# holoskii/Rendering

Measured on AMD Instinct MI355X. Metric: Mrays/s + ms/frame at 4096^2, 250k-tri BVH scene, higher is better.
Workload: dtype f32

## Files before the change

### include/rtx_debug.h

```cpp
#ifndef RTX_DEBUG_H
#define RTX_DEBUG_H
#include "rtx.h"
#ifdef __cplusplus
extern "C" {
#endif

int rtx_frame_mode(rtx_scene* scene, int* mode, float* split_ms, float* fused_ms);
int rtx_set_frame_mode(rtx_scene* scene, int mode);

int rtx_mesh_flatten_probe(const rtx_mesh* mesh, uint32_t* n_wide, void* wide_out, void* prune_out, uint32_t cap_wide, float* root_rec8);
int rtx_wide_node_slots(void);

int rtx_source_p_probe(const float* tris9, uint32_t n, const double* S3, double sigma, int cam, float* out);

int rtx_cost_grid_read(rtx_scene* scene, uint32_t* out, size_t n, uint32_t* grid_w, uint32_t* grid_h);

int rtx_set_knob(rtx_scene* scene, const char* name, double value);

#define RTX_VARIANT_BOXES    1u
#define RTX_VARIANT_PLAIN    2u
#define RTX_VARIANT_ANALYTIC 4u
#define RTX_VARIANT_STATS    8u
#define RTX_VARIANT_CULL     16u
int rtx_kernel_variant(rtx_scene* scene, uint32_t* bits);

int rtx_ssaa_list_read(rtx_scene* scene, uint32_t* info, uint32_t* scan, size_t n);

int rtx_kernel_time_reset(rtx_scene* scene);
int rtx_kernel_time_stats(rtx_scene* scene, int which, uint32_t* launches, double* total_ms);

int rtx_tile_cost_read(rtx_scene* scene, uint32_t* out, size_t n);

int rtx_math_probe(int device, int op, uint32_t n, const float* x, const float* y, float* out);

int rtx_vec_probe(int device, int op, uint32_t n, const float* a, const float* b, float ior, float* out);

int rtx_desc_serialize(const rtx_scene_desc* desc, void* out, size_t cap, size_t* need);

int rtx_bvh_build_mode(int mode);
int rtx_bvh_launches(const rtx_bvh* bvh, uint32_t* launches, int* queued);

int rtx_scene_mesh_read(rtx_scene* scene, uint32_t mesh, uint32_t* counts2, float* node_bounds, int32_t* node_skip, int32_t* leaf_begin,
                        int32_t* leaf_count, uint32_t* refs);
int rtx_scene_mesh_flat_read(rtx_scene* scene, uint32_t mesh, uint32_t* n_wide, void* wide_out, void* prune_out, uint32_t cap_wide, float* root_rec8);
int rtx_scene_edit_times(rtx_scene* scene, float* ms4);
int rtx_scene_lights_read(rtx_scene* scene, uint32_t* n_lights, rtx_light* lights_out, uint32_t cap_lights, size_t* n_point_floats,
                          float* points_out, size_t cap_point_floats);
int rtx_scene_mesh_prune_copy_read(rtx_scene* scene, uint32_t mesh, uint32_t copy, uint32_t* n_copies, uint32_t* n_wide, void* prune_out,
                                   uint32_t cap_wide);
int rtx_scene_objects_read(rtx_scene* scene, uint32_t* n_objects, rtx_object* objects_out, uint32_t cap_objects, uint32_t* n_meshes);

int rtx_live_device_memory(size_t* allocations, size_t* bytes);

#ifdef __cplusplus
}
#endif
#endif
```

### rendering_amd/__init__.py

```python
import ctypes as C
import os

import numpy as np

HERE = os.path.dirname(os.path.abspath(__file__))
ROOT = os.path.dirname(HERE)
LIB_RTX = os.path.join(HERE, "librtx_hip.so")
LIB_HOST = os.path.join(HERE, "librendering_host.so")

__all__ = ["load", "Scene", "Comm", "RtxError", "device_count", "math_probe", "gather_plan", "exported_symbols", "sphere_directions"]


class RtxError(RuntimeError):
    pass


class Counters(C.Structure):
    _fields_ = [("rays", C.c_uint64), ("box_tests", C.c_uint64), ("tri_tests", C.c_uint64), ("moot_rays", C.c_uint64)]


_rtx = None
_host = None

RTX_SYMBOLS = [
    "rtx_last_error", "rtx_device_count", "rtx_scene_create", "rtx_scene_destroy", "rtx_scene_set_view", "rtx_scene_bytes",
    "rtx_render_pass1", "rtx_sobel", "rtx_render_ssaa", "rtx_render_frame", "rtx_render_ac", "rtx_frame_status", "rtx_frame_mode", "rtx_set_frame_mode", "rtx_set_knob", "rtx_cost_grid_read", "rtx_mesh_flatten_probe", "rtx_wide_node_slots", "rtx_source_p_probe", "rtx_quantize_bgr8", "rtx_render_frame_host",
    "rtx_counters_enable", "rtx_counters_reset", "rtx_counters_read", "rtx_last_kernel_ms", "rtx_math_probe",
    "rtx_cast_rays", "rtx_trace_rays", "rtx_kernel_time_reset", "rtx_kernel_time_stats", "rtx_tile_cost_read", "rtx_set_row_ownership",
    "rtx_bvh_build", "rtx_bvh_info", "rtx_bvh_read", "rtx_bvh_destroy",
    "rtx_vec_probe", "rtx_desc_serialize", "rtx_bvh_build_mode", "rtx_bvh_launches", "rtx_comm_unique_id", "rtx_comm_create", "rtx_comm_info", "rtx_comm_destroy", "rtx_comm_agree", "rtx_gather", "rtx_gather_plan",
    "rtx_scene_mesh_read", "rtx_scene_mesh_flat_read", "rtx_scene_edit_times", "rtx_kernel_variant", "rtx_ssaa_list_read", "rtx_live_device_memory",
    "rtx_scene_lights_read", "rtx_scene_mesh_prune_copy_read", "rtx_scene_objects_read",
]

RTX_EDIT_SYMBOLS = ["rtx_scene_set_object", "rtx_scene_update_mesh", "rtx_scene_set_lights", "rtx_scene_set_objects"]

RTX_QUERY_SYMBOLS = ["rtx_occluded_rays"]

RTX_AOV_SYMBOLS = ["rtx_render_aov"]


RTX_AO_SYMBOLS = ["rtx_render_ao"]


class AovBuffers(C.Structure):
    _fields_ = [(n, C.c_void_p) for n in ("depth_dev", "object_dev", "triangle_dev", "uv_dev", "normal_dev", "albedo_dev")]


class AoParams(C.Structure):
    _fields_ = [("n_dirs", C.c_uint32), ("dirs_dev", C.c_void_p), ("radius", C.c_float)]


def sphere_directions(n):
    n = int(n)
    if n < 2 or n % 2:
        raise ValueError("sphere_directions: n must be even and at least 2, got %d" % n)
    i = np.arange(n // 2, dtype=np.float64) + 0.5
    z = 1.0 - 2.0 * i / n
    phi = i * (np.pi * (3.0 - np.sqrt(5.0)))
    r = np.sqrt(1.0 - z * z)
    half = np.stack([r * np.cos(phi), r * np.sin(phi), z], 1).astype(np.float32)
    return np.concatenate([half, -half], 0)


def load():
    global _rtx, _host
    if _rtx is not None:
        return _rtx, _host
    for p in (LIB_RTX, LIB_HOST):
        if not os.path.exists(p):
            raise RtxError("native library %s is missing -- build it with ./build.sh (hipcc, gfx950); "
                           "there is no CPU fallback" % p)
    try:
        import torch
    except Exception:
        pass
    rtx = C.CDLL(LIB_RTX, mode=C.RTLD_GLOBAL)
    host = C.CDLL(LIB_HOST, mode=C.RTLD_GLOBAL)
    rtx.rtx_last_error.restype = C.c_char_p
    vp, u32, i32 = C.c_void_p, C.c_uint32, C.c_int
    rtx.rtx_device_count.argtypes = [C.POINTER(C.c_int)]
    rtx.rtx_render_pass1.argtypes = [vp, u32, u32, vp, vp]
    rtx.rtx_sobel.argtypes = [vp, vp, u32, u32, vp, vp]
    rtx.rtx_render_ssaa.argtypes = [vp, vp, u32, u32, vp, vp]
    rtx.rtx_render_frame.argtypes = [vp, u32, u32, vp, vp, vp]
    rtx.rtx_render_ac.argtypes = [vp, vp, vp, vp]
    rtx.rtx_frame_status.argtypes = [vp, C.POINTER(C.c_uint32)]
    rtx.rtx_set_frame_mode.argtypes = [vp, C.c_int]
    rtx.rtx_set_knob.argtypes = [vp, C.c_char_p, C.c_double]
    rtx.rtx_cost_grid_read.argtypes = [vp, vp, C.c_size_t, C.POINTER(C.c_uint32), C.POINTER(C.c_uint32)]
    rtx.rtx_mesh_flatten_probe.argtypes = [vp, C.POINTER(C.c_uint32), vp, vp, C.c_uint32, vp]
    rtx.rtx_source_p_probe.argtypes = [vp, u32, vp, C.c_double, i32, vp]
    rtx.rtx_frame_mode.argtypes = [vp, C.POINTER(C.c_int), C.POINTER(C.c_float), C.POINTER(C.c_float)]
    rtx.rtx_quantize_bgr8.argtypes = [vp, vp, vp, vp]
    rtx.rtx_render_frame_host.argtypes = [vp, i32, vp]
    rtx.rtx_counters_enable.argtypes = [vp, i32]
    rtx.rtx_counters_reset.argtypes = [vp]
    rtx.rtx_counters_read.argtypes = [vp, C.POINTER(Counters)]
    rtx.rtx_last_kernel_ms.argtypes = [vp, i32, C.POINTER(C.c_float)]
    rtx.rtx_math_probe.argtypes = [i32, i32, u32, vp, vp, vp]
    rtx.rtx_cast_rays.argtypes = [vp, u32, vp, vp, vp]
    rtx.rtx_trace_rays.argtypes = [vp, u32, vp, vp, vp, vp]
    rtx.rtx_occluded_rays.argtypes = [vp, u32, vp, vp, vp, vp]
    rtx.rtx_render_aov.argtypes = [vp, u32, u32, C.POINTER(AovBuffers), vp]
    rtx.rtx_render_ao.argtypes = [vp, u32, u32, C.POINTER(AoParams), vp, vp, vp]
    rtx.rtx_kernel_time_reset.argtypes = [vp]
    rtx.rtx_kernel_time_stats.argtypes = [vp, i32, C.POINTER(C.c_uint32), C.POINTER(C.c_double)]
    rtx.rtx_tile_cost_read.argtypes = [vp, vp, C.c_size_t]
    rtx.rtx_set_row_ownership.argtypes = [vp, u32, u32, u32, i32]
    rtx.rtx_bvh_build.argtypes = [vp, u32, vp, vp, C.c_int32, i32, C.POINTER(vp)]
    rtx.rtx_bvh_info.argtypes = [vp, C.POINTER(u32), C.POINTER(u32), C.POINTER(u32), C.POINTER(C.c_float)]
    rtx.rtx_bvh_launches.argtypes = [vp, C.POINTER(u32), C.POINTER(C.c_int)]
    rtx.rtx_bvh_read.argtypes = [vp, vp, vp, vp, vp, vp]
    rtx.rtx_bvh_destroy.argtypes = [vp]
    rtx.rtx_bvh_destroy.restype = None
    rtx.rtx_scene_bytes.argtypes = [vp, C.POINTER(C.c_size_t)]
    rtx.rtx_vec_probe.argtypes = [i32, i32, u32, vp, vp, C.c_float, vp]
    rtx.rtx_comm_unique_id.argtypes = [vp]
    rtx.rtx_comm_create.argtypes = [vp, i32, i32, i32, C.POINTER(vp)]
    rtx.rtx_comm_info.argtypes = [vp, C.POINTER(C.c_int), C.POINTER(C.c_int)]
    rtx.rtx_comm_destroy.argtypes = [vp]
    rtx.rtx_comm_agree.argtypes = [vp, C.c_int, C.POINTER(C.c_int), vp]
    rtx.rtx_comm_destroy.restype = None
    rtx.rtx_gather.argtypes = [vp, vp, vp, C.c_size_t, i32, i32, vp]
    rtx.rtx_gather_plan.argtypes = [u32, u32, u32, C.c_size_t, i32, u32, vp, vp, vp, C.POINTER(u32)]
    host.rah_set_ac_build.argtypes = [i32, i32]
    host.rah_set_ac_build.restype = None
    host.rah_set_ac_build_device.argtypes = [i32]
    host.rah_set_ac_build_device.restype = None
    host.rah_bvh_build_info.argtypes = [vp, i32, C.POINTER(C.c_int), C.POINTER(C.c_float)]
    host.rah_last_error.restype = C.c_char_p
    host.rah_scene_load.restype = vp
    host.rah_scene_load.argtypes = [C.c_char_p, C.c_char_p, i32, i32]
    host.rah_scene_free.argtypes = [vp]
    host.rah_scene_dims.argtypes = [vp] + [C.POINTER(C.c_int)] * 4
    host.rah_scene_resize.argtypes = [vp, i32, i32]
    host.rah_scene_set_device.argtypes = [vp, i32]
    host.rah_set_flag.argtypes = [vp, C.c_char_p, i32]
    host.rah_flatten.restype = vp
    host.rah_flatten.argtypes = [vp]
    host.rah_flat_desc.restype = vp
    host.rah_flat_desc.argtypes = [vp]
    host.rah_flat_free.argtypes = [vp]
    host.rah_bvh_counts.argtypes = [vp, i32, vp]
    host.rah_scene_gpu.restype = vp
    host.rah_scene_gpu.argtypes = [vp]
    host.rah_render_host.argtypes = [vp, vp, i32]
    host.rah_save_bmp.argtypes = [vp, vp, C.c_char_p]
    host.rah_bvh_dump.argtypes = [vp, i32, vp, vp, vp, vp, vp]
    host.rah_tris.argtypes = [vp, i32, vp]
    host.rah_camera.argtypes = [vp, vp, vp, vp, vp]
    host.rah_scene_digest.argtypes = [vp, vp, i32]
    host.rah_view_flags.argtypes = [vp]
    host.rah_load_bmp.argtypes = [C.c_char_p, C.POINTER(C.c_int), C.POINTER(C.c_int), vp, i32]
    host.rah_object_move.argtypes = [vp, i32] + [vp] * 5
    host.rah_object_type.argtypes = [vp, i32]
    host.rah_object_move_times.argtypes = [vp, vp]
    rtx.rtx_scene_set_object.argtypes = [vp, C.c_uint32, vp]
    rtx.rtx_scene_update_mesh.argtypes = [vp, C.c_uint32, vp, vp, vp, vp, vp, i32, vp]
    rtx.rtx_scene_mesh_read.argtypes = [vp, C.c_uint32] + [vp] * 6
    rtx.rtx_scene_mesh_flat_read.argtypes = [vp, C.c_uint32, vp, vp, vp, C.c_uint32, vp]
    rtx.rtx_scene_edit_times.argtypes = [vp, vp]
    rtx.rtx_kernel_variant.argtypes = [vp, C.POINTER(C.c_uint32)]
    rtx.rtx_ssaa_list_read.argtypes = [vp, vp, vp, C.c_size_t]
    rtx.rtx_live_device_memory.argtypes = [C.POINTER(C.c_size_t), C.POINTER(C.c_size_t)]
    rtx.rtx_scene_set_lights.argtypes = [vp, C.c_uint32, vp]
    rtx.rtx_scene_lights_read.argtypes = [vp, C.POINTER(C.c_uint32), vp, C.c_uint32, C.POINTER(C.c_size_t), vp, C.c_size_t]
    rtx.rtx_scene_mesh_prune_copy_read.argtypes = [vp, C.c_uint32, C.c_uint32, C.POINTER(C.c_uint32), C.POINTER(C.c_uint32), vp, C.c_uint32]
    host.rah_light_type.argtypes = [vp, i32]
    host.rah_light_set.argtypes = [vp, i32] + [vp] * 8
    host.rah_light_add.argtypes = [vp, i32] + [vp] * 8
    host.rah_light_remove.argtypes = [vp, i32]
    rtx.rtx_scene_set_objects.argtypes = [vp, C.c_uint32, vp, C.c_uint32, vp, vp]
    rtx.rtx_scene_objects_read.argtypes = [vp, C.POINTER(C.c_uint32), vp, C.c_uint32, C.POINTER(C.c_uint32)]
    host.rah_object_add.argtypes = [vp, i32, i32, C.c_char_p] + [vp] * 4 + [C.c_char_p] + [vp] * 2 + [C.c_char_p] * 4
    host.rah_object_remove.argtypes = [vp, i32]
    _rtx, _host = rtx, host
    return rtx, host


def exported_symbols():
    rtx, _ = load()
    missing = [s for s in RTX_SYMBOLS + RTX_EDIT_SYMBOLS + RTX_QUERY_SYMBOLS + RTX_AOV_SYMBOLS + RTX_AO_SYMBOLS if not hasattr(rtx, s)]
    return list(RTX_SYMBOLS), missing


VARIANT_BITS = {"boxes": 1, "plain": 2, "analytic": 4, "stats": 8, "cull": 16}


def _check(rc, what):
    if rc != 0:
        raise RtxError("%s failed (%d): %s" % (what, rc, _rtx.rtx_last_error().decode(errors="replace")))


def device_count():
    rtx, _ = load()
    n = C.c_int(0)
    _check(rtx.rtx_device_count(C.byref(n)), "rtx_device_count")
    return n.value


def live_device_memory():
    rtx, _ = load()
    n, b = C.c_size_t(0), C.c_size_t(0)
    _check(rtx.rtx_live_device_memory(C.byref(n), C.byref(b)), "rtx_live_device_memory")
    return n.value, b.value


def _np_ptr(a):
    return a.ctypes.data_as(C.c_void_p)


def set_ac_build(mode, device=0):
    _, host = load()
    host.rah_set_ac_build({"auto": -1, "host": 0, "device": 1}[mode], device)


def bvh_build(tri_pos, root_lo, root_hi, ac_penalty=1, device=0):
    rtx, _ = load()
    pos = np.ascontiguousarray(tri_pos, np.float32).reshape(-1, 9)
    lo = np.ascontiguousarray(root_lo, np.float32); hi = np.ascontiguousarray(root_hi, np.float32)
    b = C.c_void_p()
    _check(rtx.rtx_bvh_build(_np_ptr(pos), pos.shape[0], _np_ptr(lo), _np_ptr(hi), ac_penalty, device, C.byref(b)), "rtx_bvh_build")
    try:
        nn, nr, md, ms = C.c_uint32(), C.c_uint32(), C.c_uint32(), C.c_float()
        _check(rtx.rtx_bvh_info(b, C.byref(nn), C.byref(nr), C.byref(md), C.byref(ms)), "rtx_bvh_info")
        d = dict(bounds=np.zeros((nn.value, 6), np.float32), skip=np.zeros(nn.value, np.int32),
                 leaf_begin=np.zeros(nn.value, np.int32), leaf_count=np.zeros(nn.value, np.int32),
                 refs=np.zeros(nr.value, np.uint32))
        _check(rtx.rtx_bvh_read(b, _np_ptr(d["bounds"]), _np_ptr(d["skip"]), _np_ptr(d["leaf_begin"]), _np_ptr(d["leaf_count"]),
                                _np_ptr(d["refs"])), "rtx_bvh_read")
        d.update(n_nodes=nn.value, n_refs=nr.value, max_depth=md.value, build_ms=ms.value)
        ln, q = C.c_uint32(), C.c_int()
        _check(rtx.rtx_bvh_launches(b, C.byref(ln), C.byref(q)), "rtx_bvh_launches")
        d.update(launches=ln.value, queued=bool(q.value))
        return d
    finally:
        rtx.rtx_bvh_destroy(b)


def bvh_build_mode(mode):
    rtx, _ = load()
    _check(rtx.rtx_bvh_build_mode(int(mode)), "rtx_bvh_build_mode")


def bvh_build_host(tri_pos, root_lo, root_hi, ac_penalty=1):
    _, host = load()
    pos = np.ascontiguousarray(tri_pos, np.float32).reshape(-1, 9)
    lo = np.ascontiguousarray(root_lo, np.float32); hi = np.ascontiguousarray(root_hi, np.float32)
    cnt = np.zeros(4, np.int64)
    host.rah_bvh_from_tris.argtypes = [C.c_void_p, C.c_int, C.c_void_p, C.c_void_p, C.c_int, C.c_void_p] + [C.c_void_p] * 5
    if host.rah_bvh_from_tris(_np_ptr(pos), pos.shape[0], _np_ptr(lo), _np_ptr(hi), ac_penalty, _np_ptr(cnt), None, None, None, None, None) != 0:
        raise RtxError("rah_bvh_from_tris: %s" % host.rah_last_error().decode(errors="replace"))
    nn, nl, nr, md = [int(x) for x in cnt]
    d = dict(bounds=np.zeros((nn, 6), np.float32), skip=np.zeros(nn, np.int32), leaf_begin=np.zeros(nn, np.int32), leaf_count=np.zeros(nn, np.int32),
             refs=np.zeros(max(nr, 1), np.uint32)[:nr])
    host.rah_bvh_from_tris(_np_ptr(pos), pos.shape[0], _np_ptr(lo), _np_ptr(hi), ac_penalty, _np_ptr(cnt), _np_ptr(d["bounds"]), _np_ptr(d["skip"]),
                           _np_ptr(d["leaf_begin"]), _np_ptr(d["leaf_count"]), _np_ptr(d["refs"]))
    d.update(n_nodes=nn, n_leaves=nl, n_refs=nr, max_depth=md)
    return d


def gather_plan(height, band_height, n_parts, row_bytes, bottom_up=False):
    rtx, _ = load()
    n = C.c_uint32(0)
    cap = (height + band_height - 1) // band_height
    owner = np.zeros(cap, np.uint32); off = np.zeros(cap, np.uint64); ln = np.zeros(cap, np.uint64)
    _check(rtx.rtx_gather_plan(height, band_height, n_parts, row_bytes, int(bottom_up), cap, _np_ptr(owner), _np_ptr(off), _np_ptr(ln), C.byref(n)),
           "rtx_gather_plan")
    return [(int(owner[i]), int(off[i]), int(ln[i])) for i in range(n.value)]


class Comm:

    def __init__(self, n_ranks, rank, device, exchange):
        self.rtx, _ = load()
        buf = (C.c_ubyte * 128)()
        if rank == 0:
            _check(self.rtx.rtx_comm_unique_id(buf), "rtx_comm_unique_id")
        raw = exchange(bytes(buf) if rank == 0 else None)
        if len(raw) != 128:
            raise RtxError("communicator id must be 128 bytes")
        self.h = C.c_void_p()
        _check(self.rtx.rtx_comm_create(raw, n_ranks, rank, device, C.byref(self.h)), "rtx_comm_create")
        self.n_ranks, self.rank = n_ranks, rank

    def gather(self, scene, img, bottom_up=False, root=0, stream=None):
        row_bytes = img[0].numel() * img.element_size()
        _check(self.rtx.rtx_gather(scene.gpu(), self.h, C.c_void_p(img.data_ptr()), row_bytes, int(bottom_up), root,
                                   Scene._stream_ptr(stream)), "rtx_gather")

    def info(self):
        n, r = C.c_int(0), C.c_int(0)
        _check(self.rtx.rtx_comm_info(self.h, C.byref(n), C.byref(r)), "rtx_comm_info")
        return n.value, r.value

    def agree(self, ok, stream=None):
        out = C.c_int(0)
        _check(self.rtx.rtx_comm_agree(self.h, int(bool(ok)), C.byref(out), Scene._stream_ptr(stream)), "rtx_comm_agree")
        return bool(out.value)

    def close(self):
        if self.h:
            self.rtx.rtx_comm_destroy(self.h)
            self.h = C.c_void_p()


class RtxLight(C.Structure):
    _fields_ = [("type", C.c_int32), ("color", C.c_float * 3), ("intensity", C.c_float), ("dir", C.c_float * 3), ("pos", C.c_float * 3),
                ("n_points", C.c_uint32), ("points", C.c_void_p)]


LIGHT_TYPES = {"distant": 1, "point": 2, "area": 3}
LIGHT_KEYS = {"distant": ("direction", "color", "intensity"), "point": ("position", "color", "intensity"),
              "area": ("pos", "i", "j", "samples", "color", "intensity")}
_LIGHT_ARGS = ("color", "intensity", "direction", "position", "pos", "i", "j", "samples")


class RtxObject(C.Structure):
    _fields_ = [("type", C.c_int32), ("material", C.c_int32), ("pos", C.c_float * 3), ("color", C.c_float * 3), ("ior", C.c_float),
                ("ambient", C.c_float), ("diffuse", C.c_float), ("specular", C.c_float), ("n_specular", C.c_float), ("radius2", C.c_float),
                ("normal", C.c_float * 3), ("mesh", C.c_int32)]


OBJECT_TYPES = {"sphere": 1, "plane": 2, "mesh": 3}
OBJECT_KEYS = {"sphere": ("pos", "color", "material", "radius"), "plane": ("pos", "color", "material", "normal"),
               "mesh": ("pos", "size", "rot", "color", "material", "name", "diffuse_map", "normal_map", "specular_map")}
_OBJECT_ARGS = ("pos", "size", "rot", "color", "material", "radius", "normal", "name", "diffuse_map", "normal_map", "specular_map")
_OBJECT_TEXT = ("material", "name", "diffuse_map", "normal_map", "specular_map")
MATERIAL_VALUES = {"diffuse": 0, "reflective": 0, "transparent": 1, "phong": 4}


class _RtxMesh(C.Structure):
    _fields_ = [("n_nodes", C.c_uint32), ("n_refs", C.c_uint32), ("n_tris", C.c_uint32), ("node_bounds", C.c_void_p), ("node_skip", C.c_void_p),
                ("leaf_begin", C.c_void_p), ("leaf_count", C.c_void_p), ("refs", C.c_void_p), ("tri_pos", C.c_void_p), ("tri_nrm", C.c_void_p),
                ("tri_uv", C.c_void_p), ("tri_tb", C.c_void_p), ("diffuse_w", C.c_uint32), ("diffuse_h", C.c_uint32), ("diffuse_map", C.c_void_p),
                ("normal_w", C.c_uint32), ("normal_h", C.c_uint32), ("normal_map", C.c_void_p), ("specular_w", C.c_uint32), ("specular_h", C.c_uint32),
                ("specular_map", C.c_void_p)]


class RtxView(C.Structure):
    _fields_ = [("width", C.c_uint32), ("height", C.c_uint32), ("bias", C.c_float), ("max_ray_depth", C.c_int32), ("background", C.c_float * 3),
                ("flags", C.c_uint32), ("cam_pos", C.c_float * 3), ("cam_matrix", C.c_float * 16), ("scale", C.c_float), ("aspect", C.c_float)]


class RtxSceneDesc(C.Structure):
    _fields_ = [("view", RtxView), ("n_objects", C.c_uint32), ("objects", C.POINTER(RtxObject)), ("n_meshes", C.c_uint32),
                ("meshes", C.POINTER(_RtxMesh)), ("n_lights", C.c_uint32), ("lights", C.POINTER(RtxLight)), ("sky_w", C.c_uint32), ("sky_h", C.c_uint32),
                ("sky", C.c_void_p * 6)]


class RtxMeshBuild(C.Structure):
    _fields_ = [("tri_pos_dev", C.c_void_p), ("tri_nrm_dev", C.c_void_p), ("tri_tb_dev", C.c_void_p), ("root_lo", C.c_float * 3),
                ("root_hi", C.c_float * 3), ("ac_penalty", C.c_int32)]


class RtxMeshSource(C.Structure):
    _fields_ = [("keep", C.c_int32), ("mesh", C.POINTER(_RtxMesh)), ("build", C.POINTER(RtxMeshBuild))]


def mesh_flatten_probe(bvh):
    rtx, _ = load()
    bounds = np.ascontiguousarray(bvh["bounds"], np.float32); skip = np.ascontiguousarray(bvh["skip"], np.int32)
    lb = np.ascontiguousarray(bvh["leaf_begin"], np.int32); lc = np.ascontiguousarray(bvh["leaf_count"], np.int32)
    refs = np.ascontiguousarray(bvh["refs"], np.uint32); pos = np.ascontiguousarray(bvh["tris"][:, 0:9], np.float32)
    m = _RtxMesh()
    m.n_nodes, m.n_refs, m.n_tris = len(skip), len(refs), len(pos)
    m.node_bounds, m.node_skip, m.leaf_begin, m.leaf_count = bounds.ctypes.data, skip.ctypes.data, lb.ctypes.data, lc.ctypes.data
    m.refs, m.tri_pos = refs.ctypes.data, pos.ctypes.data
    n = C.c_uint32(0)
    root = np.zeros(8, np.float32)
    _check(rtx.rtx_mesh_flatten_probe(C.byref(m), C.byref(n), None, None, 0, _np_ptr(root)), "rtx_mesh_flatten_probe")
    S = int(rtx.rtx_wide_node_slots())
    wide = np.zeros((n.value, S, 8), np.float32); prune = np.zeros((n.value, 2 * S, 8), np.float32)
    _check(rtx.rtx_mesh_flatten_probe(C.byref(m), C.byref(n), _np_ptr(wide), _np_ptr(prune), n.value, _np_ptr(root)), "rtx_mesh_flatten_probe")
    return wide, prune[:, 0:S], prune[:, S:2 * S], root


def source_p_probe(v0, e1, e2, S, sigma, cam):
    rtx, _ = load()
    t = np.ascontiguousarray(np.concatenate([v0, e1, e2], 1), np.float32)
    S = np.ascontiguousarray(S, np.float64)
    out = np.zeros(len(t), np.float32)
    _check(rtx.rtx_source_p_probe(_np_ptr(t), len(t), _np_ptr(S), float(sigma), 1 if cam else 0, _np_ptr(out)), "rtx_source_p_probe")
    return out


def math_probe(op, x, y=None, device=0):
    rtx, _ = load()
    x = np.ascontiguousarray(x, np.float32)
    out = np.zeros_like(x)
    yp = None
    if y is not None:
        y = np.ascontiguousarray(np.broadcast_to(np.asarray(y, np.float32), x.shape))
        yp = _np_ptr(y)
    _check(rtx.rtx_math_probe(device, op, x.size, _np_ptr(x), yp, _np_ptr(out)), "rtx_math_probe")
    return out


def vec_probe(op, a, b=None, ior=1.0, device=0):
    rtx, _ = load()
    a = np.ascontiguousarray(a, np.float32).reshape(-1, 3)
    out = np.zeros_like(a)
    bp = None
    if b is not None:
        b = np.ascontiguousarray(b, np.float32).reshape(-1, 3)
        bp = _np_ptr(b)
    _check(rtx.rtx_vec_probe(device, op, a.shape[0], _np_ptr(a), bp, ior, _np_ptr(out)), "rtx_vec_probe")
    return out


class Scene:

    def __init__(self, scene_path, width=-1, height=-1, device=0, cwd=ROOT):
        self.rtx, self.host = load()
        self.host.rah_set_ac_build_device(device)
        self.h = C.c_void_p(self.host.rah_scene_load(cwd.encode(), scene_path.encode(), width, height))
        if not self.h:
            raise RtxError("could not load scene %s: %s" % (scene_path, self.host.rah_last_error().decode(errors="replace")))
        self.device = device
        self._cwd = cwd
        self.host.rah_scene_set_device(self.h, device)
        self._dims()
        self._gpu = None

    def _dims(self):
        w, h, no, nl = C.c_int(), C.c_int(), C.c_int(), C.c_int()
        self.host.rah_scene_dims(self.h, C.byref(w), C.byref(h), C.byref(no), C.byref(nl))
        self.width, self.height, self.n_objects, self.n_lights = w.value, h.value, no.value, nl.value

    def close(self):
        if self.h:
            self.host.rah_scene_free(self.h)
            self.h = None
            self._gpu = None

    def resize(self, width, height):
        self.host.rah_scene_resize(self.h, width, height)
        self._dims()

    def camera_pose(self):
        pos, rot = np.zeros(3, np.float32), np.zeros(3, np.float32)
        self.host.rah_camera_get.argtypes = [C.c_void_p] * 3
        self.host.rah_camera_get(self.h, _np_ptr(pos), _np_ptr(rot))
        return pos, rot

    def set_camera(self, pos, rot):
        pos = np.ascontiguousarray(pos, np.float32); rot = np.ascontiguousarray(rot, np.float32)
        self.host.rah_camera_set.argtypes = [C.c_void_p] * 3
        self.host.rah_camera_set(self.h, _np_ptr(pos), _np_ptr(rot))

    def set_flag(self, name, value):
        self.host.rah_set_flag(self.h, name.encode(), int(value))

    def camera(self):
        scale, aspect = C.c_float(), C.c_float()
        m = np.zeros(16, np.float32)
        pos = np.zeros(3, np.float32)
        self.host.rah_camera(self.h, C.byref(scale), C.byref(aspect), _np_ptr(m), _np_ptr(pos))
        return np.float32(scale.value), np.float32(aspect.value), m, pos

    def view_flags(self):
        return self.host.rah_view_flags(self.h)

    def digest(self):
        out = np.zeros(4096, np.float32)
        n = self.host.rah_scene_digest(self.h, _np_ptr(out), out.size)
        return out[:n].copy()

    def bvh(self, obj_idx):
        cnt = np.zeros(5, np.int64)
        if self.host.rah_bvh_counts(self.h, obj_idx, _np_ptr(cnt)) != 0:
            return None
        nn, nl, nr, md, nt = [int(x) for x in cnt]
        d = dict(bounds=np.zeros((nn, 6), np.float32), skip=np.zeros(nn, np.int32),
                 leaf_begin=np.zeros(nn, np.int32), leaf_count=np.zeros(nn, np.int32),
                 refs=np.zeros(nr, np.uint32))
        self.host.rah_bvh_dump(self.h, obj_idx, _np_ptr(d["bounds"]), _np_ptr(d["skip"]), _np_ptr(d["leaf_begin"]),
                               _np_ptr(d["leaf_count"]), _np_ptr(d["refs"]))
        tris = np.zeros((nt, 30), np.float32)
        self.host.rah_tris(self.h, obj_idx, _np_ptr(tris))
        d.update(tris=tris, n_nodes=nn, n_leaves=nl, n_refs=nr, max_depth=md, n_tris=nt)
        on, ms = C.c_int(0), C.c_float(0)
        self.host.rah_bvh_build_info(self.h, obj_idx, C.byref(on), C.byref(ms))
        d.update(built_on_device=bool(on.value), build_ms=ms.value)
        return d

    def bvh_build_info(self, obj_idx):
        on, ms = C.c_int(0), C.c_float(-1)
        if self.host.rah_bvh_build_info(self.h, obj_idx, C.byref(on), C.byref(ms)) != 0:
            return None
        return bool(on.value), ms.value

    def move_object(self, index, pos=None, rot=None, size=None, radius=None, normal=None):
        keys = {"mesh": ("pos", "rot", "size"), "sphere": ("pos", "radius"), "plane": ("pos", "normal")}
        given = {k: v for k, v in (("pos", pos), ("rot", rot), ("size", size), ("radius", radius), ("normal", normal)) if v is not None}
        if not 0 <= index < self.n_objects:
            raise ValueError("move_object: object index %d out of range (%d objects)" % (index, self.n_objects))
        kind = {1: "sphere", 2: "plane", 3: "mesh"}.get(self.host.rah_object_type(self.h, index))
        bad = [k for k in given if kind is None or k not in keys[kind]]
        if bad:
            raise ValueError("move_object: a %s has no key %s (it takes %s)" % (kind, ", ".join(bad), ", ".join(keys.get(kind, ()))))
        arrs = {}
        for k, v in given.items():
            a = np.ascontiguousarray(np.asarray(v, np.float32).reshape(-1))
            if a.size != (1 if k == "radius" else 3):
                raise ValueError("move_object: %s takes %d values, got %d" % (k, 1 if k == "radius" else 3, a.size))
            arrs[k] = a
        ptr = lambda k: _np_ptr(arrs[k]) if k in arrs else None
        if self.host.rah_object_move(self.h, index, ptr("pos"), ptr("rot"), ptr("size"), ptr("radius"), ptr("normal")) != 0:
            raise RtxError("move_object: %s" % self.host.rah_last_error().decode(errors="replace"))

    def light_type(self, index):
        if not 0 <= index < self.n_lights:
            raise ValueError("light_type: light index %d out of range (%d lights)" % (index, self.n_lights))
        return {v: k for k, v in LIGHT_TYPES.items()}[self.host.rah_light_type(self.h, index)]

    @staticmethod
    def _light_args(who, kind, keys):
        bad = [k for k in keys if k not in LIGHT_KEYS[kind]]
        if bad:
            raise ValueError("%s: a %s light has no key %s (it takes %s)" % (who, kind, ", ".join(bad), ", ".join(LIGHT_KEYS[kind])))
        arrs = {}
        for k, v in keys.items():
            want = 1 if k in ("intensity", "samples") else 3
            a = np.ascontiguousarray(np.asarray(v, np.int32 if k == "samples" else np.float32).reshape(-1))
            if a.size != want:
                raise ValueError("%s: %s takes %d value%s, got %d" % (who, k, want, "" if want == 1 else "s", a.size))
            if k == "samples" and a[0] != np.asarray(v).reshape(-1)[0]:
                raise ValueError("%s: samples must be a whole number, got %r" % (who, v))
            arrs[k] = a
        return [_np_ptr(arrs[k]) if k in arrs else None for k in _LIGHT_ARGS], arrs

    def set_light(self, index, **keys):
        if not 0 <= index < self.n_lights:
            raise ValueError("set_light: light index %d out of range (%d lights)" % (index, self.n_lights))
        args, _keep = self._light_args("set_light", self.light_type(index), keys)
        if self.host.rah_light_set(self.h, index, *args) != 0:
            raise RtxError("set_light: %s" % self.host.rah_last_error().decode(errors="replace"))

    def add_light(self, type, **keys):
        if type not in LIGHT_TYPES:
            raise ValueError("add_light: unknown light type %r (point, distant, area)" % (type,))
        args, _keep = self._light_args("add_light", type, keys)
        index = self.host.rah_light_add(self.h, LIGHT_TYPES[type], *args)
        if index < 0:
            raise RtxError("add_light: %s" % self.host.rah_last_error().decode(errors="replace"))
        self._dims()
        return index

    def remove_light(self, index):
        if not 0 <= index < self.n_lights:
            raise ValueError("remove_light: light index %d out of range (%d lights)" % (index, self.n_lights))
        if self.host.rah_light_remove(self.h, index) != 0:
            raise RtxError("remove_light: %s" % self.host.rah_last_error().decode(errors="replace"))
        self._dims()

    def add_object(self, type, at=None, **keys):
        if type not in OBJECT_TYPES:
            raise ValueError("add_object: unknown object type %r (sphere, plane, mesh)" % (type,))
        if at is not None and not 0 <= at <= self.n_objects:
            raise ValueError("add_object: object index %d out of range (%d objects)" % (at, self.n_objects))
        bad = [k for k in keys if k not in OBJECT_KEYS[type]]
        if bad:
            raise ValueError("add_object: a %s has no key %s (it takes %s)" % (type, ", ".join(bad), ", ".join(OBJECT_KEYS[type])))
        arrs = {}
        for k, v in keys.items():
            if k in _OBJECT_TEXT:
                if not isinstance(v, str) or not v or "\n" in v:
                    raise ValueError("add_object: %s takes a line of text, got %r" % (k, v))
                if k == "material":
                    parts = v.split(",")
                    if parts[0] not in MATERIAL_VALUES or len(parts) - 1 != MATERIAL_VALUES[parts[0]]:
                        raise ValueError("add_object: material %r (diffuse, reflective, transparent,<ior>, phong,<ambient>,<diffuse>,<specular>,<n>)" % (v,))
                    try:
                        [float(x) for x in parts[1:]]
                    except ValueError:
                        raise ValueError("add_object: material %r: its values must be numbers" % (v,))
                arrs[k] = v.encode()
                continue
            want = 1 if k == "radius" else 3
            a = np.ascontiguousarray(np.asarray(v, np.float32).reshape(-1))
            if a.size != want:
                raise ValueError("add_object: %s takes %d value%s, got %d" % (k, want, "" if want == 1 else "s", a.size))
            arrs[k] = a
        args = [(arrs[k] if k in _OBJECT_TEXT else _np_ptr(arrs[k])) if k in arrs else None for k in _OBJECT_ARGS]
        index = self.host.rah_object_add(self.h, OBJECT_TYPES[type], -1 if at is None else at, self._cwd.encode(), *args)
        if index < 0:
            raise RtxError("add_object: %s" % self.host.rah_last_error().decode(errors="replace"))
        self._dims()
        return index

    def remove_object(self, index):
        if not 0 <= index < self.n_objects:
            raise ValueError("remove_object: object index %d out of range (%d objects)" % (index, self.n_objects))
        if self.host.rah_object_remove(self.h, index) != 0:
            raise RtxError("remove_object: %s" % self.host.rah_last_error().decode(errors="replace"))
        self._dims()

    def gpu(self):
        self._gpu = C.c_void_p(self.host.rah_scene_gpu(self.h))
        if not self._gpu:
            raise RtxError("no GPU scene: %s" % self.host.rah_last_error().decode(errors="replace"))
        return self._gpu

    @staticmethod
    def _stream_ptr(stream):
        if stream is None:
            try:
                import torch
                if torch.cuda.is_available():
                    return C.c_void_p(torch.cuda.current_stream().cuda_stream)
            except Exception:
                pass
            return None
        return C.c_void_p(getattr(stream, "cuda_stream", stream))

    def render_pass1(self, fb, rows=None, stream=None):
        r0, r1 = rows if rows is not None else (0, self.height)
        _check(self.rtx.rtx_render_pass1(self.gpu(), r0, r1, C.c_void_p(fb.data_ptr()), self._stream_ptr(stream)),
               "rtx_render_pass1")

    def sobel(self, fb, mask, rows=None, stream=None):
        r0, r1 = rows if rows is not None else (0, self.height)
        _check(self.rtx.rtx_sobel(self.gpu(), C.c_void_p(fb.data_ptr()), r0, r1, C.c_void_p(mask.data_ptr()),
                                  self._stream_ptr(stream)), "rtx_sobel")

    def render_ssaa(self, mask, fb, rows=None, stream=None):
        r0, r1 = rows if rows is not None else (0, self.height)
        _check(self.rtx.rtx_render_ssaa(self.gpu(), C.c_void_p(mask.data_ptr()), r0, r1, C.c_void_p(fb.data_ptr()),
                                        self._stream_ptr(stream)), "rtx_render_ssaa")

    def render_frame(self, fb, mask, rows=None, stream=None):
        r0, r1 = rows if rows is not None else (0, self.height)
        _check(self.rtx.rtx_render_frame(self.gpu(), r0, r1, C.c_void_p(fb.data_ptr()), C.c_void_p(mask.data_ptr()),
                                         self._stream_ptr(stream)), "rtx_render_frame")

    def render_ac(self, fb, counts=None, stream=None):
        cp = C.c_void_p(counts.data_ptr()) if counts is not None else None
        _check(self.rtx.rtx_render_ac(self.gpu(), C.c_void_p(fb.data_ptr()), cp, self._stream_ptr(stream)), "rtx_render_ac")

    def set_knob(self, name, value):
        _check(self.rtx.rtx_set_knob(self.gpu(), name.encode(), float(value)), "rtx_set_knob")

    def kernel_variant(self):
        b = C.c_uint32(0)
        _check(self.rtx.rtx_kernel_variant(self.gpu(), C.byref(b)), "rtx_kernel_variant")
        return {k: bool(b.value & bit) for k, bit in VARIANT_BITS.items()}

    def ssaa_list(self):
        g = self.gpu()
        info = np.zeros(16, np.uint32)
        _check(self.rtx.rtx_ssaa_list_read(g, _np_ptr(info), None, 0), "rtx_ssaa_list_read")
        d = dict(local=bool(info[0]), flagged=int(info[1]), sparse=bool(info[2]), tiles=int(info[3]), tiles_x=int(info[4]),
                 heavy_ticks=int(info[5]), spread_slots=int(info[6]), very=int(info[7]), spread_px=int(info[8]),
                 split4=int(info[9]), split16=int(info[10]), cost_sum=int(info[11]) | int(info[12]) << 32, frame_waves=int(info[13]), scan=None)
        if d["tiles"]:
            scan = np.zeros(2 * d["tiles"] + 1, np.uint32)
            _check(self.rtx.rtx_ssaa_list_read(g, _np_ptr(info), _np_ptr(scan), scan.size), "rtx_ssaa_list_read")
            d["scan"] = scan
        return d

    def cost_grid(self):
        gw, gh = C.c_uint32(0), C.c_uint32(0)
        _check(self.rtx.rtx_cost_grid_read(self.gpu(), None, 0, C.byref(gw), C.byref(gh)), "rtx_cost_grid_read")
        g = np.zeros((gh.value, gw.value, 2), np.uint32)
        _check(self.rtx.rtx_cost_grid_read(self.gpu(), _np_ptr(g), g.size, C.byref(gw), C.byref(gh)), "rtx_cost_grid_read")
        return g[..., 0], g[..., 1]

    def frame_status(self):
        st = C.c_uint32(0)
        _check(self.rtx.rtx_frame_status(self.gpu(), C.byref(st)), "rtx_frame_status")
        return st.value

    def set_frame_mode(self, mode):
        _check(self.rtx.rtx_set_frame_mode(self.gpu(), int(mode)), "rtx_set_frame_mode")

    def frame_mode(self):
# ... 277 lines not shown
```

### rendering_amd/csrc/rtx_api.hip

```cpp
#include <hip/hip_runtime.h>

#include <cstdio>
#include <dlfcn.h>
#include <algorithm>
#include <array>
#include <functional>
#include <cmath>
#include <cstring>
#include <memory>
#include <string>
#include <type_traits>
#include <vector>

#include "../../include/rtx.h"
#include "../../include/rtx_debug.h"
#include "../../include/rtx_scene_edit.h"
#include "../../include/rtx_query.h"
#include "../../include/rtx_aov.h"
#include "../../include/rtx_ao.h"
#include "rtx_device.h"
#include "rtx_own.h"

using namespace rtxd;
using rtxown::DevArray; using rtxown::DevBag; using rtxown::Event; using rtxown::PinnedArray;

#include "rtx_kernels.hip"
#include "rtx_source.hip"
#include "rtx_rays.hip"
#include "rtx_aov.hip"
#include "rtx_ao.hip"

hipError_t rtxSortRayKeys(void* temp, size_t* tempBytes, const uint32_t* keysIn, uint32_t* keysOut, uint32_t* order, uint32_t n, int endBit,
                          hipStream_t st);

namespace {

thread_local std::string gErr;

struct RoctxApi { int (*push)(const char*) = nullptr; int (*pop)() = nullptr; };
const RoctxApi& roctx()
{
	static const RoctxApi api = [] {
		RoctxApi a;
		if (!getenv("ROCP_TOOL_LIBRARIES") && !getenv("RTX_ROCTX")) return a;
		void* h = dlopen("librocprofiler-sdk-roctx.so.1", RTLD_NOW | RTLD_GLOBAL);
		if (!h) h = dlopen("libroctx64.so.4", RTLD_NOW | RTLD_GLOBAL);
		if (!h) return a;
		a.push = (int (*)(const char*))dlsym(h, "roctxRangePushA");
		a.pop = (int (*)())dlsym(h, "roctxRangePop");
		if (!a.push || !a.pop) a = RoctxApi();
		return a;
	}();
	return api;
}
struct RoctxRange {
	bool on;
	explicit RoctxRange(const char* name) : on(roctx().push != nullptr) { if (on) roctx().push(name); }
	~RoctxRange() { if (on) roctx().pop(); }
};

int scanExclusive(uint32_t* data, uint32_t n, uint32_t* tmp, hipStream_t st, uint32_t& launches);

int fail(int code, const std::string& msg) { gErr = msg; return code; }

#define HIPCHK(expr)                                                                                         \
	do {                                                                                                     \
		hipError_t e_ = (expr);                                                                              \
		if (e_ != hipSuccess)                                                                                \
			return fail(RTX_ERR_DEVICE, std::string(#expr) + ": " + hipGetErrorString(e_));                  \
	} while (0)

template <typename F> auto dispatchVariant(bool boxes, bool cull, bool third, F&& f)
{
	auto withThird = [&](auto b, auto c) { return third ? f(b, c, std::true_type()) : f(b, c, std::false_type()); };
	auto withCull = [&](auto b) { return cull ? withThird(b, std::integral_constant<int, 1>()) : withThird(b, std::integral_constant<int, 0>()); };
	return boxes ? withCull(std::true_type()) : withCull(std::false_type());
}

}

namespace {

void makeRef(const rtx_mesh& m, uint32_t ref, RefA& a, RefB& b, RefC& c)
{
	const uint32_t t = m.refs[ref];
	const float* p = m.tri_pos + (size_t)t * 9;
	a.v0x = p[0]; a.v0y = p[1]; a.v0z = p[2]; a.tri = t;
	b.e1x = p[3] - p[0]; b.e1y = p[4] - p[1]; b.e1z = p[5] - p[2];
	b.e2x = p[6] - p[0]; c.e2y = p[7] - p[1]; c.e2z = p[8] - p[2];
}

}

struct Knobs {
	int pass1BlocksPerCU = 0, ssaaBlocksPerCU = 0, frameBlocksPerCU = 0;
	bool prune = true;
	bool sources = true;
	int pruneBoxes = -1;
	bool estimate = true;
	bool estimateShadows = true;
	float costPerRef = 2.0f, costPerLeaf = 95.0f, costBase = 6100.0f;
	float fatFactor = 3.0f;
	uint32_t stripLimit = 100000u;
	uint32_t heavyTicks = 18000u;
	uint32_t spreadSlots = 1u << 20;
	uint32_t splitPercent = 100;
	long long localBelow = -1;
	long long sparseBelow = -1;
	int frameMode = -1;
	uint32_t frameRuleTiles = 65536u, frameRuleTilesAnalytic = 8192u;
	uint32_t frameQueueCap = 0;
	bool debugItems = false;
	int traceReorder = -1;
	int traceOriginFirst = 1;
	int occludedSceneOrder = 0;
	uint32_t dbgTile = 0;
};

struct rtx_scene {
	int device = 0;
	int numCUs = 0;
	Knobs knobs;
	DevBag owned;
	DevBag lightsOwned;
	std::vector<Light> lightRecs;
	std::vector<Mesh> meshRecs;
	std::vector<DevBag> meshOwned;
	std::vector<DevBag> meshFixed;
	DevBag recordsOwned;
	std::vector<Object> objectRecs;
	std::vector<rtx_object> objectDescs;
	DevArray<float> sphereLeafDev;
	DevArray<char> flatScratch;
	float editMs[4] = { 0, 0, 0, 0 };
	Params params;
	bool stats = false;
	bool analytic = true;
	bool boxPrune = false;
	bool plain = true;
	DevArray<float> frames; size_t framesArea = 0;
	DevArray<uint32_t> tileCost, items; size_t tileCap = 0;
	DevArray<uint32_t> ssaaPixels;
	DevArray<uint32_t> work;
	DevArray<unsigned long long> counters;
	DevArray<uint32_t> orderWork;
	int blocksPass1 = 0, blocksSsaa = 0, blocksFrame = 0;
	DevArray<uint32_t> tileDeps; DevArray<unsigned long long> tileFlags; DevArray<uint8_t> tileClass;
	DevArray<unsigned long long> ssaaQueue;
	DevArray<unsigned long long> frameCtl;
	uint32_t epoch = 0;
	std::vector<float> meshBounds;
	struct TileQueues {
		std::vector<uint32_t> key;
		uint32_t* list = nullptr;
		uint8_t* need = nullptr; uint32_t listed = 0;
		uint32_t* countExpect = nullptr; bool needValid = false;
		bool costValid = false;
		uint64_t lastUse = 0;
		float frameMs[2] = { -1.f, -1.f };
		uint32_t frameSamples[2] = { 0, 0 };
		uint32_t framesSeen = 0, generation = 0;
		bool fusedGaveUp = false;
		hipStream_t builtOn = nullptr; Event builtEv;
		void forget()
		{
			key.clear(); costValid = false;
			frameMs[0] = frameMs[1] = -1.f; frameSamples[0] = frameSamples[1] = 0; framesSeen = 0; generation++; fusedGaveUp = false;
		}
	};
	struct LastFused { bool valid = false; uint32_t rowBegin = 0, rowEnd = 0; float* fb = nullptr; uint8_t* mask = nullptr; void* stream = nullptr; size_t queue = ~(size_t)0; uint32_t generation = 0;
	                   uint64_t viewSerial = 0; uint32_t bandH = 0, nParts = 0, part = 0, halo = 0; };
	LastFused lastFused;
	uint32_t framesRecovered = 0;
	DevArray<uint32_t> acCounts, acMax;
	DevArray<uint32_t> rayKeys, rayOrder; size_t rayCap = 0;
	DevArray<char> raySortTemp;
	DevArray<uint32_t> rayWork;
	int rayHitBlocks[2] = { 0, 0 };
	int rayOccludedBlocks[2][2] = { { 0, 0 }, { 0, 0 } };
	struct MeshLeaves { const float* boxes; uint32_t n; };
	std::vector<MeshLeaves> meshLeaves;
	DevArray<uint32_t> costGrid;
	DevArray<uint8_t> needSlab; size_t needStride = 0;
	DevArray<uint32_t> listSlab; size_t listStride = 0;
	DevArray<uint32_t> orderedList;
	bool costsUsable = false;
	struct SrcMesh { PruneBlock* pruneAlloc = nullptr; uint32_t pruneWide = 0; PruneBlock* base = nullptr; uint32_t nWide = 0, nRefs = 0; const RefA* refA = nullptr; const RefB* refB = nullptr; const RefC* refC = nullptr;
	                 const uint32_t* slotRange = nullptr; float* refP = nullptr; float* blockP = nullptr; float vmax = 0; uint32_t meshIndex = 0; };
	std::vector<SrcMesh> srcMeshes;
	std::vector<std::array<float, 4>> estLights;
	std::vector<std::array<float, 6>> estPlanes;
	std::vector<std::array<float, 3>> srcLightPos;
	std::vector<uint8_t> srcLightIsPoint;
	float srcNmax = 1.0f;
	float srcBuiltBias = -1.0f; bool srcLightsBuilt = false;
	std::vector<uint8_t> srcLightFresh;
	float srcBuiltCam[3] = { 0, 0, 0 }; bool srcCamBuilt = false;
	hipStream_t lastRenderStream = nullptr; bool rendered = false;
	Event evPrepDone; bool prepRecorded = false; hipStream_t prepSeenBy = nullptr;
	struct RenderStream { hipStream_t st = nullptr; Event done; bool active = false, prepSeen = false; };
	std::vector<RenderStream> renderStreams;
	struct PlanSlot { uint32_t* host = nullptr; uint32_t* dev = nullptr; size_t capWords = 0; PinnedArray<uint32_t> own; Event done; bool used = false; };
	PinnedArray<uint32_t> planRingBase;
	PlanSlot planRing[8]; unsigned planNext = 0;
	bool verifyLists = false;
	struct FrameProbe { Event a, b; int mode = -1; size_t queue = 0; uint32_t generation = 0; bool pending = false, refresh = false; };
	FrameProbe probes[8];
	unsigned probeNext = 0;
	int lastFrameMode = -1, frameModeForced = -1;
	uint64_t viewSerial = 1, ssaaLayoutKey = 0;
	uint32_t ssaaLayoutAge = 0;
	uint32_t ssaaListTiles = 0, ssaaListHeavy = 0, ssaaListSpread = 0;
	size_t lastFrameQueue = ~(size_t)0;
	std::vector<TileQueues> tileQueues;
	uint64_t tileUse = 0;
	std::vector<Event> evPool[5];
	size_t evUsed[5] = { 0, 0, 0, 0, 0 };
	bool evCollect = false;
};

namespace {

void readKnobs(Knobs& k)
{
	const char* allow = ::getenv("RTX_ALLOW_ENV_KNOBS");
	if (!(allow && allow[0] == '1')) return;
	auto getenv = [](const char* name) { return ::getenv(name); };
	auto num = [](const char* name, long long dflt) { const char* e = ::getenv(name); return e ? strtoll(e, nullptr, 10) : dflt; };
	k.pass1BlocksPerCU = (int)num("RTX_PASS1_BLOCKS_PER_CU", 0); k.ssaaBlocksPerCU = (int)num("RTX_SSAA_BLOCKS_PER_CU", 0); k.frameBlocksPerCU = (int)num("RTX_FRAME_BLOCKS_PER_CU", 0);
	k.prune = !getenv("RTX_NO_PRUNE");
	k.sources = !getenv("RTX_NO_SRC");
	k.pruneBoxes = (int)num("RTX_PRUNE_BOXES", -1);
	k.estimate = !getenv("RTX_NO_COST_ESTIMATE");
	k.estimateShadows = !getenv("RTX_NO_SHADOW_ESTIMATE");
	if (const char* e = getenv("RTX_COST_COEFFS")) sscanf(e, "%f,%f,%f", &k.costPerRef, &k.costPerLeaf, &k.costBase);
	if (const char* e = getenv("RTX_FAT_FACTOR")) k.fatFactor = strtof(e, nullptr);
	k.stripLimit = (uint32_t)num("RTX_STRIP_LIMIT", k.stripLimit);
	k.heavyTicks = (uint32_t)num("RTX_SSAA_HEAVY_TICKS", k.heavyTicks);
	k.spreadSlots = (uint32_t)std::min<long long>(num("RTX_SSAA_SPREAD_SLOTS", k.spreadSlots), 1ll << 20);
	k.splitPercent = (uint32_t)num("RTX_SPLIT_PERCENT", k.splitPercent);
	k.localBelow = num("RTX_SSAA_LOCAL_BELOW", -1);
	k.sparseBelow = num("RTX_SSAA_SPARSE_BELOW", -1);
	if (const char* e = getenv("RTX_FRAME_MODE")) k.frameMode = !strcmp(e, "split") ? 0 : (!strcmp(e, "fused") ? 1 : -1);
	k.frameQueueCap = (uint32_t)num("RTX_FRAME_QUEUE_CAP", 0);
	k.debugItems = getenv("RTX_DEBUG_ITEMS") != nullptr;
	if (const char* e = getenv("RTX_DBG_TILE")) { unsigned tx = 0, ty = 0; if (sscanf(e, "%u,%u", &tx, &ty) == 2) k.dbgTile = ((ty << 16) | tx) + 1; }
}

void chooseBoxPrune(rtx_scene* s)
{
	s->boxPrune = false;
	for (const Object& d : s->objectRecs) {
		if (d.type != RTX_OBJ_MESH) continue;
		if (d.pruneBoxes && s->knobs.pruneBoxes != 0) s->boxPrune = true;
		if (s->knobs.pruneBoxes > 0 && d.prune) s->boxPrune = true;
	}
}

int setView(rtx_scene* s, const rtx_view* v)
{
	if (v->width < 2 || v->height < 2) return fail(RTX_ERR_ARG, "view: width/height must be >= 2");
	View& d = s->params.view;
	d.width = v->width; d.height = v->height; d.bias = v->bias; d.maxDepth = v->max_ray_depth;
	memcpy(d.bg, v->background, 12);
	d.flags = v->flags;
	memcpy(d.camPos, v->cam_pos, 12);
	memcpy(d.camM, v->cam_matrix, 64);
	d.scale = v->scale; d.aspect = v->aspect;
	if ((d.flags & RTX_FLAG_SKYBOX) && !s->params.sky) return fail(RTX_ERR_ARG, "view: skybox flag without skybox faces");
	if (d.maxDepth < 0) d.maxDepth = -1;
	return RTX_OK;
}

constexpr size_t kMaxTimedLaunches = 4096;
constexpr uint32_t kSsaaSpreadSlots = 1u << 20;
constexpr size_t kFrameCtlBytes = 256 * 64;

struct Variant { bool analytic, stats, boxes, cull, plain; };
Variant variantOf(const rtx_scene* s)
{
	return { s->analytic, s->stats, s->boxPrune, (s->params.view.flags & RTX_FLAG_BACKFACE_CULL) != 0, s->plain };
}

typedef void (*FrameKernel)(const Params);
FrameKernel pass1Kernel(const Variant& v)
{
	if (v.stats) return rtxPass1Kernel<true>;
	if (v.analytic) return rtxPass1Kernel<false, false>;
	return dispatchVariant(v.boxes, v.cull, v.plain, [](auto b, auto c, auto pl) -> FrameKernel { return rtxPass1Kernel<false, true, decltype(b)::value, decltype(c)::value, decltype(pl)::value>; });
}
FrameKernel ssaaKernel(const Variant& v)
{
	if (v.stats) return rtxSsaaKernel<true>;
	if (v.analytic) return rtxSsaaKernel<false, false>;
	return dispatchVariant(v.boxes, v.cull, v.plain, [](auto b, auto c, auto pl) -> FrameKernel { return rtxSsaaKernel<false, true, decltype(b)::value, decltype(c)::value, decltype(pl)::value>; });
}
FrameKernel frameKernel(const Variant& v)
{
	if (v.analytic) return rtxFrameKernel<false>;
	return dispatchVariant(v.boxes, v.cull, v.plain, [](auto b, auto c, auto pl) -> FrameKernel { return rtxFrameKernel<true, decltype(b)::value, decltype(c)::value, decltype(pl)::value>; });
}
typedef void (*RayKernel)(const Params, const uint32_t*, float*);
RayKernel rayHitKernel(const Variant& v)
{
	if (v.analytic) return rtxRayHitKernel<false, true, -1>;
	return dispatchVariant(v.boxes, v.cull, false, [](auto b, auto c, auto) -> RayKernel { return rtxRayHitKernel<true, decltype(b)::value, decltype(c)::value>; });
}
RayKernel rayColourKernel(const Variant& v)
{
	if (v.analytic) return rtxRayColourKernel<false, true, -1, false>;
	return dispatchVariant(v.boxes, v.cull, v.plain, [](auto b, auto c, auto pl) -> RayKernel { return rtxRayColourKernel<true, decltype(b)::value, decltype(c)::value, decltype(pl)::value>; });
}
typedef void (*AovKernel)(const Params, const rtx_aov_buffers);
AovKernel aovKernel(const Variant& v, bool surface)
{
	if (v.analytic) return surface ? rtxAovKernel<false, true, -1, true> : rtxAovKernel<false, true, -1, false>;
	return dispatchVariant(v.boxes, v.cull, surface, [](auto b, auto c, auto sf) -> AovKernel { return rtxAovKernel<true, decltype(b)::value, decltype(c)::value, decltype(sf)::value>; });
}
typedef void (*AoKernel)(const Params, const AoArgs);
AoKernel aoKernel(const Variant& v)
{
	if (v.analytic) return rtxAoKernel<false, true, -1>;
	return dispatchVariant(v.boxes, v.cull, false, [](auto b, auto c, auto) -> AoKernel { return rtxAoKernel<true, decltype(b)::value, decltype(c)::value>; });
}
typedef void (*OccludedKernel)(const Params, const uint32_t*, const float*, uint8_t*);
OccludedKernel rayOccludedKernel(const Variant& v, bool sceneOrder)
{
	if (v.analytic) return rtxRayOccludedKernel<false, true, -1, true>;
	return dispatchVariant(v.boxes, v.cull, sceneOrder, [](auto b, auto c, auto ord) -> OccludedKernel { return rtxRayOccludedKernel<true, decltype(b)::value, decltype(c)::value, decltype(ord)::value>; });
}

int askBlocksPerCU(int& perCU, const void* kernel)
{
	if (perCU == 0) { HIPCHK(hipOccupancyMaxActiveBlocksPerMultiprocessor(&perCU, kernel, 256, 0)); perCU = std::max(perCU, 1); }
	return RTX_OK;
}

int residentBlocks(const rtx_scene* s, FrameKernel kernel, int knobPerCU, int* blocks)
{
	int b = 0;
	const int rc = askBlocksPerCU(b, (const void*)kernel);
	if (rc) return rc;
	if (knobPerCU >= 1 && knobPerCU < b) b = knobPerCU;
	*blocks = b * s->numCUs;
	return RTX_OK;
}

int askResidentBlocks(rtx_scene* s)
{
	Variant v = { false, false, true, true, s->plain };
	int rc;
	if ((rc = residentBlocks(s, pass1Kernel(v), s->knobs.pass1BlocksPerCU, &s->blocksPass1))) return rc;
	v.plain = false;
	if ((rc = residentBlocks(s, ssaaKernel(v), s->knobs.ssaaBlocksPerCU, &s->blocksSsaa))) return rc;
	v.analytic = s->analytic;
	return residentBlocks(s, frameKernel(v), s->knobs.frameBlocksPerCU, &s->blocksFrame);
}

int ensureWork(rtx_scene* s)
{
	HIPCHK(hipSetDevice(s->device));
	if (!s->work) {
		HIPCHK(s->work.reserve(256));
		HIPCHK(hipMemset(s->work, 0, 256 * sizeof(uint32_t)));
		HIPCHK(s->orderWork.reserve(8 * 32 * 32));
		HIPCHK(s->counters.reserve(16));
		HIPCHK(hipMemset(s->counters, 0, 16 * sizeof(unsigned long long)));
		const int rc = askResidentBlocks(s);
		if (rc) return rc;
	}
	const int blocks = std::max(s->blocksFrame, s->blocksPass1 > s->blocksSsaa ? s->blocksPass1 : s->blocksSsaa);
	const uint32_t totalLanes = (uint32_t)blocks * 256u;
	const int slots = s->params.view.maxDepth + 2;
	const size_t area = (size_t)(slots < 1 ? 1 : slots) * kFrameFields * sizeof(float) * totalLanes;
	const size_t need = 2 * area;
	s->framesArea = area / sizeof(float);
	HIPCHK(s->frames.reserve(need / sizeof(float)));
	const uint32_t txFull = (s->params.view.width + 7) / 8, tyFull = (s->params.view.height + 7) / 8;
	const size_t tiles = (size_t)txFull * tyFull;
	if (tiles > s->tileCap) {
		s->tileCap = 0;
		HIPCHK(s->tileCost.reserve(2 * tiles));
		HIPCHK(s->items.reserve(tiles * 2 + 1 + tiles / 256 + 1024));
		HIPCHK(hipMemset(s->tileCost, 0, 2 * tiles * sizeof(uint32_t)));
		s->tileCap = tiles;
	}
	const size_t pixels = tiles * 64 + kSsaaSpreadSlots;
	HIPCHK(s->ssaaPixels.reserve(pixels));
	s->params.tileCost = s->tileCost;
	s->params.tilesXFull = txFull;
	s->params.frames = s->frames;
	s->params.totalLanes = totalLanes;
	s->params.workCounter = s->work;
	s->params.counters = s->counters;
	return RTX_OK;
}

int prepareView(rtx_scene* s);

int prepBegin(rtx_scene* s)
{
	for (auto& rs : s->renderStreams) {
		if (!rs.active) continue;
		HIPCHK(rs.done.create(hipEventDisableTiming));
		if (hipEventRecord(rs.done, rs.st) == hipSuccess) HIPCHK(hipStreamWaitEvent(nullptr, rs.done, 0));
		else (void)hipGetLastError();
		rs.active = false;
	}
	return RTX_OK;
}
int prepEnd(rtx_scene* s)
{
	HIPCHK(s->evPrepDone.create(hipEventDisableTiming));
	HIPCHK(hipEventRecord(s->evPrepDone, nullptr));
	s->prepRecorded = true; s->prepSeenBy = nullptr;
	for (auto& rs : s->renderStreams) rs.prepSeen = false;
	return RTX_OK;
}
int renderOn(rtx_scene* s, hipStream_t st)
{
	s->lastRenderStream = st; s->rendered = true;
	if (st == nullptr) return RTX_OK;
	rtx_scene::RenderStream* rs = nullptr;
	for (auto& r : s->renderStreams) if (r.st == st) { rs = &r; break; }
	if (!rs) {
		if (s->renderStreams.size() >= 8) { for (auto& r : s->renderStreams) if (!r.active) { rs = &r; break; } }
		if (!rs) { s->renderStreams.emplace_back(); rs = &s->renderStreams.back(); }
		rs->st = st; rs->active = false; rs->prepSeen = false;
	}
	if (s->prepRecorded && !rs->prepSeen) { HIPCHK(hipStreamWaitEvent(st, s->evPrepDone, 0)); rs->prepSeen = true; s->prepSeenBy = st; }
	rs->active = true;
	return RTX_OK;
}

int buildSources(rtx_scene* s)
{
	if (s->srcMeshes.empty() || !s->knobs.sources) return RTX_OK;
	const View& v = s->params.view;
	const bool camSame = s->srcCamBuilt && !memcmp(s->srcBuiltCam, v.camPos, 12);
	const bool lightsSame = s->srcLightsBuilt && s->srcBuiltBias == v.bias;
	if (camSame && lightsSame) return RTX_OK;
	bool any = false;
	for (const auto& sm : s->srcMeshes) any = any || sm.base;
	if (!any) return RTX_OK;
	const uint32_t nLights = std::min<uint32_t>((uint32_t)s->srcLightPos.size(), kMaxSrcLights);
	bool failed = false;
	for (const auto& sm : s->srcMeshes) {
		if (!sm.base) continue;
		auto build = [&](uint32_t copy, const float* S, double sigma, bool cam) {
			PruneBlock* dst = sm.base + (size_t)copy * sm.nWide;
			if (hipMemcpyAsync(dst, sm.base, (size_t)sm.nWide * sizeof(PruneBlock), hipMemcpyDeviceToDevice, nullptr) != hipSuccess) { failed = true; return; }
			if (!(sigma >= 0.0) || !std::isfinite(sigma) || !std::isfinite((double)S[0] + S[1] + S[2])) return;
			hipLaunchKernelGGL(rtxsrc::rtxSourceRefKernel, dim3((sm.nRefs + 255) / 256), dim3(256), 0, nullptr, sm.refA, sm.refB, sm.refC, sm.nRefs,
			                   (double)S[0], (double)S[1], (double)S[2], sigma, cam ? 1 : 0, sm.refP, sm.blockP);
			hipLaunchKernelGGL(rtxsrc::rtxSourceSlotKernel, dim3(sm.nWide * (kWideSlots / 4)), dim3(256), 0, nullptr, sm.slotRange, sm.nWide, (const float*)sm.refP, (const float*)sm.blockP, dst);
		};
		if (!camSame) build(1, v.camPos, 0.0, true);
		if (!lightsSame)
			for (uint32_t l = 0; l < nLights; l++) {
				if (!s->srcLightIsPoint[l]) continue;
				if (s->srcBuiltBias == v.bias && l < s->srcLightFresh.size() && s->srcLightFresh[l]) continue;
				const float* lp = s->srcLightPos[l].data();
				const double nb = (double)s->srcNmax * std::fabs((double)v.bias);
				const double lpm = std::max(std::fabs((double)lp[0]), std::max(std::fabs((double)lp[1]), std::fabs((double)lp[2])));
				const double sigma = nb * 1.001 + 4.0 * 0x1p-24 * (3.01 * ((double)sm.vmax + kSrcAinfMax + nb) + 2.01 * lpm);
				build(2 + l, lp, sigma, false);
			}
	}
	HIPCHK(hipGetLastError());
	s->srcLightFresh.clear();
	if (failed) { s->srcCamBuilt = false; s->srcLightsBuilt = false; return fail(RTX_ERR_DEVICE, "buildSources: a source copy of the prune records could not be reset"); }
	memcpy(s->srcBuiltCam, v.camPos, 12); s->srcCamBuilt = true;
	s->srcBuiltBias = v.bias; s->srcLightsBuilt = true;
	return RTX_OK;
}

int estimateCosts(rtx_scene* s)
{
	s->costsUsable = false;
	if (!s->knobs.estimate || s->meshLeaves.empty() || !s->tileCost) return RTX_OK;
	const View& v = s->params.view;
	const uint32_t txFull = (v.width + 7) / 8, tyFull = (v.height + 7) / 8;
	const uint32_t gridW = (txFull + 1) / 2, gridH = (tyFull + 1) / 2;
	const size_t cells = (size_t)gridW * gridH;
	HIPCHK(s->costGrid.reserve(2 * cells));
	HIPCHK(hipMemsetAsync(s->costGrid, 0, 2 * cells * sizeof(uint32_t), nullptr));
	SplatSources src;
	memset(&src, 0, sizeof(src));
	if (s->knobs.estimateShadows)
		for (size_t l = 0; l < s->estLights.size() && l < 8; l++)
			for (size_t q = 0; q < s->estPlanes.size() && q < 4 && src.n < 16; q++) {
				const auto& L = s->estLights[l]; const auto& P = s->estPlanes[q];
				src.kind[src.n] = L[3] > 2.5f ? 2 : (int32_t)L[3]; src.weight[src.n] = L[3] > 2.5f ? (uint32_t)((L[3] - 2.0f) / 4.0f) : 1u;
				memcpy(src.l[src.n], L.data(), 12); memcpy(src.p[src.n], P.data(), 24);
				src.n++;
			}
	for (const auto& m : s->meshLeaves)
		if (m.n) hipLaunchKernelGGL(rtxCostSplatKernel, dim3((m.n + 255) / 256, 1 + src.n), dim3(256), 0, nullptr, m.boxes, m.n, v, gridW, gridH, s->costGrid, src);
	const uint32_t tiles = txFull * tyFull;
	FarPlanes far;
	memset(&far, 0, sizeof(far));
	if (s->knobs.estimateShadows) {
		for (size_t q = 0; q < s->estPlanes.size() && q < 4; q++) memcpy(far.p[far.n++], s->estPlanes[q].data(), 24);
		far.farDist = 1500.0f; far.farTicks = 200000u;
	}
	hipLaunchKernelGGL(rtxCostFillKernel, dim3((tiles + 255) / 256), dim3(256), 0, nullptr, (const uint32_t*)s->costGrid, gridW, txFull, tyFull, s->tileCost,
	                   s->knobs.costPerRef, s->knobs.costPerLeaf, s->knobs.costBase, v, far);
	HIPCHK(hipGetLastError());
	s->costsUsable = true;
	return RTX_OK;
}

int stamp(rtx_scene* s, int which, hipStream_t st)
{
	if ((s->evUsed[which] & 1) == 0 && s->evUsed[which] >= 2 && (!s->evCollect || s->evUsed[which] >= 2 * kMaxTimedLaunches))
		s->evUsed[which] -= 2;
	if (s->evUsed[which] == s->evPool[which].size()) {
		Event e;
		HIPCHK(e.create());
		s->evPool[which].push_back(std::move(e));
	}
	HIPCHK(hipEventRecord(s->evPool[which][s->evUsed[which]++], st));
	return RTX_OK;
}

}

namespace {

struct FlatMesh {
	std::vector<Node> nodes;
	std::vector<WideNode> wide;
	std::vector<PruneBlock> prune;
	std::vector<uint32_t> slotRange;
	PruneRec rootRec;
	float vmaxMesh = 0;
	bool boxesRegular = true;
};

int flattenMesh(const rtx_mesh& m, bool pruneWanted, FlatMesh& out)
{
	if (!m.node_bounds || !m.node_skip || !m.leaf_begin || !m.leaf_count || (m.n_refs && !m.refs) || (m.n_tris && !m.tri_pos)) return fail(RTX_ERR_ARG, "mesh arrays missing");
	for (uint32_t r = 0; r < m.n_refs; r++)
		if (m.refs[r] >= m.n_tris) return fail(RTX_ERR_ARG, "leaf reference out of range");
	std::vector<Node> nodes(m.n_nodes);
	bool boxesRegular = true;
	for (uint32_t i = 0; i < m.n_nodes; i++) {
		Node& nd = nodes[i];
		for (int c = 0; c < 3; c++) {
			nd.b[2 * c] = m.node_bounds[(size_t)i * 6 + c]; nd.b[2 * c + 1] = m.node_bounds[(size_t)i * 6 + 3 + c];
			if (!(std::fabs(nd.b[2 * c]) < 1e30f && std::fabs(nd.b[2 * c + 1]) < 1e30f && nd.b[2 * c] <= nd.b[2 * c + 1])) boxesRegular = false;
		}
		if (m.leaf_count[i] < 0) {
			if (m.node_skip[i] <= (int32_t)i + 1 || m.node_skip[i] > (int32_t)m.n_nodes) return (fail(RTX_ERR_ARG, "bad skip index"));
			nd.link = m.node_skip[i]; nd.first = 0;
			continue;
		}
		const uint32_t begin = (uint32_t)m.leaf_begin[i], count = (uint32_t)m.leaf_count[i];
		if (begin + count > m.n_refs) return (fail(RTX_ERR_ARG, "leaf range out of bounds"));
		nd.link = ~m.leaf_count[i]; nd.first = (int32_t)begin;
	}
	for (uint32_t i = 0; i < m.n_nodes; i++) {
		if (m.leaf_count[i] >= 0) continue;
		if (i + 1 >= m.n_nodes) return fail(RTX_ERR_ARG, "inner node without children");
		const uint32_t right = m.leaf_count[i + 1] >= 0 ? i + 2 : (uint32_t)m.node_skip[i + 1];
		if (right <= i + 1 || right >= (uint32_t)m.node_skip[i] || right >= m.n_nodes) return fail(RTX_ERR_ARG, "inner node whose right child lies outside its subtree");
	}
	std::vector<WideNode> wide;
	
	std::vector<PruneBlock> prune;
	float vmaxMesh = 0;
	PruneRec rootRec;
	memset(&rootRec, 0, sizeof(rootRec));
	rootRec.h[0] = rootRec.h[1] = rootRec.h[2] = INFINITY; rootRec.P = INFINITY;
	std::vector<std::array<uint32_t, kWideSlots>> slotNode;
	constexpr uint32_t kNoNode = 0xffffffffu;
	std::array<uint32_t, kWideSlots> noSlots; noSlots.fill(kNoNode);
	if (boxesRegular && m.n_nodes > 0) {
		bool nested = true;
		uint32_t depthMax = 0;
		auto isLeaf = [&](uint32_t i) { return m.leaf_count[i] >= 0; };
		auto rightOf = [&](uint32_t i) { return isLeaf(i + 1) ? i + 2 : (uint32_t)m.node_skip[i + 1]; };
		auto inside = [&](uint32_t c, uint32_t p) {
			for (int k = 0; k < 3; k++)
				if (!(nodes[c].b[2 * k] >= nodes[p].b[2 * k] && nodes[c].b[2 * k + 1] <= nodes[p].b[2 * k + 1])) return false;
			return true;
		};
		struct Item { uint32_t node, wideIndex, depth; };
		std::vector<Item> todo;
		wide.emplace_back(); memset(&wide[0], 0, sizeof(WideNode));
		slotNode.push_back(noSlots);
		if (isLeaf(0)) { wide[0].slot[0] = nodes[0]; slotNode[0][0] = 0; }
		else todo.push_back({ 0u, 0u, 1u });
		while (!todo.empty() && nested) {
			const Item it = todo.back(); todo.pop_back();
			depthMax = std::max(depthMax, it.depth);
			uint32_t slots[kWideSlots]; int ns = 0;
			std::function<void(uint32_t, int)> gather = [&](uint32_t node, int levels) {
				if (!nested) return;
				const uint32_t kids[2] = { node + 1, rightOf(node) };
				for (uint32_t c : kids) {
					if (c >= m.n_nodes || !inside(c, node)) { nested = false; return; }
					if (isLeaf(c) || levels == 1) slots[ns++] = c;
					else gather(c, levels - 1);
					if (!nested) return;
				}
			};
			gather(it.node, kWideLevels);
			if (!nested) break;
			uint32_t childWide[kWideSlots] = { 0 };
			for (int k = 0; k < ns; k++)
				if (!isLeaf(slots[k])) { childWide[k] = (uint32_t)wide.size(); wide.emplace_back(); memset(&wide.back(), 0, sizeof(WideNode)); slotNode.push_back(noSlots); }
			for (int k = ns - 1; k >= 0; k--) {
				slotNode[it.wideIndex][k] = slots[k];
				Node sl = nodes[slots[k]];
				if (!isLeaf(slots[k])) { sl.link = (int32_t)childWide[k] + 1; sl.first = 0; todo.push_back({ slots[k], childWide[k], it.depth + 1 }); }
				wide[it.wideIndex].slot[k] = sl;
			}
		}
		if (!nested || (kWideSlots - 1) * depthMax + 1 > kWideStackEntries) wide.clear();
		if (!wide.empty() && pruneWanted) {
			struct Agg { double lo[3], hi[3], ps, qlo[3], qhi[3], wlo, whi; bool planes; uint32_t rb, re; };
			std::vector<Agg> agg(m.n_nodes);
			for (uint32_t i = m.n_nodes; i-- > 0;) {
				Agg& a = agg[i];
				for (int k = 0; k < 3; k++) { a.lo[k] = a.qlo[k] = INFINITY; a.hi[k] = a.qhi[k] = -INFINITY; }
				a.ps = 0; a.wlo = INFINITY; a.whi = -INFINITY; a.planes = true; a.rb = 0xffffffffu; a.re = 0;
				auto merge = [&](const Agg& b) {
					a.rb = std::min(a.rb, b.rb); a.re = std::max(a.re, b.re);
					for (int k = 0; k < 3; k++) {
						a.lo[k] = std::min(a.lo[k], b.lo[k]); a.hi[k] = std::max(a.hi[k], b.hi[k]);
						a.qlo[k] = std::min(a.qlo[k], b.qlo[k]); a.qhi[k] = std::max(a.qhi[k], b.qhi[k]);
					}
					a.ps = std::max(a.ps, b.ps); a.wlo = std::min(a.wlo, b.wlo); a.whi = std::max(a.whi, b.whi);
					a.planes = a.planes && b.planes;
				};
				if (!isLeaf(i)) { merge(agg[i + 1]); merge(agg[rightOf(i)]); continue; }
				const uint32_t begin = (uint32_t)m.leaf_begin[i], count = (uint32_t)m.leaf_count[i];
				if (count) { a.rb = begin; a.re = begin + count; }
				for (uint32_t r = begin; r < begin + count; r++) {
					RefA ra; RefB rb; RefC rc;
					makeRef(m, r, ra, rb, rc);
					const double v0[3] = { ra.v0x, ra.v0y, ra.v0z }, e1[3] = { rb.e1x, rb.e1y, rb.e1z }, e2[3] = { rb.e2x, rc.e2y, rc.e2z };
					double s1 = 0, s2 = 0;
					for (int k = 0; k < 3; k++) {
						const double x1 = v0[k] + e1[k], x2 = v0[k] + e2[k];
						a.lo[k] = std::min(a.lo[k], std::min(v0[k], std::min(x1, x2)));
						a.hi[k] = std::max(a.hi[k], std::max(v0[k], std::max(x1, x2)));
						s1 += std::fabs(e1[k]); s2 += std::fabs(e2[k]);
					}
					a.ps = std::max(a.ps, s1 * s2);
					if (s1 == 0 || s2 == 0) continue;
					const double sc = s1 * s2;
					if (!(sc > 1e-30) || !std::isfinite(sc)) { a.planes = false; continue; }
					const double mq[3] = { (e2[1] * e1[2] - e2[2] * e1[1]) / sc, (e2[2] * e1[0] - e2[0] * e1[2]) / sc, (e2[0] * e1[1] - e2[1] * e1[0]) / sc };
					double w = 0;
					for (int k = 0; k < 3; k++) { a.qlo[k] = std::min(a.qlo[k], mq[k]); a.qhi[k] = std::max(a.qhi[k], mq[k]); w += v0[k] * mq[k]; }
					a.wlo = std::min(a.wlo, w); a.whi = std::max(a.whi, w);
				}
			}
			auto makeRec = [&](const Agg& a, PruneRec& pr) {
				memset(&pr, 0, sizeof(pr));
				pr.h[0] = pr.h[1] = pr.h[2] = -1e30f;
				if (!(a.lo[0] <= a.hi[0])) return;
				bool finite = std::isfinite(a.ps);
				for (int c = 0; c < 3; c++) finite = finite && std::isfinite(a.lo[c]) && std::isfinite(a.hi[c]);
				if (!finite) { pr.h[0] = pr.h[1] = pr.h[2] = INFINITY; pr.P = pr.Pgen = INFINITY; return; }
				for (int c = 0; c < 3; c++) {
					const double mid = 0.5 * (a.lo[c] + a.hi[c]), big = std::max(std::fabs(a.lo[c]), std::fabs(a.hi[c]));
					pr.c[c] = (float)mid;
					pr.h[c] = (float)((0.5 * (a.hi[c] - a.lo[c]) + std::fabs((double)pr.c[c] - mid)) * (1.0 + 0x1p-20) + 0x1p-24 * big + 1e-37);
				}
				pr.P = pr.Pgen = (float)(a.ps * (1.0 + 0x1p-20) + 1e-37);
			};
			makeRec(agg[0], rootRec);
			prune.resize(wide.size());
			out.slotRange.assign(wide.size() * kWideSlots * 2, 0u);
			for (int c = 0; c < 3; c++) vmaxMesh = std::max(vmaxMesh, (float)std::max(std::fabs(agg[0].lo[c]), std::fabs(agg[0].hi[c])));
			for (size_t wi = 0; wi < wide.size(); wi++)
				for (int k = 0; k < kWideSlots; k++) {
					PruneRec& pr = prune[wi].box[k];
					PlaneRec& pl = prune[wi].plane[k];
					memset(&pr, 0, sizeof(pr)); memset(&pl, 0, sizeof(pl));
					pr.h[0] = pr.h[1] = pr.h[2] = -1e30f;
					pl.wlo = -INFINITY; pl.whi = INFINITY;
					const uint32_t nd = slotNode[wi][k];
					if (nd == kNoNode) continue;
					const Agg& a = agg[nd];
					if (a.rb < a.re) { out.slotRange[(wi * kWideSlots + k) * 2] = a.rb; out.slotRange[(wi * kWideSlots + k) * 2 + 1] = a.re; }
					makeRec(a, pr);
					if (!(a.lo[0] <= a.hi[0]) || !std::isfinite(pr.P)) continue;
					if (a.planes && a.wlo <= a.whi && std::isfinite(a.wlo) && std::isfinite(a.whi)) {
						for (int c = 0; c < 3; c++) {
							const double mid = 0.5 * (a.qlo[c] + a.qhi[c]);
							pl.qc[c] = (float)mid;
							pl.qr[c] = (float)((0.5 * (a.qhi[c] - a.qlo[c]) + std::fabs((double)pl.qc[c] - mid)) * (1.0 + 0x1p-20) + 0x1p-24);
						}
						pl.wlo = (float)(a.wlo - (std::fabs(a.wlo) * 0x1p-22 + 1e-37)); pl.whi = (float)(a.whi + (std::fabs(a.whi) * 0x1p-22 + 1e-37));
					}
				}
		}
	}
	out.nodes.swap(nodes); out.wide.swap(wide); out.prune.swap(prune);
	out.rootRec = rootRec; out.vmaxMesh = vmaxMesh; out.boxesRegular = boxesRegular;
	return RTX_OK;
}

int uploadMeshGeometry(rtx_scene* s, const rtx_mesh& m, uint32_t mi, uint32_t nLights, DevBag& owned, Mesh& dm, rtx_scene::SrcMesh& sm,
                       rtx_scene::MeshLeaves& leaves, float bounds[6])
{
	FlatMesh flat;
	{
		const int frc = flattenMesh(m, s->knobs.prune, flat);
		if (frc) return frc;
	}
	std::vector<Node>& nodes = flat.nodes;
	std::vector<WideNode>& wide = flat.wide;
	std::vector<PruneBlock>& prune = flat.prune;
	const PruneRec rootRec = flat.rootRec;
	const float vmaxMesh = flat.vmaxMesh;
	const bool boxesRegular = flat.boxesRegular;
	std::vector<RefA> refA((size_t)m.n_refs + 64);
	std::vector<RefB> refB((size_t)m.n_refs + 64);
	std::vector<RefC> refC((size_t)m.n_refs + 64);
	memset(refA.data(), 0, refA.size() * sizeof(RefA)); memset(refB.data(), 0, refB.size() * sizeof(RefB)); memset(refC.data(), 0, refC.size() * sizeof(RefC));
	for (uint32_t r = 0; r < m.n_refs; r++) {
		if (m.refs[r] >= m.n_tris) return (fail(RTX_ERR_ARG, "leaf reference out of range"));
		makeRef(m, r, refA[r], refB[r], refC[r]);
	}
	for (int c = 0; c < 6; c++) bounds[c] = m.n_nodes ? m.node_bounds[c] : 0.0f;
	HIPCHK(owned.upload(nodes.data(), nodes.size(), &dm.nodes));
	{
		std::vector<float> lb;
		for (uint32_t i = 0; i < m.n_nodes; i++) {
			if (m.leaf_count[i] <= 0) continue;
			float lo[3] = { INFINITY, INFINITY, INFINITY }, hi[3] = { -INFINITY, -INFINITY, -INFINITY };
			for (uint32_t r = (uint32_t)m.leaf_begin[i]; r < (uint32_t)(m.leaf_begin[i] + m.leaf_count[i]); r++) {
				const float* p = m.tri_pos + (size_t)m.refs[r] * 9;
				for (int v = 0; v < 9; v++) { lo[v % 3] = std::min(lo[v % 3], p[v]); hi[v % 3] = std::max(hi[v % 3], p[v]); }
			}
			if (!(std::isfinite(lo[0] + lo[1] + lo[2] + hi[0] + hi[1] + hi[2]))) continue;
			lb.insert(lb.end(), { lo[0], lo[1], lo[2], hi[0], hi[1], hi[2], (float)m.leaf_count[i], 0.0f });
		}
		const float* dev = nullptr;
		HIPCHK(owned.upload(lb.data(), lb.size(), &dev));
		leaves = { dev, (uint32_t)(lb.size() / 8) };
	}
	HIPCHK(owned.upload(wide.data(), wide.size(), &dm.wide));
	dm.nWide = (uint32_t)wide.size();
	sm = rtx_scene::SrcMesh();
	const uint32_t nCopies = (s->knobs.sources && !prune.empty()) ? 2u + std::min<uint32_t>(nLights, kMaxSrcLights) : 1u;
	if (!prune.empty()) {
		PruneBlock* pb = nullptr;
		if (owned.alloc(&pb, (size_t)nCopies * prune.size() * sizeof(PruneBlock)) != hipSuccess) return (fail(RTX_ERR_DEVICE, "hipMalloc (prune blocks)"));
		for (uint32_t c = 0; c < nCopies; c++)
			if (hipMemcpy(pb + (size_t)c * prune.size(), prune.data(), prune.size() * sizeof(PruneBlock), hipMemcpyHostToDevice) != hipSuccess) return (fail(RTX_ERR_DEVICE, "hipMemcpy (prune blocks)"));
		dm.prune = pb;
		sm.pruneAlloc = pb; sm.pruneWide = (uint32_t)prune.size();
		if (nCopies > 1) { sm.base = pb; sm.nWide = (uint32_t)prune.size(); }
	}
	dm.vmax = vmaxMesh;
	dm.rootRec = rootRec;
	if (!(vmaxMesh < 0x1p40f)) { dm.prune = nullptr; dm.rootRec.h[0] = dm.rootRec.h[1] = dm.rootRec.h[2] = INFINITY; }
	HIPCHK(owned.upload(refA.data(), refA.size(), &dm.refA));
	HIPCHK(owned.upload(refB.data(), refB.size(), &dm.refB));
	HIPCHK(owned.upload(refC.data(), refC.size(), &dm.refC));
	if (sm.base && vmaxMesh < 0x1p40f && m.n_refs) {
		sm.nRefs = m.n_refs; sm.refA = dm.refA; sm.refB = dm.refB; sm.refC = dm.refC; sm.vmax = vmaxMesh; sm.meshIndex = mi;
		HIPCHK(owned.upload(flat.slotRange.data(), flat.slotRange.size(), &sm.slotRange));
		if (owned.alloc(&sm.refP, ((size_t)m.n_refs + m.n_refs / 64 + 2) * sizeof(float), false) != hipSuccess) return (fail(RTX_ERR_DEVICE, "hipMalloc (source scratch)"));
		sm.blockP = sm.refP + m.n_refs;
	}
	else sm.base = nullptr;
	dm.nNodes = m.n_nodes; dm.nRefs = m.n_refs; dm.nTris = m.n_tris; dm.boxesRegular = boxesRegular ? 1u : 0u;
	{
		double sum = 0; size_t cnt = 0;
		const size_t stride = m.n_refs > 65536 ? m.n_refs / 65536 : 1;
		for (size_t r = 0; r < m.n_refs; r += stride) {
			const RefB& b = refB[r]; const RefC& c = refC[r];
			const double l1 = std::sqrt((double)b.e1x * b.e1x + (double)b.e1y * b.e1y + (double)b.e1z * b.e1z);
			const double l2 = std::sqrt((double)b.e2x * b.e2x + (double)c.e2y * c.e2y + (double)c.e2z * c.e2z);
			if (std::isfinite(l1 + l2)) { sum += l1 + l2; cnt += 2; }
		}
		const float factor = s->knobs.fatFactor;
		dm.fatRadius = cnt && factor > 0 ? (float)(sum / (double)cnt) * factor : INFINITY;
		double rad = 0;
		for (int c = 0; c < 3; c++) {
			const double lo = m.n_nodes ? m.node_bounds[c] : 0.0, hi = m.n_nodes ? m.node_bounds[3 + c] : 0.0;
			dm.centre[c] = (float)(0.5 * (lo + hi)); rad += 0.25 * (hi - lo) * (hi - lo);
		}
		dm.radius = (float)std::sqrt(rad);
		if (!std::isfinite(dm.radius)) { dm.radius = 0; dm.fatRadius = INFINITY; }
	}
	return RTX_OK;
}

void meshObjectRecord(const float* bx, Object& d, const Mesh& dm, const rtx_scene::SrcMesh& sm)
{
	for (int c = 0; c < 3; c++) { d.rootBox[2 * c] = bx[c]; d.rootBox[2 * c + 1] = bx[3 + c]; }
	d.fatRadius = dm.fatRadius; memcpy(d.centre, dm.centre, 12); d.radius = dm.radius;
	d.meshFlags = (dm.nNodes ? 1u : 0u) | (dm.boxesRegular ? 2u : 0u) | (dm.nWide ? 4u : 0u);
	d.nodes = dm.nodes; d.refA = dm.refA; d.refB = dm.refB; d.refC = dm.refC; d.wide = dm.wide; d.prune = dm.prune;
	d.nNodes = dm.nNodes; d.vmax = dm.vmax;
	d.srcStride = (dm.prune && sm.base) ? sm.nWide : 0u;
	d.pruneBoxes = (dm.prune && std::isfinite(dm.rootRec.P) && dm.rootRec.P < 1.0f / 216.0f) ? 1u : 0u;
}

int checkMesh(const rtx_mesh& m)
{
	if (!m.node_bounds || !m.node_skip || !m.leaf_begin || !m.leaf_count || (m.n_refs && !m.refs) || (m.n_tris && (!m.tri_pos || !m.tri_nrm || !m.tri_uv)))
		return fail(RTX_ERR_ARG, "mesh arrays missing");
	if (m.normal_map && !m.tri_tb) return fail(RTX_ERR_ARG, "normal map without tangents");
	return RTX_OK;
}

int uploadMeshFixed(const rtx_mesh& m, DevBag& fixed, Mesh& dm)
{
	HIPCHK(fixed.upload(m.tri_uv, (size_t)m.n_tris * 6, &dm.uv));
	HIPCHK(fixed.upload(m.diffuse_map, (size_t)m.diffuse_w * m.diffuse_h * 3, &dm.diffuse));
	HIPCHK(fixed.upload(m.normal_map, (size_t)m.normal_w * m.normal_h * 3, &dm.normal));
	HIPCHK(fixed.upload(m.specular_map, (size_t)m.specular_w * m.specular_h, &dm.specular));
	dm.dW = m.diffuse_w; dm.dH = m.diffuse_h; dm.nW = m.normal_w; dm.nH = m.normal_h; dm.sW = m.specular_w; dm.sH = m.specular_h;
	return RTX_OK;
}

int uploadMesh(rtx_scene* s, const rtx_mesh& m, uint32_t mi, uint32_t nLights, DevBag& owned, DevBag& fixed, Mesh& dm, rtx_scene::SrcMesh& sm,
               rtx_scene::MeshLeaves& leaves, float bounds[6])
{
	memset(&dm, 0, sizeof(dm));
	int rc;
	if ((rc = uploadMeshGeometry(s, m, mi, nLights, owned, dm, sm, leaves, bounds))) return rc;
	HIPCHK(owned.upload(m.tri_nrm, (size_t)m.n_tris * 9, &dm.nrm));
	HIPCHK(owned.upload(m.tri_tb, m.tri_tb ? (size_t)m.n_tris * 6 : 0, &dm.tb));
	return uploadMeshFixed(m, fixed, dm);
}

int checkObjects(uint32_t n, const rtx_object* objects, uint32_t nMeshes)
{
	if (n && !objects) return fail(RTX_ERR_ARG, "objects is NULL");
	for (uint32_t i = 0; i < n; i++) {
		const rtx_object& o = objects[i];
		if (o.type < RTX_OBJ_SPHERE || o.type > RTX_OBJ_MESH) return fail(RTX_ERR_ARG, "bad object type");
		if (o.material < 0 || o.material > 3) return fail(RTX_ERR_ARG, "bad material");
		if (o.type == RTX_OBJ_MESH && (o.mesh < 0 || (uint32_t)o.mesh >= nMeshes)) return fail(RTX_ERR_ARG, "bad mesh index");
	}
	return RTX_OK;
}

std::vector<Object> objectRecords(uint32_t n, const rtx_object* objects, const std::vector<Mesh>& meshes, const std::vector<rtx_scene::SrcMesh>& sms,
                                  const std::vector<float>& meshBounds)
{
	std::vector<Object> objs(n);
	for (uint32_t i = 0; i < n; i++) {
		const rtx_object& o = objects[i];
		Object& d = objs[i];
		memset(&d, 0, sizeof(d));
		d.type = o.type; d.material = o.material;
		memcpy(d.pos, o.pos, 12); memcpy(d.color, o.color, 12); memcpy(d.normal, o.normal, 12);
		d.ior = o.ior; d.ambient = o.ambient; d.diffuse = o.diffuse; d.specular = o.specular; d.nSpecular = o.n_specular;
		d.r2 = o.radius2; d.mesh = o.mesh;
		if (o.type == RTX_OBJ_MESH) meshObjectRecord(&meshBounds[(size_t)o.mesh * 6], d, meshes[o.mesh], sms[o.mesh]);
	}
	return objs;
}

int uploadRecords(const std::vector<Mesh>& meshes, const std::vector<Object>& objs, const std::vector<float>& sb, DevBag& bag, const Mesh** devMeshes,
                  const Object** devObjs, const float** devSpheres)
{
	HIPCHK(bag.upload(sb.data(), sb.size(), devSpheres));
	HIPCHK(bag.upload(meshes.data(), meshes.size(), devMeshes));
	HIPCHK(bag.upload(objs.data(), objs.size(), devObjs));
	return RTX_OK;
}

void chooseAnalytic(rtx_scene* s)
{
	s->analytic = true;
	for (const Object& d : s->objectRecs) if (d.type == RTX_OBJ_MESH) s->analytic = false;
}

int checkLights(uint32_t n, const rtx_light* lights)
{
	if (n && !lights) return fail(RTX_ERR_ARG, "lights is NULL");
	for (uint32_t i = 0; i < n; i++) {
		const rtx_light& l = lights[i];
		if (l.type < RTX_LIGHT_DISTANT || l.type > RTX_LIGHT_AREA) return fail(RTX_ERR_ARG, "bad light type");
		if (l.type == RTX_LIGHT_AREA && (!l.points || l.n_points == 0)) return fail(RTX_ERR_ARG, "area light without sample points");
	}
	return RTX_OK;
}

int uploadLights(uint32_t n, const rtx_light* lights, DevBag& bag, std::vector<Light>& recs, const Light** dev)
{
	recs.resize(n);
	for (uint32_t i = 0; i < n; i++) {
		const rtx_light& l = lights[i];
		Light& d = recs[i];
		memset(&d, 0, sizeof(d));
		d.type = l.type; memcpy(d.color, l.color, 12); d.intensity = l.intensity;
		memcpy(d.dir, l.dir, 12); memcpy(d.pos, l.pos, 12);
		d.nPoints = l.n_points;
		if (l.type == RTX_LIGHT_AREA) HIPCHK(bag.upload(l.points, (size_t)l.n_points * 3, &d.points));
	}
	HIPCHK(bag.upload(recs.data(), recs.size(), dev));
	return RTX_OK;
}

void deriveLights(rtx_scene* s, uint32_t n, const rtx_light* lights)
{
	s->srcLightPos.clear(); s->srcLightIsPoint.clear(); s->estLights.clear();
	for (uint32_t i = 0; i < n; i++) {
		const rtx_light& l = lights[i];
		s->srcLightPos.push_back({ { l.pos[0], l.pos[1], l.pos[2] } });
		s->srcLightIsPoint.push_back(l.type == RTX_LIGHT_POINT ? 1 : 0);
		if (l.type == RTX_LIGHT_POINT) s->estLights.push_back({ { l.pos[0], l.pos[1], l.pos[2], 2.0f } });
		else if (l.type == RTX_LIGHT_DISTANT) s->estLights.push_back({ { l.dir[0], l.dir[1], l.dir[2], 1.0f } });
		else if (l.type == RTX_LIGHT_AREA) s->estLights.push_back({ { l.pos[0], l.pos[1], l.pos[2], 2.0f + 4.0f * (float)std::min<uint32_t>(l.n_points, 4096u) } });
	}
	s->params.nLights = n;
	s->params.nSrcLights = s->knobs.sources ? std::min<uint32_t>(n, kMaxSrcLights) : 0u;
}

void choosePlain(rtx_scene* s)
{
	s->plain = true;
	for (const Object& d : s->objectRecs) if (d.material != 0) s->plain = false;
	for (const Light& l : s->lightRecs) if (l.type == RTX_LIGHT_AREA) s->plain = false;
}

std::vector<float> analyticEstimate(rtx_scene* s, const rtx_object* objects, size_t n)
{
	std::vector<float> sb;
	s->estPlanes.clear();
	s->srcNmax = 1.0f;
	for (size_t i = 0; i < n; i++) {
		const rtx_object& o = objects[i];
		if (o.type == RTX_OBJ_PLANE) {
			s->estPlanes.push_back({ { o.pos[0], o.pos[1], o.pos[2], o.normal[0], o.normal[1], o.normal[2] } });
			const double nl = std::sqrt((double)o.normal[0] * o.normal[0] + (double)o.normal[1] * o.normal[1] + (double)o.normal[2] * o.normal[2]);
			if (!(nl <= 1e30)) s->srcNmax = INFINITY; else s->srcNmax = std::max(s->srcNmax, (float)(nl * 1.000001));
		}
		if (o.type != RTX_OBJ_SPHERE || !(o.radius2 > 0) || !std::isfinite(o.radius2)) continue;
		const float r = std::sqrt(o.radius2), w = (o.material == 1 || o.material == 2) ? 4000.0f : 300.0f;
		sb.insert(sb.end(), { o.pos[0] - r, o.pos[1] - r, o.pos[2] - r, o.pos[0] + r, o.pos[1] + r, o.pos[2] + r, w, 0.0f });
	}
	s->params.srcNmax2 = s->srcNmax * s->srcNmax * 1.00001f;
	return sb;
}

}

extern "C" {

const char* rtx_last_error(void) { return gErr.c_str(); }

int rtx_device_count(int* count)
{
	if (!count) return fail(RTX_ERR_ARG, "count is NULL");
	*count = 0;
	int n = 0;
	hipError_t e = hipGetDeviceCount(&n);
	if (e != hipSuccess) return fail(RTX_ERR_NO_DEVICE, std::string("hipGetDeviceCount: ") + hipGetErrorString(e));
	*count = n;
	return RTX_OK;
}

int rtx_scene_create(const rtx_scene_desc* desc, int device, rtx_scene** out)
{
	if (!desc || !out) return fail(RTX_ERR_ARG, "desc/out is NULL");
	*out = nullptr;
	int n = 0;
	if (hipGetDeviceCount(&n) != hipSuccess || n <= 0) return fail(RTX_ERR_NO_DEVICE, "no HIP device visible");
	if (device < 0 || device >= n) return fail(RTX_ERR_ARG, "device index out of range");
	HIPCHK(hipSetDevice(device));
	hipDeviceProp_t prop;
	HIPCHK(hipGetDeviceProperties(&prop, device));

	std::unique_ptr<rtx_scene, void (*)(rtx_scene*)> hold(new rtx_scene, rtx_scene_destroy);
	rtx_scene* s = hold.get();
	readKnobs(s->knobs);
	s->tileQueues.reserve(16);
	s->device = device;
	s->numCUs = prop.multiProcessorCount;
	memset(&s->params, 0, sizeof(Params));

	int rc;
	std::vector<Mesh> meshes(desc->n_meshes);
	s->meshOwned.resize(desc->n_meshes);
	s->meshFixed.resize(desc->n_meshes);
	for (uint32_t mi = 0; mi < desc->n_meshes; mi++) {
		const rtx_mesh& m = desc->meshes[mi];
		if ((rc = checkMesh(m))) return rc;
		rtx_scene::SrcMesh sm;
		rtx_scene::MeshLeaves leaves{ nullptr, 0 };
		float bounds[6];
		if ((rc = uploadMesh(s, m, mi, desc->n_lights, s->meshOwned[mi], s->meshFixed[mi], meshes[mi], sm, leaves, bounds))) return rc;
		s->meshBounds.insert(s->meshBounds.end(), bounds, bounds + 6);
		s->meshLeaves.push_back(leaves);
		s->srcMeshes.push_back(sm);
	}
	if ((rc = checkObjects(desc->n_objects, desc->objects, desc->n_meshes))) return rc;
	std::vector<Object> objs = objectRecords(desc->n_objects, desc->objects, meshes, s->srcMeshes, s->meshBounds);
	if ((rc = checkLights(desc->n_lights, desc->lights))) return rc;
	{
		const std::vector<float> sb = analyticEstimate(s, desc->objects, desc->n_objects);
		const float* dev = nullptr;
		if ((rc = uploadRecords(meshes, objs, sb, s->recordsOwned, &s->params.meshes, &s->params.objects, &dev))) return rc;
		if (!sb.empty()) s->meshLeaves.push_back({ dev, (uint32_t)(sb.size() / 8) });
	}
	s->meshRecs = meshes; s->objectRecs = objs;
	chooseAnalytic(s);
	chooseBoxPrune(s);
	s->objectDescs.assign(desc->objects, desc->objects + desc->n_objects);
	if ((rc = uploadLights(desc->n_lights, desc->lights, s->lightsOwned, s->lightRecs, &s->params.lights))) return rc;
	s->params.nObjects = desc->n_objects;
	deriveLights(s, desc->n_lights, desc->lights);
// ... 699 lines not shown
	const uint32_t scanN = 2 * p.nTiles + 1;
	uint32_t localBelow = (uint32_t)s->blocksSsaa * 4u * 16u * 8u;
	if (s->knobs.localBelow >= 0) localBelow = (uint32_t)std::min<long long>(s->knobs.localBelow, 0xffffffffll);
	uint32_t* mode = s->work + 8;
	uint32_t launches = 0;
	const uint64_t key = (((((((uint64_t)s->viewSerial * 0x9e3779b97f4a7c15ull + W) * 31 + H) * 31 + rowBegin) * 31 + rowEnd) * 31 + p.bandH * 64 + p.nParts * 8 + p.part) * 31 + localBelow) * 31 + (uint64_t)(s->knobs.sparseBelow + 1);
	const bool decideNow = key != s->ssaaLayoutKey || (s->ssaaLayoutAge++ & 15u) == 15u;
	if (decideNow) {
		hipLaunchKernelGGL(rtxSsaaCountKernel, dim3((scanN + 255) / 256), dim3(256), 0, st, p, s->items, mode, heavyTicks, 0u, 0u, 0u);
		if ((rc = scanExclusive(s->items, scanN, s->items + scanN, st, launches))) return rc;
		HIPCHK(hipMemcpyAsync(mode + 1, s->items + 2 * (size_t)p.nTiles, sizeof(uint32_t), hipMemcpyDeviceToDevice, st));
		s->ssaaLayoutKey = key; s->ssaaLayoutAge = 0;
	}
	uint32_t sparseBelow = (uint32_t)s->blocksSsaa * 4u * 16u / 2u;
	if (s->knobs.sparseBelow >= 0) sparseBelow = (uint32_t)std::min<long long>(s->knobs.sparseBelow, 0xffffffffll);
	hipLaunchKernelGGL(rtxSsaaCountKernel, dim3((scanN + 255) / 256), dim3(256), 0, st, p, s->items, mode, heavyTicks, decideNow ? 1u : 2u, localBelow, spreadSlots, sparseBelow);
	if ((rc = scanExclusive(s->items, scanN, s->items + scanN, st, launches))) return rc;
	hipLaunchKernelGGL(rtxSsaaScatterKernel, dim3((p.nTiles + 255) / 256), dim3(256), 0, st, p, s->items, mode, s->ssaaPixels);
	HIPCHK(hipGetLastError());
	s->ssaaListTiles = p.nTiles; s->ssaaListHeavy = heavyTicks; s->ssaaListSpread = spreadSlots;
	hipLaunchKernelGGL(ssaaKernel(variantOf(s)), dim3(s->blocksSsaa), dim3(256), 0, st, p);
	HIPCHK(hipGetLastError());
	if ((rc = stamp(s, 2, st))) return rc;
	return RTX_OK;
}

int rtx_quantize_bgr8(rtx_scene* s, const float* fb_dev, uint8_t* bgr_dev, void* stream)
{
	if (!s || !fb_dev || !bgr_dev) return fail(RTX_ERR_ARG, "scene/fb/out is NULL");
	const uint32_t W = s->params.view.width, H = s->params.view.height;
	if (W % 4) return fail(RTX_ERR_UNSUPPORTED, "saveImage is only defined for width % 4 == 0 (util.cpp:28-29)");
	HIPCHK(hipSetDevice(s->device));
	if (((uintptr_t)fb_dev & 15u) || ((uintptr_t)bgr_dev & 3u)) return fail(RTX_ERR_ARG, "rtx_quantize_bgr8: fb must be 16-byte aligned, the image 4-byte aligned");
	const size_t n = (size_t)(W / 4) * H;
	if (int ro = renderOn(s, (hipStream_t)stream)) return ro;
	hipLaunchKernelGGL(rtxQuantizeKernel, dim3((unsigned)((n + 255) / 256)), dim3(256), 0, (hipStream_t)stream, fb_dev, bgr_dev, W, H,
	                   s->params.bandH, s->params.nParts, s->params.part);
	HIPCHK(hipGetLastError());
	return RTX_OK;
}

int rtx_render_frame_host(rtx_scene* s, int with_ssaa, float* fb_host)
{
	if (!s || !fb_host) return fail(RTX_ERR_ARG, "scene/fb is NULL");
	HIPCHK(hipSetDevice(s->device));
	const uint32_t W = s->params.view.width, H = s->params.view.height;
	const size_t bytes = (size_t)W * H * 3 * sizeof(float);
	DevArray<float> fb; DevArray<uint8_t> mask;
	HIPCHK(fb.reserve((size_t)W * H * 3));
	HIPCHK(hipMemset(fb, 0, bytes));
	int rc = rtx_render_pass1(s, 0, H, fb, nullptr);
	if (rc) return rc;
	if (with_ssaa) {
		HIPCHK(mask.reserve((size_t)W * H));
		if ((rc = rtx_sobel(s, fb, 0, H, mask, nullptr))) return rc;
		if ((rc = rtx_render_ssaa(s, mask, 0, H, fb, nullptr))) return rc;
	}
	HIPCHK(hipMemcpy(fb_host, fb, bytes, hipMemcpyDeviceToHost));
	return RTX_OK;
}

int rtx_render_ac(rtx_scene* s, float* fb_dev, uint32_t* counts_dev, void* stream)
{
	RoctxRange range("Render AC heat map (rtx_render_ac)");
	if (!s || !fb_dev) return fail(RTX_ERR_ARG, "scene/fb is NULL");
	if (s->params.bandH != 0 && s->params.nParts > 1) return fail(RTX_ERR_ARG, "rtx_render_ac: the heat map is normalised by the maximum of the whole frame -- not under row ownership with more than one part");
	if (s->stats) return fail(RTX_ERR_ARG, "rtx_render_ac: the debug views collect no statistics (rtx_counters_enable)");
	int rc = ensureWork(s);
	if (rc) return rc;
	const uint32_t W = s->params.view.width, H = s->params.view.height;
	const size_t px = (size_t)W * H;
	const size_t waves = (size_t)((W + 7) / 8) * ((H + 7) / 8);
	if (waves >= (1ull << 32)) return fail(RTX_ERR_ARG, "frame too large");
	HIPCHK(s->acMax.reserve(1));
	uint32_t* counts = counts_dev;
	if (!counts) {
		if (s->acCounts.capacity() < px) {
			HIPCHK(hipDeviceSynchronize());
			HIPCHK(s->acCounts.reserve(px));
		}
		counts = s->acCounts;
	}
	hipStream_t st = (hipStream_t)stream;
	if (int ro = renderOn(s, st)) return ro;
	HIPCHK(hipMemsetAsync(s->acMax, 0, sizeof(uint32_t), st));
	hipLaunchKernelGGL(rtxAcCountKernel, dim3((unsigned)((waves + 3) / 4)), dim3(256), 0, st, s->params, counts, s->acMax);
	HIPCHK(hipGetLastError());
	hipLaunchKernelGGL(rtxAcNormalizeKernel, dim3((unsigned)((px + 255) / 256)), dim3(256), 0, st, (const uint32_t*)counts, (const uint32_t*)s->acMax, fb_dev, px);
	HIPCHK(hipGetLastError());
	return RTX_OK;
}

int rtx_counters_enable(rtx_scene* s, int enable)
{
	if (!s) return fail(RTX_ERR_ARG, "scene is NULL");
	s->stats = enable != 0;
	return RTX_OK;
}

int rtx_counters_reset(rtx_scene* s)
{
	if (!s) return fail(RTX_ERR_ARG, "scene is NULL");
	int rc = ensureWork(s);
	if (rc) return rc;
	HIPCHK(hipDeviceSynchronize());
	HIPCHK(hipMemset(s->counters, 0, 16 * sizeof(unsigned long long)));
	return RTX_OK;
}

int rtx_counters_read(rtx_scene* s, rtx_counters* out)
{
	if (!s || !out) return fail(RTX_ERR_ARG, "scene/out is NULL");
	int rc = ensureWork(s);
	if (rc) return rc;
	HIPCHK(hipDeviceSynchronize());
	unsigned long long c[16];
	HIPCHK(hipMemcpy(c, s->counters, sizeof(c), hipMemcpyDeviceToHost));
	out->rays = c[0]; out->box_tests = c[1]; out->tri_tests = c[2]; out->moot_rays = c[15];
	if (s->knobs.debugItems) fprintf(stderr, "[rtx] slowest work item %.3f ms, sum of items %.3f ms (100 MHz wall clock)\n", c[3] * 1e-5, c[4] * 1e-5);
	if (s->knobs.debugItems) fprintf(stderr, "[rtx] wave-level: node visits %llu, reached leaves %llu, filter passes (64 references) %llu, of which rejected whole by stage 1 %llu, by stage 2 %llu; survivors tested exactly %llu; slots pruned by their records %llu, per-ray slot tests %llu, evaluations of prune records %llu\n", c[5], c[10], c[12], c[13], c[7], c[6], c[11], c[8], c[9]);
#if RTX_DBG || RTX_WAVE_TRACE
	if (s->knobs.debugItems) {
		std::vector<unsigned long long> w(3 * 16384);
		HIPCHK(hipMemcpyFromSymbol(w.data(), HIP_SYMBOL(gDbgWave), w.size() * 8));
		unsigned long long t0 = ~0ull, t1 = 0; double busy = 0; int n = 0;
		for (int i = 0; i < 16384; i++) if (w[3 * i]) { t0 = std::min(t0, w[3 * i]); t1 = std::max(t1, w[3 * i + 1]); busy += (double)w[3 * i + 2]; n++; }
		if (n) {
			int hist[10] = { 0 }; double idleEnd = 0, idleStart = 0;
			for (int i = 0; i < 16384; i++) if (w[3 * i]) { int b = (int)(10.0 * (double)(w[3 * i + 1] - t0) / (double)(t1 - t0 + 1)); hist[b < 0 ? 0 : b > 9 ? 9 : b]++; idleEnd += (double)(t1 - w[3 * i + 1]); idleStart += (double)(w[3 * i] - t0); }
			fprintf(stderr, "[rtx] pass-1 waves %d: span %.3f ms, mean busy %.3f ms, mean idle before first tile %.3f ms, after last tile %.3f ms; waves ending in each tenth of the span:", n, (t1 - t0) * 1e-5, busy / n * 1e-5, idleStart / n * 1e-5, idleEnd / n * 1e-5);
			for (int b = 0; b < 10; b++) fprintf(stderr, " %d", hist[b]);
			fprintf(stderr, "\n");
			fprintf(stderr, "[rtx] waves still rendering x ms before the end:");
			for (int k = 12; k >= 0; k--) { int m = 0; const double at = (double)t1 - k * 5000.0; for (int i = 0; i < 16384; i++) if (w[3 * i] && (double)w[3 * i + 1] > at) m++; fprintf(stderr, " %.2f:%d", k * 0.05, m); }
			fprintf(stderr, "\n");
		}
	}
#endif
#if RTX_DBG
	if (s->knobs.debugItems) {
		unsigned long long h[64];
		HIPCHK(hipMemcpyFromSymbol(h, HIP_SYMBOL(gDbgHist), sizeof(h)));
		{ unsigned long long z[8] = {}; HIPCHK(hipMemcpyToSymbol(HIP_SYMBOL(gDbgHist), z, sizeof(z), 8 * sizeof(unsigned long long))); }
		static const char* names[10] = { "depth limit sky", "next light", "lights done: mirror", "lights done: transparent", "return: mirror", "return: transparent 1", "return: transparent 2", "consume: miss", "consume: shade", "consume: shadow" };
		for (int k = 0; k < 10; k++) if (h[17 + 2 * k]) fprintf(stderr, "[rtx]   %-26s %8llu wave-level executions, %7.0f cycles each\n", names[k], h[17 + 2 * k], (double)h[16 + 2 * k] / (double)h[17 + 2 * k]);
		{ unsigned long long z[32] = {}; HIPCHK(hipMemcpyToSymbol(HIP_SYMBOL(gDbgHist), z, sizeof(z), 16 * sizeof(unsigned long long))); }
		if (h[32] + h[33] + h[34]) fprintf(stderr, "[rtx] walk cycles (waves whose walk ended early inside the reference passes are not counted for that batch): nodes %llu, reference passes without the exact tests %llu, exact tests %llu\n", h[32], h[33], h[34]);
		{ unsigned long long z[3] = {}; HIPCHK(hipMemcpyToSymbol(HIP_SYMBOL(gDbgHist), z, sizeof(z), 32 * sizeof(unsigned long long))); }
		if (h[40]) fprintf(stderr, "[rtx] wide walks %llu, of shadow bundles %llu: their node visits %llu, leaves %llu, filter passes %llu, exact tests %llu (these six: since the last print)\n", h[40], h[41], h[42], h[43], h[44], h[45]);
		{ unsigned long long z[6] = {}; HIPCHK(hipMemcpyToSymbol(HIP_SYMBOL(gDbgHist), z, sizeof(z), 40 * sizeof(unsigned long long))); }
		if (h[15]) fprintf(stderr, "[rtx] work items %llu: slowest = %llu trace rounds, %llu cycles in Render::trace + %llu in the castRay state machine; "
		                   "all items: %llu rounds, %.0f + %.0f cycles per round\n", h[15], h[9], h[10], h[11], h[12], (double)h[13] / (double)h[12], (double)h[14] / (double)h[12]);
	}
#endif
#if RTX_DBG >= 2
	if (s->knobs.debugItems) {
		unsigned long long h[64];
		HIPCHK(hipMemcpyFromSymbol(h, HIP_SYMBOL(gDbgHist), sizeof(h)));
		{ unsigned long long z[64] = {}; HIPCHK(hipMemcpyToSymbol(HIP_SYMBOL(gDbgHist), z, sizeof(z))); }
		if (h[0]) fprintf(stderr, "[rtx] certificates (one sampled lane per evaluation): %llu, back-facing %.1f%%, facing %.1f%% (behind %.1f%%, miss %.1f%%, neither %.1f%%), uncertain %.1f%%; skipped %.1f%%\n",
		                  h[0], 100.0 * h[1] / h[0], 100.0 * h[2] / h[0], 100.0 * h[4] / h[0], 100.0 * h[5] / h[0], 100.0 * h[6] / h[0], 100.0 * (h[0] - h[1] - h[2]) / h[0], 100.0 * h[7] / h[0]);
		for (int b = 0; b < 12; b++)
			if (h[16 + b]) fprintf(stderr, "[rtx]   leaves of %4d..%4d refs: unskipped wave visits %10llu, chunk headers %10llu, triangle iterations %10llu\n", 1 << b, (2 << b) - 1, h[16 + b], h[32 + b], h[48 + b]);
	}
#endif
	return RTX_OK;
}

int rtx_last_kernel_ms(rtx_scene* s, int which, float* ms)
{
	if (!s || !ms || which < 0 || which > 4) return fail(RTX_ERR_ARG, "bad argument");
	const size_t n = s->evUsed[which];
	if (n < 2) return fail(RTX_ERR_ARG, "no such launch recorded yet");
	HIPCHK(hipSetDevice(s->device));
	HIPCHK(hipEventSynchronize(s->evPool[which][n - 1]));
	HIPCHK(hipEventElapsedTime(ms, s->evPool[which][n - 2], s->evPool[which][n - 1]));
	return RTX_OK;
}

int rtx_kernel_time_reset(rtx_scene* s)
{
	if (!s) return fail(RTX_ERR_ARG, "scene is NULL");
	for (int i = 0; i < 5; i++) s->evUsed[i] = 0;
	s->evCollect = true;
	return RTX_OK;
}

int rtx_kernel_time_stats(rtx_scene* s, int which, uint32_t* launches, double* total_ms)
{
	if (!s || !launches || !total_ms || which < 0 || which > 4) return fail(RTX_ERR_ARG, "bad argument");
	HIPCHK(hipSetDevice(s->device));
	*launches = 0; *total_ms = 0;
	for (size_t i = 0; i + 1 < s->evUsed[which]; i += 2) {
		float ms = 0;
		HIPCHK(hipEventSynchronize(s->evPool[which][i + 1]));
		HIPCHK(hipEventElapsedTime(&ms, s->evPool[which][i], s->evPool[which][i + 1]));
		*total_ms += ms; (*launches)++;
	}
	return RTX_OK;
}

int rtx_scene_bytes(rtx_scene* s, size_t* bytes)
{
	if (!s || !bytes) return fail(RTX_ERR_ARG, "scene/bytes is NULL");
	*bytes = s->owned.bytes() + s->lightsOwned.bytes() + s->recordsOwned.bytes();
	for (const DevBag& m : s->meshOwned) *bytes += m.bytes();
	for (const DevBag& m : s->meshFixed) *bytes += m.bytes();
	return RTX_OK;
}

int rtx_live_device_memory(size_t* allocations, size_t* bytes)
{
	if (allocations) *allocations = rtxown::gLiveAllocations.load();
	if (bytes) *bytes = rtxown::gLiveBytes.load();
	return RTX_OK;
}

int rtx_tile_cost_read(rtx_scene* s, uint32_t* out, size_t n)
{
	if (!s || !out) return fail(RTX_ERR_ARG, "scene/out is NULL");
	HIPCHK(hipSetDevice(s->device));
	const size_t tiles = (size_t)((s->params.view.width + 7) / 8) * ((s->params.view.height + 7) / 8);
	if (n != tiles && n != 2 * tiles) return fail(RTX_ERR_ARG, "n must be ceil(width/8) * ceil(height/8), or twice that");
	if (!s->tileCost || s->tileCap < tiles) return fail(RTX_ERR_ARG, "no pass 1 has run at this size");
	HIPCHK(hipDeviceSynchronize());
	HIPCHK(hipMemcpy(out, s->tileCost, n * sizeof(uint32_t), hipMemcpyDeviceToHost));
	return RTX_OK;
}

int rtx_cost_grid_read(rtx_scene* s, uint32_t* out, size_t n, uint32_t* grid_w, uint32_t* grid_h)
{
	if (!s || !grid_w || !grid_h) return fail(RTX_ERR_ARG, "scene/grid_w/grid_h is NULL");
	const View& v = s->params.view;
	*grid_w = ((v.width + 7) / 8 + 1) / 2; *grid_h = ((v.height + 7) / 8 + 1) / 2;
	if (!out) return RTX_OK;
	if (!s->costsUsable || !s->costGrid) return fail(RTX_ERR_ARG, "no cost estimate for this view");
	const size_t cells = (size_t)*grid_w * *grid_h;
	HIPCHK(hipSetDevice(s->device));
	HIPCHK(hipDeviceSynchronize());
	HIPCHK(hipMemcpy(out, s->costGrid, std::min(n, 2 * cells) * sizeof(uint32_t), hipMemcpyDeviceToHost));
	return RTX_OK;
}

int rtx_source_p_probe(const float* tris9, uint32_t n, const double* S3, double sigma, int cam, float* out)
{
	if (!tris9 || !S3 || !out) return fail(RTX_ERR_ARG, "rtx_source_p_probe: NULL argument");
	for (uint32_t i = 0; i < n; i++) out[i] = rtxsrc::sourceP(tris9 + (size_t)i * 9, tris9 + (size_t)i * 9 + 3, tris9 + (size_t)i * 9 + 6, S3, sigma, cam != 0);
	return RTX_OK;
}

int rtx_wide_node_slots(void) { return kWideSlots; }

int rtx_desc_serialize(const rtx_scene_desc* d, void* out, size_t cap, size_t* need)
{
	if (!d || !need) return fail(RTX_ERR_ARG, "desc/need is NULL");
	size_t at = 0;
	auto put = [&](const void* src, size_t bytes) {
		if (out && src && at + bytes <= cap) memcpy((char*)out + at, src, bytes);
		at += bytes;
	};
	auto put32 = [&](uint32_t v) { put(&v, 4); };
	auto arr = [&](const void* p, size_t n, size_t elem) {
		put32(p ? 1u : 0u);
		const unsigned long long cnt = p ? n : 0;
		put(&cnt, 8);
		if (p) put(p, n * elem);
	};
	put("RTXD0001", 8);
	static_assert(sizeof(rtx_view) == 4 * 29, "rtx_view has no padding");
	put(&d->view, sizeof(rtx_view));
	put32(d->n_objects);
	static_assert(sizeof(rtx_object) == 4 * 18, "rtx_object has no padding");
	if (d->n_objects && !d->objects) return fail(RTX_ERR_ARG, "objects is NULL");
	put(d->objects, (size_t)d->n_objects * sizeof(rtx_object));
	put32(d->n_meshes);
	if (d->n_meshes && !d->meshes) return fail(RTX_ERR_ARG, "meshes is NULL");
	for (uint32_t i = 0; i < d->n_meshes; i++) {
		const rtx_mesh& m = d->meshes[i];
		put32(m.n_nodes); put32(m.n_refs); put32(m.n_tris);
		arr(m.node_bounds, (size_t)m.n_nodes * 6, 4); arr(m.node_skip, m.n_nodes, 4); arr(m.leaf_begin, m.n_nodes, 4); arr(m.leaf_count, m.n_nodes, 4);
		arr(m.refs, m.n_refs, 4);
		arr(m.tri_pos, (size_t)m.n_tris * 9, 4); arr(m.tri_nrm, (size_t)m.n_tris * 9, 4); arr(m.tri_uv, (size_t)m.n_tris * 6, 4);
		arr(m.normal_map ? m.tri_tb : nullptr, (size_t)m.n_tris * 6, 4);
		put32(m.diffuse_map ? m.diffuse_w : 0u); put32(m.diffuse_map ? m.diffuse_h : 0u); arr(m.diffuse_map, (size_t)m.diffuse_w * m.diffuse_h * 3, 4);
		put32(m.normal_map ? m.normal_w : 0u); put32(m.normal_map ? m.normal_h : 0u); arr(m.normal_map, (size_t)m.normal_w * m.normal_h * 3, 4);
		put32(m.specular_map ? m.specular_w : 0u); put32(m.specular_map ? m.specular_h : 0u); arr(m.specular_map, (size_t)m.specular_w * m.specular_h, 4);
	}
	put32(d->n_lights);
	if (d->n_lights && !d->lights) return fail(RTX_ERR_ARG, "lights is NULL");
	for (uint32_t i = 0; i < d->n_lights; i++) {
		const rtx_light& l = d->lights[i];
		put32((uint32_t)l.type); put(l.color, 12); put(&l.intensity, 4); put(l.dir, 12); put(l.pos, 12);
		arr(l.type == RTX_LIGHT_AREA ? l.points : nullptr, (size_t)l.n_points * 3, 4);
	}
	const bool sky = d->sky_w && d->sky_h && d->sky[0];
	put32(sky ? d->sky_w : 0u); put32(sky ? d->sky_h : 0u);
	for (int k = 0; k < 6; k++) arr(sky ? d->sky[k] : nullptr, (size_t)d->sky_w * d->sky_h * 3, 4);
	*need = at;
	return RTX_OK;
}

int rtx_mesh_flatten_probe(const rtx_mesh* m, uint32_t* n_wide, void* wide_out, void* prune_out, uint32_t cap_wide, float* root_rec8)
{
	if (!m || !n_wide) return fail(RTX_ERR_ARG, "mesh/n_wide is NULL");
	FlatMesh flat;
	int rc = flattenMesh(*m, true, flat);
	if (rc) return rc;
	*n_wide = (uint32_t)flat.wide.size();
	if (root_rec8) memcpy(root_rec8, &flat.rootRec, sizeof(PruneRec));
	if (flat.prune.size() != flat.wide.size() && !flat.wide.empty()) return fail(RTX_ERR_DEVICE, "prune blocks missing");
	const size_t n = std::min<size_t>(cap_wide, flat.wide.size());
	if (wide_out && n) memcpy(wide_out, flat.wide.data(), n * sizeof(WideNode));
	if (prune_out && n) memcpy(prune_out, flat.prune.data(), n * sizeof(PruneBlock));
	return RTX_OK;
}

int rtx_set_row_ownership(rtx_scene* s, uint32_t band_height, uint32_t n_parts, uint32_t part, int halo)
{
	if (!s) return fail(RTX_ERR_ARG, "scene is NULL");
	if (band_height != 0 && (n_parts == 0 || part >= n_parts)) return fail(RTX_ERR_ARG, "bad ownership");
	s->params.bandH = band_height; s->params.nParts = n_parts ? n_parts : 1; s->params.part = part; s->params.halo = halo ? 1u : 0u;
	s->lastFused.valid = false;
	return RTX_OK;
}

int rtx_cast_rays(rtx_scene* s, uint32_t n, const float* rays, float* hits, float* colours)
{
	if (!s || !rays || !hits || !colours) return fail(RTX_ERR_ARG, "NULL argument");
	if (n == 0) return RTX_OK;
	int rc = ensureWork(s);
	if (rc) return rc;
	DevArray<float> dr, dh, dc;
	HIPCHK(dr.reserve((size_t)n * 6)); HIPCHK(dh.reserve((size_t)n * 8)); HIPCHK(dc.reserve((size_t)n * 3));
	HIPCHK(hipMemcpy(dr, rays, (size_t)n * 24, hipMemcpyHostToDevice));
	HIPCHK(hipMemset(s->work + 3, 0, sizeof(uint32_t)));
	Params p = s->params;
	p.workCounter = s->work + 3;
	p.probeRays = dr; p.probeHits = dh; p.probeColours = dc; p.nProbe = n;
	uint32_t blocks = (uint32_t)s->blocksPass1;
	const uint32_t need = ((n + 63) / 64 + 3) / 4;
	if (blocks > need) blocks = need;
	if (showNormals(s)) hipLaunchKernelGGL(rtxNormalsKernel, dim3(need), dim3(256), 0, nullptr, p, 2);
	else hipLaunchKernelGGL(rtxProbeKernel, dim3(blocks), dim3(256), 0, nullptr, p);
	HIPCHK(hipGetLastError());
	HIPCHK(hipMemcpy(hits, dh, (size_t)n * 32, hipMemcpyDeviceToHost));
	HIPCHK(hipMemcpy(colours, dc, (size_t)n * 12, hipMemcpyDeviceToHost));
	return RTX_OK;
}

namespace {

constexpr uint32_t kTraceReorderMin = 1u << 20;
constexpr uint32_t kOccludedReorderMin = kTraceReorderMin;

int ensureRayScratch(rtx_scene* s, uint32_t n, bool reorder, hipStream_t st)
{
	HIPCHK(s->rayWork.reserve(64));
	if (!reorder) return RTX_OK;
	if (n > s->rayCap) {
		s->rayCap = 0;
		HIPCHK(s->rayKeys.reserve(2 * (size_t)n));
		HIPCHK(s->rayOrder.reserve(n));
		s->rayCap = n;
	}
	size_t bytes = 0;
	HIPCHK(rtxSortRayKeys(nullptr, &bytes, s->rayKeys, s->rayKeys + s->rayCap, s->rayOrder, n, kRayKeyBits, st));
	HIPCHK(s->raySortTemp.reserve(bytes));
	return RTX_OK;
}

int groupRays(rtx_scene* s, const Params& p, const float* rays_dev, uint32_t n, hipStream_t st, const uint32_t** order)
{
	const float* M = p.view.camM;
	const RayAxes ax = { { M[0], M[1], M[2], M[4], M[5], M[6], M[8], M[9], M[10] }, { p.view.camPos[0], p.view.camPos[1], p.view.camPos[2] } };
	const uint32_t groups = (uint32_t)(((size_t)n + 255) / 256);
	double* spread = (double*)(s->rayWork + 44);
	hipLaunchKernelGGL(rtxRayBoxKernel, dim3(std::min<uint32_t>(groups, (uint32_t)s->numCUs * 8u)), dim3(256), 0, st, rays_dev, n, ax, s->rayWork + 32, spread);
	hipLaunchKernelGGL(rtxRayKeyKernel, dim3(groups), dim3(256), 0, st, rays_dev, n, ax, (const uint32_t*)(s->rayWork + 32), (const double*)spread,
	                   s->knobs.traceOriginFirst, s->knobs.traceReorder < 0 ? 1 : 0, s->rayKeys);
	size_t bytes = s->raySortTemp.capacity();
	HIPCHK(rtxSortRayKeys(s->raySortTemp.get(), &bytes, s->rayKeys, s->rayKeys + s->rayCap, s->rayOrder, n, kRayKeyBits, st));
	*order = s->rayOrder;
	return RTX_OK;
}

int beginRays(rtx_scene* s, uint32_t n, const float* rays_dev, uint32_t reorderMin, hipStream_t st, Params& p, const uint32_t** order)
{
	int rc = ensureWork(s);
	if (rc) return rc;
	if ((rc = renderOn(s, st))) return rc;
	const bool reorder = s->knobs.traceReorder < 0 ? n >= reorderMin : s->knobs.traceReorder != 0;
	if ((rc = ensureRayScratch(s, n, reorder, st))) return rc;
	p = s->params;
	p.probeRays = rays_dev; p.nProbe = n;
	hipLaunchKernelGGL(rtxRayInitKernel, dim3(1), dim3(64), 0, st, s->rayWork.get());
	*order = nullptr;
	if (reorder && (rc = groupRays(s, p, rays_dev, n, st, order))) return rc;
	return RTX_OK;
}

}

int rtx_trace_rays(rtx_scene* s, uint32_t n, const float* rays_dev, float* hits_dev, float* colours_dev, void* stream)
{
	RoctxRange range("Trace rays (rtx_trace_rays)");
	if (!s) return fail(RTX_ERR_ARG, "scene is NULL");
	if (!hits_dev && !colours_dev) return fail(RTX_ERR_ARG, "rtx_trace_rays: no output (hits and colours are both NULL)");
	if (n == 0) return RTX_OK;
	if (!rays_dev) return fail(RTX_ERR_ARG, "rays is NULL");
	if (n > 0xffffffc0u) return fail(RTX_ERR_ARG, "too many rays");
	hipStream_t st = (hipStream_t)stream;
	Params p;
	const uint32_t* order = nullptr;
	if (int rc = beginRays(s, n, rays_dev, kTraceReorderMin, st, p, &order)) return rc;
	const uint32_t waves = (n + 63) / 64;
	const Variant v = variantOf(s);
	if (showNormals(s)) {
		p.workCounter = s->rayWork;
		const uint32_t blocks = std::min<uint32_t>((uint32_t)s->blocksPass1, (waves + 3) / 4);
		hipLaunchKernelGGL(rtxRayNormalsKernel, dim3(blocks), dim3(256), 0, st, p, order, hits_dev, colours_dev);
	}
	else {
		if (hits_dev) {
			const RayKernel k = rayHitKernel(v);
			int& perCU = s->rayHitBlocks[v.cull ? 1 : 0];
			if (int rc = askBlocksPerCU(perCU, (const void*)k)) return rc;
			p.workCounter = s->rayWork;
			const uint32_t blocks = std::min<uint32_t>((uint32_t)(perCU * s->numCUs), (waves + 3) / 4);
			hipLaunchKernelGGL(k, dim3(blocks), dim3(256), 0, st, p, order, hits_dev);
		}
		if (colours_dev) {
			p.workCounter = s->rayWork + 16;
			const uint32_t blocks = std::min<uint32_t>((uint32_t)s->blocksPass1, (waves + 3) / 4);
			hipLaunchKernelGGL(rayColourKernel(v), dim3(blocks), dim3(256), 0, st, p, order, colours_dev);
		}
	}
	HIPCHK(hipGetLastError());
	return RTX_OK;
}

int rtx_occluded_rays(rtx_scene* s, uint32_t n, const float* rays_dev, const float* tmax_dev, uint8_t* occluded_dev, void* stream)
{
	RoctxRange range("Occluded rays (rtx_occluded_rays)");
	if (!s) return fail(RTX_ERR_ARG, "scene is NULL");
	if (n == 0) return RTX_OK;
	if (!rays_dev) return fail(RTX_ERR_ARG, "rays is NULL");
	if (!occluded_dev) return fail(RTX_ERR_ARG, "rtx_occluded_rays: no output (occluded is NULL)");
	if (n > 0xffffffc0u) return fail(RTX_ERR_ARG, "too many rays");
	hipStream_t st = (hipStream_t)stream;
	Params p;
	const uint32_t* order = nullptr;
	if (int rc = beginRays(s, n, rays_dev, kOccludedReorderMin, st, p, &order)) return rc;
	const Variant v = variantOf(s);
	const bool sceneOrder = s->knobs.occludedSceneOrder != 0;
	const OccludedKernel k = rayOccludedKernel(v, sceneOrder);
	int& perCU = s->rayOccludedBlocks[v.cull ? 1 : 0][sceneOrder ? 1 : 0];
	if (int rc = askBlocksPerCU(perCU, (const void*)k)) return rc;
	p.workCounter = s->rayWork;
	const uint32_t waves = (n + 63) / 64;
	const uint32_t blocks = std::min<uint32_t>((uint32_t)(perCU * s->numCUs), (waves + 3) / 4);
	hipLaunchKernelGGL(k, dim3(blocks), dim3(256), 0, st, p, order, tmax_dev, occluded_dev);
	HIPCHK(hipGetLastError());
	return RTX_OK;
}

int rtx_render_aov(rtx_scene* s, uint32_t rowBegin, uint32_t rowEnd, const rtx_aov_buffers* out, void* stream)
{
	RoctxRange range("First-hit buffers (rtx_render_aov)");
	if (!s || !out) return fail(RTX_ERR_ARG, "scene/out is NULL");
	if (!out->depth_dev && !out->object_dev && !out->triangle_dev && !out->uv_dev && !out->normal_dev && !out->albedo_dev)
		return fail(RTX_ERR_ARG, "rtx_render_aov: no output (all six buffers are NULL)");
	if (s->stats) return fail(RTX_ERR_UNSUPPORTED, "rtx_render_aov collects no statistics (rtx_counters_enable)");
	const uint32_t W = s->params.view.width, H = s->params.view.height;
	if (rowEnd > H) rowEnd = H;
	if (rowBegin >= rowEnd) return RTX_OK;
	const uint32_t lastRow = (rowEnd < H - 1 ? rowEnd : H - 1);
	if (lastRow <= rowBegin) return RTX_OK;
	HIPCHK(hipSetDevice(s->device));
	hipStream_t st = (hipStream_t)stream;
	if (int ro = renderOn(s, st)) return ro;
	Params p = s->params;
	p.rowBegin = rowBegin; p.rowEnd = rowEnd;
	p.tilesX = (W - 1 + 7) / 8;
	p.tileRow0 = rowBegin / 8;
	const size_t tiles = (size_t)p.tilesX * ((lastRow + 7) / 8 - p.tileRow0);
	if (tiles >= (1u << 30)) return fail(RTX_ERR_ARG, "frame too large");
	p.nTiles = (uint32_t)tiles;
	const bool surface = out->normal_dev || out->albedo_dev;
	hipLaunchKernelGGL(aovKernel(variantOf(s), surface), dim3((unsigned)((tiles + 3) / 4)), dim3(256), 0, st, p, *out);
	HIPCHK(hipGetLastError());
	return RTX_OK;
}

int rtx_render_ao(rtx_scene* s, uint32_t rowBegin, uint32_t rowEnd, const rtx_ao_params* par, float* ao, uint32_t* counts, void* stream)
{
	RoctxRange range("Ambient occlusion (rtx_render_ao)");
	if (!s || !par) return fail(RTX_ERR_ARG, "scene/params is NULL");
	if (!ao && !counts) return fail(RTX_ERR_ARG, "rtx_render_ao: no output (both buffers are NULL)");
	if (!par->dirs_dev) return fail(RTX_ERR_ARG, "rtx_render_ao: dirs_dev is NULL");
	if (par->n_dirs < 1 || par->n_dirs > 256) return fail(RTX_ERR_ARG, "rtx_render_ao: n_dirs must be 1 .. 256");
	if (!(par->radius > 0)) return fail(RTX_ERR_ARG, "rtx_render_ao: radius must be > 0 (+inf: the whole ray)");
	if (s->stats) return fail(RTX_ERR_UNSUPPORTED, "rtx_render_ao collects no statistics (rtx_counters_enable)");
	const uint32_t W = s->params.view.width, H = s->params.view.height;
	if (rowEnd > H) rowEnd = H;
	if (rowBegin >= rowEnd) return RTX_OK;
	const uint32_t lastRow = (rowEnd < H - 1 ? rowEnd : H - 1);
	if (lastRow <= rowBegin) return RTX_OK;
	HIPCHK(hipSetDevice(s->device));
	hipStream_t st = (hipStream_t)stream;
	if (int ro = renderOn(s, st)) return ro;
	Params p = s->params;
	p.rowBegin = rowBegin; p.rowEnd = rowEnd;
	p.tilesX = (W - 1 + 7) / 8;
	p.tileRow0 = rowBegin / 8;
	const size_t tiles = (size_t)p.tilesX * ((lastRow + 7) / 8 - p.tileRow0);
	if (tiles >= (1u << 30)) return fail(RTX_ERR_ARG, "frame too large");
	p.nTiles = (uint32_t)tiles;
	const AoArgs a = { par->dirs_dev, par->n_dirs, par->radius, ao, counts };
	hipLaunchKernelGGL(aoKernel(variantOf(s)), dim3((unsigned)((tiles + 3) / 4)), dim3(256), 0, st, p, a);
	HIPCHK(hipGetLastError());
	return RTX_OK;
}

int rtx_math_probe(int device, int op, uint32_t n, const float* x, const float* y, float* out)
{
	if (!x || !out || op < 0 || op > 4) return fail(RTX_ERR_ARG, "bad argument");
	int cnt = 0;
	if (hipGetDeviceCount(&cnt) != hipSuccess || cnt <= 0) return fail(RTX_ERR_NO_DEVICE, "no HIP device visible");
	HIPCHK(hipSetDevice(device));
	DevArray<float> dx, dy, dout;
	const size_t bytes = (size_t)n * sizeof(float);
	HIPCHK(dx.reserve(n)); HIPCHK(dy.reserve(n)); HIPCHK(dout.reserve(n));
	HIPCHK(hipMemcpy(dx, x, bytes, hipMemcpyHostToDevice));
	if (y) HIPCHK(hipMemcpy(dy, y, bytes, hipMemcpyHostToDevice));
	else HIPCHK(hipMemset(dy, 0, bytes));
	hipLaunchKernelGGL(rtxMathProbeKernel, dim3((n + 255) / 256), dim3(256), 0, nullptr, op, n, (const float*)dx, (const float*)dy, dout.get());
	HIPCHK(hipGetLastError());
	HIPCHK(hipMemcpy(out, dout, bytes, hipMemcpyDeviceToHost));
	return RTX_OK;
}

int rtx_vec_probe(int device, int op, uint32_t n, const float* a, const float* b, float ior, float* out)
{
	if (!a || !out || op < 0 || op > 3 || (op < 3 && !b)) return fail(RTX_ERR_ARG, "bad argument");
	int cnt = 0;
	if (hipGetDeviceCount(&cnt) != hipSuccess || cnt <= 0) return fail(RTX_ERR_NO_DEVICE, "no HIP device visible");
	HIPCHK(hipSetDevice(device));
	DevArray<float> da, db, dout;
	const size_t bytes = (size_t)n * 3 * sizeof(float);
	HIPCHK(da.reserve((size_t)n * 3)); HIPCHK(dout.reserve((size_t)n * 3));
	HIPCHK(hipMemcpy(da, a, bytes, hipMemcpyHostToDevice));
	if (b) { HIPCHK(db.reserve((size_t)n * 3)); HIPCHK(hipMemcpy(db, b, bytes, hipMemcpyHostToDevice)); }
	hipLaunchKernelGGL(rtxVecProbeKernel, dim3((n + 255) / 256), dim3(256), 0, nullptr, op, n, (const float*)da, (const float*)db, ior, dout.get());
	HIPCHK(hipGetLastError());
	HIPCHK(hipMemcpy(out, dout, bytes, hipMemcpyDeviceToHost));
	return RTX_OK;
}

}

#include "rtx_bvh.hip"

#include "rtx_comm.hip"

#include "rtx_edit.hip"
```

### rendering_amd/csrc/rtx_flatten.hip

```cpp

namespace rtxflat {

constexpr uint32_t kNone = 0xffffffffu;

__device__ inline double dmin(double a, double b) { return b < a ? b : a; }
__device__ inline double dmax(double a, double b) { return a < b ? b : a; }
__device__ inline float fmin_(float a, float b) { return b < a ? b : a; }
__device__ inline float fmax_(float a, float b) { return a < b ? b : a; }

struct Agg { double lo[3], hi[3], ps, qlo[3], qhi[3], wlo, whi; uint32_t planes, rb, re, pad; };

constexpr int kCtlWords = 64;

__global__ void __launch_bounds__(256) nodesKernel(const float* bounds, const int32_t* skip, const int32_t* lb, const int32_t* lc, uint32_t n,
                                                   Node* nodes, uint32_t* parent, uint32_t* ctl)
{
	const uint32_t i = blockIdx.x * 256 + threadIdx.x;
	if (i >= n) return;
	Node nd;
	bool regular = true;
	for (int c = 0; c < 3; c++) {
		nd.b[2 * c] = bounds[(size_t)i * 6 + c]; nd.b[2 * c + 1] = bounds[(size_t)i * 6 + 3 + c];
		if (!(fabsf(nd.b[2 * c]) < 1e30f && fabsf(nd.b[2 * c + 1]) < 1e30f && nd.b[2 * c] <= nd.b[2 * c + 1])) regular = false;
	}
	if (!regular) atomicOr(&ctl[0], 1u);
	if (lc[i] < 0) {
		nd.link = skip[i]; nd.first = 0;
		if (i + 1 < n) {
			parent[i + 1] = i;
			const uint32_t right = lc[i + 1] >= 0 ? i + 2 : (uint32_t)skip[i + 1];
			if (right < n) parent[right] = i;
		}
	}
	else { nd.link = ~lc[i]; nd.first = lb[i]; }
	nodes[i] = nd;
	if (i == 0) {
		parent[0] = kNone;
		for (int c = 0; c < 6; c++) reinterpret_cast<float*>(ctl)[8 + c] = bounds[c];
	}
}

__device__ inline bool isLeaf(const Node* nodes, uint32_t i) { return nodes[i].link < 0; }
__device__ inline uint32_t rightOf(const Node* nodes, uint32_t i) { return isLeaf(nodes, i + 1) ? i + 2 : (uint32_t)nodes[i + 1].link; }

__global__ void __launch_bounds__(256) depthKernel(const Node* nodes, const uint32_t* parent, uint32_t n, uint32_t* depth, uint32_t* isRoot, uint32_t* ctl)
{
	const uint32_t i = blockIdx.x * 256 + threadIdx.x;
	if (i >= n) return;
	uint32_t d = 0;
	for (uint32_t p = parent[i]; p != kNone && d < n; p = parent[p]) d++;
	depth[i] = d;
	const bool root = !isLeaf(nodes, i) && d % 3 == 0;
	isRoot[i] = root ? 1u : 0u;
	atomicMax(&ctl[3], d);
	if (root) { atomicMax(&ctl[1], d / 3 + 1); atomicAdd(&ctl[2], 1u); }
	if (i > 0 && parent[i] == kNone) atomicOr(&ctl[0], 2u);
	else if (i > 0) {
		const Node& c = nodes[i];
		const Node& q = nodes[parent[i]];
		for (int k = 0; k < 3; k++)
			if (!(c.b[2 * k] >= q.b[2 * k] && c.b[2 * k + 1] <= q.b[2 * k + 1])) { atomicOr(&ctl[0], 2u); break; }
	}
}

__device__ inline int gatherSlots(const Node* nodes, uint32_t w, uint32_t slots[kWideSlots])
{
	int ns = 0;
	const uint32_t k1[2] = { w + 1, rightOf(nodes, w) };
	for (uint32_t a : k1) {
		if (isLeaf(nodes, a)) { slots[ns++] = a; continue; }
		const uint32_t k2[2] = { a + 1, rightOf(nodes, a) };
		for (uint32_t b : k2) {
			if (isLeaf(nodes, b)) { slots[ns++] = b; continue; }
			slots[ns++] = b + 1; slots[ns++] = rightOf(nodes, b);
		}
	}
	return ns;
}

__global__ void __launch_bounds__(256) innerCountKernel(const Node* nodes, uint32_t n, const uint32_t* isRoot, const uint32_t* rank, uint32_t* count)
{
	const uint32_t i = blockIdx.x * 256 + threadIdx.x;
	if (i >= n || !isRoot[i]) return;
	uint32_t slots[kWideSlots];
	const int ns = gatherSlots(nodes, i, slots);
	uint32_t c = 0;
	for (int k = 0; k < ns; k++) c += isLeaf(nodes, slots[k]) ? 0u : 1u;
	count[rank[i]] = c;
}

__global__ void __launch_bounds__(256) childIndexKernel(const Node* nodes, uint32_t n, const uint32_t* isRoot, const uint32_t* rank, const uint32_t* first,
                                                        uint32_t* wideOf)
{
	const uint32_t i = blockIdx.x * 256 + threadIdx.x;
	if (i >= n || !isRoot[i]) return;
	uint32_t slots[kWideSlots];
	const int ns = gatherSlots(nodes, i, slots);
	uint32_t next = 1 + first[rank[i]];
	for (int k = 0; k < ns; k++)
		if (!isLeaf(nodes, slots[k])) wideOf[slots[k]] = next++;
	if (i == 0) wideOf[0] = 0;
}

__global__ void __launch_bounds__(256) wideKernel(const Node* nodes, uint32_t n, const uint32_t* isRoot, const uint32_t* wideOf, uint32_t nWide,
                                                  WideNode* wide, uint32_t* slotNode)
{
	const uint32_t i = blockIdx.x * 256 + threadIdx.x;
	if (i >= n) return;
	uint32_t slots[kWideSlots];
	int ns;
	uint32_t wi;
	if (n == 1 || (i == 0 && isLeaf(nodes, 0))) { if (i != 0) return; slots[0] = 0; ns = 1; wi = 0; }
	else {
		if (!isRoot[i]) return;
		ns = gatherSlots(nodes, i, slots);
		wi = wideOf[i];
	}
	if (wi >= nWide) return;
	for (int k = 0; k < kWideSlots; k++) {
		Node sl;
		for (int c = 0; c < 6; c++) sl.b[c] = 0.0f;
		sl.link = 0; sl.first = 0;
		uint32_t sn = kNone;
		if (k < ns) {
			sn = slots[k];
			sl = nodes[sn];
			if (!isLeaf(nodes, sn)) { sl.link = (int32_t)wideOf[sn] + 1; sl.first = 0; }
		}
		wide[wi].slot[k] = sl;
		slotNode[(size_t)wi * kWideSlots + k] = sn;
	}
}

__device__ inline void aggInit(Agg& a)
{
	for (int k = 0; k < 3; k++) { a.lo[k] = a.qlo[k] = INFINITY; a.hi[k] = a.qhi[k] = -INFINITY; }
	a.ps = 0; a.wlo = INFINITY; a.whi = -INFINITY; a.planes = 1; a.rb = 0xffffffffu; a.re = 0; a.pad = 0;
}

__global__ void __launch_bounds__(256) leafAggKernel(const Node* nodes, uint32_t n, const uint32_t* refs, const float* pos, Agg* agg)
{
	const uint32_t i = blockIdx.x * 256 + threadIdx.x;
	if (i >= n || !isLeaf(nodes, i)) return;
	Agg a;
	aggInit(a);
	const uint32_t begin = (uint32_t)nodes[i].first, count = (uint32_t)~nodes[i].link;
	if (count) { a.rb = begin; a.re = begin + count; }
	for (uint32_t r = begin; r < begin + count; r++) {
		const float* p = pos + (size_t)refs[r] * 9;
		const float e1f[3] = { p[3] - p[0], p[4] - p[1], p[5] - p[2] }, e2f[3] = { p[6] - p[0], p[7] - p[1], p[8] - p[2] };
		const double v0[3] = { p[0], p[1], p[2] }, e1[3] = { e1f[0], e1f[1], e1f[2] }, e2[3] = { e2f[0], e2f[1], e2f[2] };
		double s1 = 0, s2 = 0;
		for (int k = 0; k < 3; k++) {
			const double x1 = v0[k] + e1[k], x2 = v0[k] + e2[k];
			a.lo[k] = dmin(a.lo[k], dmin(v0[k], dmin(x1, x2)));
			a.hi[k] = dmax(a.hi[k], dmax(v0[k], dmax(x1, x2)));
			s1 += fabs(e1[k]); s2 += fabs(e2[k]);
		}
		a.ps = dmax(a.ps, s1 * s2);
		if (s1 == 0 || s2 == 0) continue;
		const double sc = s1 * s2;
		if (!(sc > 1e-30) || !isfinite(sc)) { a.planes = 0; continue; }
		const double mq[3] = { (e2[1] * e1[2] - e2[2] * e1[1]) / sc, (e2[2] * e1[0] - e2[0] * e1[2]) / sc, (e2[0] * e1[1] - e2[1] * e1[0]) / sc };
		double w = 0;
		for (int k = 0; k < 3; k++) { a.qlo[k] = dmin(a.qlo[k], mq[k]); a.qhi[k] = dmax(a.qhi[k], mq[k]); w += v0[k] * mq[k]; }
		a.wlo = dmin(a.wlo, w); a.whi = dmax(a.whi, w);
	}
	agg[i] = a;
}

__device__ inline void aggMerge(Agg& a, const Agg& b)
{
	a.rb = b.rb < a.rb ? b.rb : a.rb; a.re = a.re < b.re ? b.re : a.re;
	for (int k = 0; k < 3; k++) {
		a.lo[k] = dmin(a.lo[k], b.lo[k]); a.hi[k] = dmax(a.hi[k], b.hi[k]);
		a.qlo[k] = dmin(a.qlo[k], b.qlo[k]); a.qhi[k] = dmax(a.qhi[k], b.qhi[k]);
	}
	a.ps = dmax(a.ps, b.ps); a.wlo = dmin(a.wlo, b.wlo); a.whi = dmax(a.whi, b.whi);
	a.planes = (a.planes && b.planes) ? 1u : 0u;
}

__global__ void __launch_bounds__(256) mergeLevelKernel(const Node* nodes, uint32_t n, const uint32_t* depth, uint32_t d, Agg* agg)
{
	const uint32_t i = blockIdx.x * 256 + threadIdx.x;
	if (i >= n || depth[i] != d || isLeaf(nodes, i)) return;
	Agg a;
	aggInit(a);
	aggMerge(a, agg[i + 1]);
	aggMerge(a, agg[rightOf(nodes, i)]);
	agg[i] = a;
}

__device__ inline void makeRec(const Agg& a, PruneRec& pr)
{
	for (int c = 0; c < 3; c++) pr.c[c] = 0.0f;
	pr.P = 0.0f; pr.Pgen = 0.0f;
	pr.h[0] = pr.h[1] = pr.h[2] = -1e30f;
	if (!(a.lo[0] <= a.hi[0])) return;
	bool finite = isfinite(a.ps);
	for (int c = 0; c < 3; c++) finite = finite && isfinite(a.lo[c]) && isfinite(a.hi[c]);
	if (!finite) { pr.h[0] = pr.h[1] = pr.h[2] = INFINITY; pr.P = pr.Pgen = INFINITY; return; }
	for (int c = 0; c < 3; c++) {
		const double mid = 0.5 * (a.lo[c] + a.hi[c]), big = dmax(fabs(a.lo[c]), fabs(a.hi[c]));
		pr.c[c] = (float)mid;
		pr.h[c] = (float)((0.5 * (a.hi[c] - a.lo[c]) + fabs((double)pr.c[c] - mid)) * (1.0 + 0x1p-20) + 0x1p-24 * big + 1e-37);
	}
	pr.P = pr.Pgen = (float)(a.ps * (1.0 + 0x1p-20) + 1e-37);
}

__global__ void __launch_bounds__(256) pruneKernel(const uint32_t* slotNode, uint32_t nWide, const Agg* agg, PruneBlock* prune, uint32_t* slotRange)
{
	const uint32_t t = blockIdx.x * 256 + threadIdx.x;
	if (t >= nWide * kWideSlots) return;
	const uint32_t wi = t / kWideSlots, k = t % kWideSlots;
	PruneRec pr;
	PlaneRec pl;
	for (int c = 0; c < 3; c++) { pr.c[c] = 0.0f; pl.qc[c] = 0.0f; pl.qr[c] = 0.0f; }
	pr.P = pr.Pgen = 0.0f;
	pr.h[0] = pr.h[1] = pr.h[2] = -1e30f;
	pl.wlo = -INFINITY; pl.whi = INFINITY;
	uint32_t rb = 0, re = 0;
	const uint32_t nd = slotNode[t];
	if (nd != kNone) {
		const Agg& a = agg[nd];
		if (a.rb < a.re) { rb = a.rb; re = a.re; }
		makeRec(a, pr);
		if ((a.lo[0] <= a.hi[0]) && isfinite(pr.P) && a.planes && a.wlo <= a.whi && isfinite(a.wlo) && isfinite(a.whi)) {
			for (int c = 0; c < 3; c++) {
				const double mid = 0.5 * (a.qlo[c] + a.qhi[c]);
				pl.qc[c] = (float)mid;
				pl.qr[c] = (float)((0.5 * (a.qhi[c] - a.qlo[c]) + fabs((double)pl.qc[c] - mid)) * (1.0 + 0x1p-20) + 0x1p-24);
			}
			pl.wlo = (float)(a.wlo - (fabs(a.wlo) * 0x1p-22 + 1e-37)); pl.whi = (float)(a.whi + (fabs(a.whi) * 0x1p-22 + 1e-37));
		}
	}
	prune[wi].box[k] = pr;
	prune[wi].plane[k] = pl;
	slotRange[(size_t)t * 2] = rb; slotRange[(size_t)t * 2 + 1] = re;
}

__global__ void rootRecKernel(const Agg* agg, uint32_t* ctl)
{
	if (blockIdx.x != 0 || threadIdx.x != 0) return;
	PruneRec pr;
	makeRec(agg[0], pr);
	memcpy(&ctl[16], &pr, sizeof(PruneRec));
	float v = 0.0f;
	for (int c = 0; c < 3; c++) v = fmax_(v, (float)dmax(fabs(agg[0].lo[c]), fabs(agg[0].hi[c])));
	memcpy(&ctl[24], &v, 4);
}

__global__ void __launch_bounds__(256) refsKernel(const uint32_t* refs, uint32_t nRefs, const float* pos, RefA* ra, RefB* rb, RefC* rc)
{
	const uint32_t r = blockIdx.x * 256 + threadIdx.x;
	if (r >= nRefs) return;
	const uint32_t t = refs[r];
	const float* p = pos + (size_t)t * 9;
	RefA a; RefB b; RefC c;
	a.v0x = p[0]; a.v0y = p[1]; a.v0z = p[2]; a.tri = t;
	b.e1x = p[3] - p[0]; b.e1y = p[4] - p[1]; b.e1z = p[5] - p[2];
	b.e2x = p[6] - p[0]; c.e2y = p[7] - p[1]; c.e2z = p[8] - p[2];
	ra[r] = a; rb[r] = b; rc[r] = c;
}

__global__ void __launch_bounds__(256) leafBoxKernel(const Node* nodes, uint32_t n, const uint32_t* refs, const float* pos, float* box8, uint32_t* flag)
{
	const uint32_t i = blockIdx.x * 256 + threadIdx.x;
	if (i >= n) return;
	flag[i] = 0;
	if (!isLeaf(nodes, i)) return;
	const int32_t count = ~nodes[i].link;
	if (count <= 0) return;
	float lo[3] = { INFINITY, INFINITY, INFINITY }, hi[3] = { -INFINITY, -INFINITY, -INFINITY };
	for (uint32_t r = (uint32_t)nodes[i].first; r < (uint32_t)(nodes[i].first + count); r++) {
		const float* p = pos + (size_t)refs[r] * 9;
		for (int v = 0; v < 9; v++) { lo[v % 3] = fmin_(lo[v % 3], p[v]); hi[v % 3] = fmax_(hi[v % 3], p[v]); }
	}
	if (!(isfinite(lo[0] + lo[1] + lo[2] + hi[0] + hi[1] + hi[2]))) return;
	const float b[8] = { lo[0], lo[1], lo[2], hi[0], hi[1], hi[2], (float)count, 0.0f };
	for (int c = 0; c < 8; c++) box8[(size_t)i * 8 + c] = b[c];
	flag[i] = 1;
}

__global__ void __launch_bounds__(256) leafCompactKernel(const float* box8, const uint32_t* flag, const uint32_t* at, uint32_t n, float* out, uint32_t* ctl)
{
	const uint32_t i = blockIdx.x * 256 + threadIdx.x;
	if (i >= n) return;
	if (i == n - 1) ctl[4] = at[i] + flag[i];
	if (!flag[i] || !out) return;
	for (int c = 0; c < 8; c++) out[(size_t)at[i] * 8 + c] = box8[(size_t)i * 8 + c];
}

__global__ void __launch_bounds__(1024) edgeSumKernel(const RefB* rb, const RefC* rc, uint32_t nRefs, uint32_t stride, uint32_t* ctl)
{
	__shared__ double sum[1024];
	__shared__ uint32_t cnt[1024];
	double s = 0; uint32_t c = 0;
	for (size_t r = (size_t)threadIdx.x * stride; r < nRefs; r += (size_t)1024 * stride) {
		const RefB& b = rb[r]; const RefC& e = rc[r];
		const double l1 = sqrt((double)b.e1x * b.e1x + (double)b.e1y * b.e1y + (double)b.e1z * b.e1z);
		const double l2 = sqrt((double)b.e2x * b.e2x + (double)e.e2y * e.e2y + (double)e.e2z * e.e2z);
		if (isfinite(l1 + l2)) { s += l1 + l2; c += 2; }
	}
	sum[threadIdx.x] = s; cnt[threadIdx.x] = c;
	__syncthreads();
	for (uint32_t h = 512; h > 0; h >>= 1) {
		if (threadIdx.x < h) { sum[threadIdx.x] += sum[threadIdx.x + h]; cnt[threadIdx.x] += cnt[threadIdx.x + h]; }
		__syncthreads();
	}
	if (threadIdx.x == 0) { memcpy(&ctl[32], &sum[0], 8); ctl[34] = cnt[0]; }
}

}

namespace {

inline unsigned blocksFor(size_t n) { return n ? (unsigned)((n + 255) / 256) : 1u; }

int deviceMeshGeometry(rtx_scene* s, const rtx_bvh* b, const float* pos_dev, uint32_t nTris, uint32_t mi, uint32_t nLights, DevBag& owned,
                       Mesh& dm, rtx_scene::SrcMesh& sm, rtx_scene::MeshLeaves& leaves, float bounds[6])
{
	using namespace rtxflat;
	const uint32_t n = b->nNodes, nRefs = b->nRefs;
	if (n == 0) return fail(RTX_ERR_DEVICE, "rtx_scene_update_mesh: the build left no nodes");
	hipStream_t st = nullptr;
	const size_t scanTmp = n / 512 + 64;
	const size_t szCtl = kCtlWords * 4, szU = ((size_t)n * 4 + 255) & ~(size_t)255;
	const size_t szAgg = (size_t)n * sizeof(Agg), szBox = (size_t)n * 32, szTmp = scanTmp * 4;
	const size_t need = szCtl + 7 * szU + szAgg + szBox + szTmp;
	HIPCHK(s->flatScratch.reserve(need));
	char* scratch = s->flatScratch;
	uint32_t* ctl = (uint32_t*)scratch;
	uint32_t* parent = (uint32_t*)(scratch + szCtl);
	uint32_t* depth = (uint32_t*)(scratch + szCtl + szU);
	uint32_t* isRoot = (uint32_t*)(scratch + szCtl + 2 * szU);
	uint32_t* rank = (uint32_t*)(scratch + szCtl + 3 * szU);
	uint32_t* count = (uint32_t*)(scratch + szCtl + 4 * szU);
	uint32_t* wideOf = (uint32_t*)(scratch + szCtl + 5 * szU);
	uint32_t* at = (uint32_t*)(scratch + szCtl + 6 * szU);
	Agg* agg = (Agg*)(scratch + szCtl + 7 * szU);
	float* box8 = (float*)(scratch + szCtl + 7 * szU + szAgg);
	uint32_t* tmp = (uint32_t*)(scratch + szCtl + 7 * szU + szAgg + szBox);
	uint32_t launches = 0;

	Node* nodes = nullptr;
	int rc;
	HIPCHK(owned.alloc(&nodes, (size_t)n * sizeof(Node)));
	HIPCHK(hipMemsetAsync(ctl, 0, szCtl, st));
	HIPCHK(hipMemsetAsync(parent, 0xff, (size_t)n * 4, st));
	hipLaunchKernelGGL(nodesKernel, dim3(blocksFor(n)), dim3(256), 0, st, b->bounds, b->skip, b->leafBegin, b->leafCount, n, nodes, parent, ctl);
	hipLaunchKernelGGL(depthKernel, dim3(blocksFor(n)), dim3(256), 0, st, nodes, (const uint32_t*)parent, n, depth, isRoot, ctl);
	uint32_t c0[16];
	HIPCHK(hipMemcpy(c0, ctl, sizeof(c0), hipMemcpyDeviceToHost));
	const bool boxesRegular = (c0[0] & 1u) == 0, nested = (c0[0] & 2u) == 0;
	const uint32_t depthMax = c0[1], nRoots = c0[2], maxDepth = c0[3];
	memcpy(bounds, &c0[8], 24);
	const bool hasWide = boxesRegular && nested && !((uint32_t)(kWideSlots - 1) * depthMax + 1 > (uint32_t)kWideStackEntries);
	const bool rootLeaf = nRoots == 0;
	const uint32_t nWide = hasWide ? (rootLeaf ? 1u : nRoots) : 0u;

	WideNode* wide = nullptr;
	DevArray<uint32_t> slotNode;
	if (nWide) {
		HIPCHK(owned.alloc(&wide, (size_t)nWide * sizeof(WideNode)));
		HIPCHK(slotNode.reserve((size_t)nWide * kWideSlots));
	}
	if (nWide && !rootLeaf) {
		HIPCHK(hipMemcpyAsync(rank, isRoot, (size_t)n * 4, hipMemcpyDeviceToDevice, st));
		if ((rc = scanExclusive(rank, n, tmp, st, launches))) return rc;
		hipLaunchKernelGGL(innerCountKernel, dim3(blocksFor(n)), dim3(256), 0, st, nodes, n, (const uint32_t*)isRoot, (const uint32_t*)rank, count);
		if ((rc = scanExclusive(count, nRoots, tmp, st, launches))) return rc;
		hipLaunchKernelGGL(childIndexKernel, dim3(blocksFor(n)), dim3(256), 0, st, nodes, n, (const uint32_t*)isRoot, (const uint32_t*)rank, (const uint32_t*)count, wideOf);
	}
	if (nWide) hipLaunchKernelGGL(wideKernel, dim3(blocksFor(n)), dim3(256), 0, st, nodes, n, (const uint32_t*)isRoot, (const uint32_t*)wideOf, nWide, wide, slotNode.get());
	dm.wide = wide; dm.nWide = nWide;

	RefA* ra = nullptr; RefB* rb = nullptr; RefC* rcr = nullptr;
	const size_t nPad = (size_t)nRefs + 64;
	HIPCHK(owned.alloc(&ra, nPad * sizeof(RefA))); HIPCHK(owned.alloc(&rb, nPad * sizeof(RefB))); HIPCHK(owned.alloc(&rcr, nPad * sizeof(RefC)));
	HIPCHK(hipMemsetAsync(ra, 0, nPad * sizeof(RefA), st)); HIPCHK(hipMemsetAsync(rb, 0, nPad * sizeof(RefB), st)); HIPCHK(hipMemsetAsync(rcr, 0, nPad * sizeof(RefC), st));
	if (nRefs) hipLaunchKernelGGL(refsKernel, dim3(blocksFor(nRefs)), dim3(256), 0, st, (const uint32_t*)b->refs, nRefs, pos_dev, ra, rb, rcr);

	uint32_t* flag = count;
	hipLaunchKernelGGL(leafBoxKernel, dim3(blocksFor(n)), dim3(256), 0, st, nodes, n, (const uint32_t*)b->refs, pos_dev, box8, flag);
	HIPCHK(hipMemcpyAsync(at, flag, (size_t)n * 4, hipMemcpyDeviceToDevice, st));
	if ((rc = scanExclusive(at, n, tmp, st, launches))) return rc;

	const bool pruneOn = nWide && s->knobs.prune;
	if (pruneOn) {
		hipLaunchKernelGGL(leafAggKernel, dim3(blocksFor(n)), dim3(256), 0, st, nodes, n, (const uint32_t*)b->refs, pos_dev, agg);
		for (uint32_t d = maxDepth + 1; d-- > 0;)
			hipLaunchKernelGGL(mergeLevelKernel, dim3(blocksFor(n)), dim3(256), 0, st, nodes, n, (const uint32_t*)depth, d, agg);
		hipLaunchKernelGGL(rootRecKernel, dim3(1), dim3(64), 0, st, (const Agg*)agg, ctl);
	}
	const uint32_t stride = nRefs > 65536 ? nRefs / 65536 : 1;
	hipLaunchKernelGGL(edgeSumKernel, dim3(1), dim3(1024), 0, st, (const RefB*)rb, (const RefC*)rcr, nRefs, stride, ctl);
	HIPCHK(hipGetLastError());
	hipLaunchKernelGGL(leafCompactKernel, dim3(blocksFor(n)), dim3(256), 0, st, (const float*)box8, (const uint32_t*)flag, (const uint32_t*)at, n, (float*)nullptr, ctl);
	uint32_t c1[kCtlWords];
	HIPCHK(hipMemcpy(c1, ctl, sizeof(c1), hipMemcpyDeviceToHost));
	const uint32_t nLeafBoxes = c1[4];
	float* lb = nullptr;
	if (nLeafBoxes) {
		HIPCHK(owned.alloc(&lb, (size_t)nLeafBoxes * 32));
		hipLaunchKernelGGL(leafCompactKernel, dim3(blocksFor(n)), dim3(256), 0, st, (const float*)box8, (const uint32_t*)flag, (const uint32_t*)at, n, lb, ctl);
	}
	leaves = { lb, nLeafBoxes };

	PruneRec rootRec;
	memset(&rootRec, 0, sizeof(rootRec));
	rootRec.h[0] = rootRec.h[1] = rootRec.h[2] = INFINITY; rootRec.P = INFINITY;
	float vmaxMesh = 0;
	if (pruneOn) { memcpy(&rootRec, &c1[16], sizeof(PruneRec)); memcpy(&vmaxMesh, &c1[24], 4); }

	sm = rtx_scene::SrcMesh();
	dm.prune = nullptr;
	DevArray<uint32_t> slotRange;
	if (pruneOn) {
		const uint32_t nCopies = s->knobs.sources ? 2u + std::min<uint32_t>(nLights, kMaxSrcLights) : 1u;
		PruneBlock* pb = nullptr;
		HIPCHK(owned.alloc(&pb, (size_t)nCopies * nWide * sizeof(PruneBlock)));
		HIPCHK(slotRange.reserve((size_t)nWide * kWideSlots * 2));
		hipLaunchKernelGGL(pruneKernel, dim3(blocksFor((size_t)nWide * kWideSlots)), dim3(256), 0, st, (const uint32_t*)slotNode, nWide, (const Agg*)agg, pb, slotRange.get());
		for (uint32_t c = 1; c < nCopies; c++) HIPCHK(hipMemcpyAsync(pb + (size_t)c * nWide, pb, (size_t)nWide * sizeof(PruneBlock), hipMemcpyDeviceToDevice, st));
		dm.prune = pb;
		sm.pruneAlloc = pb; sm.pruneWide = nWide;
		if (nCopies > 1) { sm.base = pb; sm.nWide = nWide; }
	}
	dm.vmax = vmaxMesh;
	dm.rootRec = rootRec;
	if (!(vmaxMesh < 0x1p40f)) { dm.prune = nullptr; dm.rootRec.h[0] = dm.rootRec.h[1] = dm.rootRec.h[2] = INFINITY; }
	dm.nodes = nodes; dm.refA = ra; dm.refB = rb; dm.refC = rcr;
	if (sm.base && vmaxMesh < 0x1p40f && nRefs) {
		sm.nRefs = nRefs; sm.refA = ra; sm.refB = rb; sm.refC = rcr; sm.vmax = vmaxMesh; sm.meshIndex = mi;
		HIPCHK(owned.copyFrom(slotRange.get(), (size_t)nWide * kWideSlots * 2, &sm.slotRange));
		HIPCHK(owned.alloc(&sm.refP, ((size_t)nRefs + nRefs / 64 + 2) * sizeof(float), false));
		sm.blockP = sm.refP + nRefs;
	}
	else sm.base = nullptr;
	dm.nNodes = n; dm.nRefs = nRefs; dm.nTris = nTris; dm.boxesRegular = boxesRegular ? 1u : 0u;
	{
		double sum;
		memcpy(&sum, &c1[32], 8);
		const uint32_t cnt = c1[34];
		const float factor = s->knobs.fatFactor;
		dm.fatRadius = cnt && factor > 0 ? (float)(sum / (double)cnt) * factor : INFINITY;
		double rad = 0;
		for (int c = 0; c < 3; c++) {
			const double lo = bounds[c], hi = bounds[3 + c];
			dm.centre[c] = (float)(0.5 * (lo + hi)); rad += 0.25 * (hi - lo) * (hi - lo);
		}
		dm.radius = (float)std::sqrt(rad);
		if (!std::isfinite(dm.radius)) { dm.radius = 0; dm.fatRadius = INFINITY; }
	}
	HIPCHK(hipStreamSynchronize(st));
	HIPCHK(hipGetLastError());
	return RTX_OK;
}

}
```

Before: 18180.

## Split oversized BVH leaves into wide-node chunk subtrees of 64 refs

```diff
diff --git a/include/rtx_debug.h b/include/rtx_debug.h
--- a/include/rtx_debug.h
+++ b/include/rtx_debug.h
@@ -9,6 +9,8 @@
 int rtx_set_frame_mode(rtx_scene* scene, int mode);
 
 int rtx_mesh_flatten_probe(const rtx_mesh* mesh, uint32_t* n_wide, void* wide_out, void* prune_out, uint32_t cap_wide, float* root_rec8);
+int rtx_mesh_flatten_probe_chunks(const rtx_mesh* mesh, uint32_t leaf_chunk_min, uint32_t* n_wide, void* wide_out, void* prune_out, uint32_t cap_wide,
+                                  float* root_rec8);
 int rtx_wide_node_slots(void);
 
 int rtx_source_p_probe(const float* tris9, uint32_t n, const double* S3, double sigma, int cam, float* out);
diff --git a/rendering_amd/__init__.py b/rendering_amd/__init__.py
--- a/rendering_amd/__init__.py
+++ b/rendering_amd/__init__.py
@@ -24,7 +24,7 @@
 
 RTX_SYMBOLS = [
     "rtx_last_error", "rtx_device_count", "rtx_scene_create", "rtx_scene_destroy", "rtx_scene_set_view", "rtx_scene_bytes",
-    "rtx_render_pass1", "rtx_sobel", "rtx_render_ssaa", "rtx_render_frame", "rtx_render_ac", "rtx_frame_status", "rtx_frame_mode", "rtx_set_frame_mode", "rtx_set_knob", "rtx_cost_grid_read", "rtx_mesh_flatten_probe", "rtx_wide_node_slots", "rtx_source_p_probe", "rtx_quantize_bgr8", "rtx_render_frame_host",
+    "rtx_render_pass1", "rtx_sobel", "rtx_render_ssaa", "rtx_render_frame", "rtx_render_ac", "rtx_frame_status", "rtx_frame_mode", "rtx_set_frame_mode", "rtx_set_knob", "rtx_cost_grid_read", "rtx_mesh_flatten_probe", "rtx_mesh_flatten_probe_chunks", "rtx_wide_node_slots", "rtx_source_p_probe", "rtx_quantize_bgr8", "rtx_render_frame_host",
     "rtx_counters_enable", "rtx_counters_reset", "rtx_counters_read", "rtx_last_kernel_ms", "rtx_math_probe",
     "rtx_cast_rays", "rtx_trace_rays", "rtx_kernel_time_reset", "rtx_kernel_time_stats", "rtx_tile_cost_read", "rtx_set_row_ownership",
     "rtx_bvh_build", "rtx_bvh_info", "rtx_bvh_read", "rtx_bvh_destroy",
@@ -90,6 +90,7 @@
     rtx.rtx_set_knob.argtypes = [vp, C.c_char_p, C.c_double]
     rtx.rtx_cost_grid_read.argtypes = [vp, vp, C.c_size_t, C.POINTER(C.c_uint32), C.POINTER(C.c_uint32)]
     rtx.rtx_mesh_flatten_probe.argtypes = [vp, C.POINTER(C.c_uint32), vp, vp, C.c_uint32, vp]
+    rtx.rtx_mesh_flatten_probe_chunks.argtypes = [vp, C.c_uint32, C.POINTER(C.c_uint32), vp, vp, C.c_uint32, vp]
     rtx.rtx_source_p_probe.argtypes = [vp, u32, vp, C.c_double, i32, vp]
     rtx.rtx_frame_mode.argtypes = [vp, C.POINTER(C.c_int), C.POINTER(C.c_float), C.POINTER(C.c_float)]
     rtx.rtx_quantize_bgr8.argtypes = [vp, vp, vp, vp]
@@ -359,7 +360,7 @@
     _fields_ = [("keep", C.c_int32), ("mesh", C.POINTER(_RtxMesh)), ("build", C.POINTER(RtxMeshBuild))]
 
 
-def mesh_flatten_probe(bvh):
+def mesh_flatten_probe(bvh, leaf_chunk_min=None):
     rtx, _ = load()
     bounds = np.ascontiguousarray(bvh["bounds"], np.float32); skip = np.ascontiguousarray(bvh["skip"], np.int32)
     lb = np.ascontiguousarray(bvh["leaf_begin"], np.int32); lc = np.ascontiguousarray(bvh["leaf_count"], np.int32)
@@ -370,10 +371,14 @@
     m.refs, m.tri_pos = refs.ctypes.data, pos.ctypes.data
     n = C.c_uint32(0)
     root = np.zeros(8, np.float32)
-    _check(rtx.rtx_mesh_flatten_probe(C.byref(m), C.byref(n), None, None, 0, _np_ptr(root)), "rtx_mesh_flatten_probe")
+    def probe(*args):
+        if leaf_chunk_min is None:
+            return rtx.rtx_mesh_flatten_probe(C.byref(m), *args)
+        return rtx.rtx_mesh_flatten_probe_chunks(C.byref(m), int(leaf_chunk_min), *args)
+    _check(probe(C.byref(n), None, None, 0, _np_ptr(root)), "rtx_mesh_flatten_probe")
     S = int(rtx.rtx_wide_node_slots())
     wide = np.zeros((n.value, S, 8), np.float32); prune = np.zeros((n.value, 2 * S, 8), np.float32)
-    _check(rtx.rtx_mesh_flatten_probe(C.byref(m), C.byref(n), _np_ptr(wide), _np_ptr(prune), n.value, _np_ptr(root)), "rtx_mesh_flatten_probe")
+    _check(probe(C.byref(n), _np_ptr(wide), _np_ptr(prune), n.value, _np_ptr(root)), "rtx_mesh_flatten_probe")
     return wide, prune[:, 0:S], prune[:, S:2 * S], root
 
 
diff --git a/rendering_amd/csrc/rtx_api.hip b/rendering_amd/csrc/rtx_api.hip
--- a/rendering_amd/csrc/rtx_api.hip
+++ b/rendering_amd/csrc/rtx_api.hip
@@ -29,6 +29,7 @@
 #include "rtx_rays.hip"
 #include "rtx_aov.hip"
 #include "rtx_ao.hip"
+#include "rtx_chunks.h"
 
 hipError_t rtxSortRayKeys(void* temp, size_t* tempBytes, const uint32_t* keysIn, uint32_t* keysOut, uint32_t* order, uint32_t n, int endBit,
                           hipStream_t st);
@@ -92,6 +93,7 @@
 
 }
 
+constexpr uint32_t kLeafChunkMinDefault = 513;
 struct Knobs {
 	int pass1BlocksPerCU = 0, ssaaBlocksPerCU = 0, frameBlocksPerCU = 0;
 	bool prune = true;
@@ -114,6 +116,7 @@
 	int traceReorder = -1;
 	int traceOriginFirst = 1;
 	int occludedSceneOrder = 0;
+	uint32_t leafChunkMin = kLeafChunkMinDefault;
 	uint32_t dbgTile = 0;
 };
 
@@ -244,6 +247,7 @@
 	if (const char* e = getenv("RTX_FRAME_MODE")) k.frameMode = !strcmp(e, "split") ? 0 : (!strcmp(e, "fused") ? 1 : -1);
 	k.frameQueueCap = (uint32_t)num("RTX_FRAME_QUEUE_CAP", 0);
 	k.debugItems = getenv("RTX_DEBUG_ITEMS") != nullptr;
+	k.leafChunkMin = (uint32_t)std::max<long long>(0, std::min<long long>(num("RTX_LEAF_CHUNK_MIN", k.leafChunkMin), 0x7fffffff));
 	if (const char* e = getenv("RTX_DBG_TILE")) { unsigned tx = 0, ty = 0; if (sscanf(e, "%u,%u", &tx, &ty) == 2) k.dbgTile = ((ty << 16) | tx) + 1; }
 }
 
@@ -538,7 +542,7 @@
 	bool boxesRegular = true;
 };
 
-int flattenMesh(const rtx_mesh& m, bool pruneWanted, FlatMesh& out)
+int flattenMesh(const rtx_mesh& m, bool pruneWanted, uint32_t chunkMin, FlatMesh& out)
 {
 	if (!m.node_bounds || !m.node_skip || !m.leaf_begin || !m.leaf_count || (m.n_refs && !m.refs) || (m.n_tris && !m.tri_pos)) return fail(RTX_ERR_ARG, "mesh arrays missing");
 	for (uint32_t r = 0; r < m.n_refs; r++)
@@ -588,8 +592,9 @@
 		};
 		struct Item { uint32_t node, wideIndex, depth; };
 		std::vector<Item> todo;
+		std::vector<uint32_t> wideLevel;
 		wide.emplace_back(); memset(&wide[0], 0, sizeof(WideNode));
-		slotNode.push_back(noSlots);
+		slotNode.push_back(noSlots); wideLevel.push_back(1u);
 		if (isLeaf(0)) { wide[0].slot[0] = nodes[0]; slotNode[0][0] = 0; }
 		else todo.push_back({ 0u, 0u, 1u });
 		while (!todo.empty() && nested) {
@@ -610,7 +615,7 @@
 			if (!nested) break;
 			uint32_t childWide[kWideSlots] = { 0 };
 			for (int k = 0; k < ns; k++)
-				if (!isLeaf(slots[k])) { childWide[k] = (uint32_t)wide.size(); wide.emplace_back(); memset(&wide.back(), 0, sizeof(WideNode)); slotNode.push_back(noSlots); }
+				if (!isLeaf(slots[k])) { childWide[k] = (uint32_t)wide.size(); wide.emplace_back(); memset(&wide.back(), 0, sizeof(WideNode)); slotNode.push_back(noSlots); wideLevel.push_back(it.depth + 1); }
 			for (int k = ns - 1; k >= 0; k--) {
 				slotNode[it.wideIndex][k] = slots[k];
 				Node sl = nodes[slots[k]];
@@ -619,24 +624,31 @@
 			}
 		}
 		if (!nested || (kWideSlots - 1) * depthMax + 1 > kWideStackEntries) wide.clear();
+		const size_t nRegular = wide.size();
+		std::vector<uint32_t> chunkRange;
+		if (!wide.empty() && chunkMin) {
+			std::vector<uint32_t> slotOf(m.n_nodes, kNoNode);
+			for (size_t wi = 0; wi < nRegular; wi++)
+				for (int k = 0; k < kWideSlots; k++)
+					if (slotNode[wi][k] != kNoNode && isLeaf(slotNode[wi][k])) slotOf[slotNode[wi][k]] = (uint32_t)(wi * kWideSlots + k);
+			for (uint32_t i = 0; i < m.n_nodes; i++) {
+				if (slotOf[i] == kNoNode) continue;
+				const uint32_t wi = slotOf[i] / kWideSlots, k = slotOf[i] % kWideSlots;
+				if (!rtxchunk::chunkSplit((uint32_t)m.leaf_count[i], chunkMin, wideLevel[wi])) continue;
+				const uint32_t base = (uint32_t)wide.size(), count = rtxchunk::chunkNodes(nodes[i], base, nullptr, nullptr);
+				wide.resize(wide.size() + count); slotNode.resize(slotNode.size() + count, noSlots);
+				chunkRange.resize(wide.size() * kWideSlots * 2, 0u);
+				rtxchunk::chunkNodes(nodes[i], base, wide.data(), chunkRange.data());
+				wide[wi].slot[k].link = (int32_t)base + 1; wide[wi].slot[k].first = 0;
+			}
+		}
 		if (!wide.empty() && pruneWanted) {
 			struct Agg { double lo[3], hi[3], ps, qlo[3], qhi[3], wlo, whi; bool planes; uint32_t rb, re; };
-			std::vector<Agg> agg(m.n_nodes);
-			for (uint32_t i = m.n_nodes; i-- > 0;) {
-				Agg& a = agg[i];
+			auto aggInit = [](Agg& a) {
 				for (int k = 0; k < 3; k++) { a.lo[k] = a.qlo[k] = INFINITY; a.hi[k] = a.qhi[k] = -INFINITY; }
 				a.ps = 0; a.wlo = INFINITY; a.whi = -INFINITY; a.planes = true; a.rb = 0xffffffffu; a.re = 0;
-				auto merge = [&](const Agg& b) {
-					a.rb = std::min(a.rb, b.rb); a.re = std::max(a.re, b.re);
-					for (int k = 0; k < 3; k++) {
-						a.lo[k] = std::min(a.lo[k], b.lo[k]); a.hi[k] = std::max(a.hi[k], b.hi[k]);
-						a.qlo[k] = std::min(a.qlo[k], b.qlo[k]); a.qhi[k] = std::max(a.qhi[k], b.qhi[k]);
-					}
-					a.ps = std::max(a.ps, b.ps); a.wlo = std::min(a.wlo, b.wlo); a.whi = std::max(a.whi, b.whi);
-					a.planes = a.planes && b.planes;
-				};
-				if (!isLeaf(i)) { merge(agg[i + 1]); merge(agg[rightOf(i)]); continue; }
-				const uint32_t begin = (uint32_t)m.leaf_begin[i], count = (uint32_t)m.leaf_count[i];
+			};
+			auto aggRefs = [&](Agg& a, uint32_t begin, uint32_t count) {
 				if (count) { a.rb = begin; a.re = begin + count; }
 				for (uint32_t r = begin; r < begin + count; r++) {
 					RefA ra; RefB rb; RefC rc;
@@ -658,6 +670,22 @@
 					for (int k = 0; k < 3; k++) { a.qlo[k] = std::min(a.qlo[k], mq[k]); a.qhi[k] = std::max(a.qhi[k], mq[k]); w += v0[k] * mq[k]; }
 					a.wlo = std::min(a.wlo, w); a.whi = std::max(a.whi, w);
 				}
+			};
+			std::vector<Agg> agg(m.n_nodes);
+			for (uint32_t i = m.n_nodes; i-- > 0;) {
+				Agg& a = agg[i];
+				aggInit(a);
+				auto merge = [&](const Agg& b) {
+					a.rb = std::min(a.rb, b.rb); a.re = std::max(a.re, b.re);
+					for (int k = 0; k < 3; k++) {
+						a.lo[k] = std::min(a.lo[k], b.lo[k]); a.hi[k] = std::max(a.hi[k], b.hi[k]);
+						a.qlo[k] = std::min(a.qlo[k], b.qlo[k]); a.qhi[k] = std::max(a.qhi[k], b.qhi[k]);
+					}
+					a.ps = std::max(a.ps, b.ps); a.wlo = std::min(a.wlo, b.wlo); a.whi = std::max(a.whi, b.whi);
+					a.planes = a.planes && b.planes;
+				};
+				if (!isLeaf(i)) { merge(agg[i + 1]); merge(agg[rightOf(i)]); continue; }
+				aggRefs(a, (uint32_t)m.leaf_begin[i], (uint32_t)m.leaf_count[i]);
 			}
 			auto makeRec = [&](const Agg& a, PruneRec& pr) {
 				memset(&pr, 0, sizeof(pr));
@@ -685,8 +713,15 @@
 					pr.h[0] = pr.h[1] = pr.h[2] = -1e30f;
 					pl.wlo = -INFINITY; pl.whi = INFINITY;
 					const uint32_t nd = slotNode[wi][k];
-					if (nd == kNoNode) continue;
-					const Agg& a = agg[nd];
+					Agg own;
+					if (nd == kNoNode) {
+						if (wi < nRegular) continue;
+						const uint32_t rb = chunkRange[(wi * kWideSlots + k) * 2], re = chunkRange[(wi * kWideSlots + k) * 2 + 1];
+						if (rb >= re) continue;
+						aggInit(own);
+						aggRefs(own, rb, re - rb);
+					}
+					const Agg& a = nd == kNoNode ? own : agg[nd];
 					if (a.rb < a.re) { out.slotRange[(wi * kWideSlots + k) * 2] = a.rb; out.slotRange[(wi * kWideSlots + k) * 2 + 1] = a.re; }
 					makeRec(a, pr);
 					if (!(a.lo[0] <= a.hi[0]) || !std::isfinite(pr.P)) continue;
@@ -711,7 +746,7 @@
 {
 	FlatMesh flat;
 	{
-		const int frc = flattenMesh(m, s->knobs.prune, flat);
+		const int frc = flattenMesh(m, s->knobs.prune, s->knobs.leafChunkMin, flat);
 		if (frc) return frc;
 	}
 	std::vector<Node>& nodes = flat.nodes;
@@ -2017,9 +2052,14 @@
 
 int rtx_mesh_flatten_probe(const rtx_mesh* m, uint32_t* n_wide, void* wide_out, void* prune_out, uint32_t cap_wide, float* root_rec8)
 {
+	return rtx_mesh_flatten_probe_chunks(m, kLeafChunkMinDefault, n_wide, wide_out, prune_out, cap_wide, root_rec8);
+}
+
+int rtx_mesh_flatten_probe_chunks(const rtx_mesh* m, uint32_t leaf_chunk_min, uint32_t* n_wide, void* wide_out, void* prune_out, uint32_t cap_wide, float* root_rec8)
+{
 	if (!m || !n_wide) return fail(RTX_ERR_ARG, "mesh/n_wide is NULL");
 	FlatMesh flat;
-	int rc = flattenMesh(*m, true, flat);
+	int rc = flattenMesh(*m, true, leaf_chunk_min, flat);
 	if (rc) return rc;
 	*n_wide = (uint32_t)flat.wide.size();
 	if (root_rec8) memcpy(root_rec8, &flat.rootRec, sizeof(PruneRec));
diff --git a/rendering_amd/csrc/rtx_chunks.h b/rendering_amd/csrc/rtx_chunks.h
--- /dev/null
+++ b/rendering_amd/csrc/rtx_chunks.h
@@ -0,0 +1,75 @@
+#pragma once
+#include "rtx_device.h"
+
+namespace rtxchunk {
+
+#if defined(__HIPCC__)
+#define RTX_CHUNK_FN __host__ __device__ inline
+#else
+#define RTX_CHUNK_FN inline
+#endif
+
+constexpr uint32_t kChunkRefs = 64;
+constexpr uint32_t kMaxWideLevels = (uint32_t)((rtxd::kWideStackEntries - 1) / (rtxd::kWideSlots - 1));
+
+RTX_CHUNK_FN uint32_t chunkLevels(uint32_t n)
+{
+	const uint64_t chunks = ((uint64_t)n + kChunkRefs - 1) / kChunkRefs;
+	uint32_t levels = 0;
+	for (uint64_t cap = 1; cap < chunks; cap *= rtxd::kWideSlots) levels++;
+	return levels;
+}
+
+RTX_CHUNK_FN bool chunkSplit(uint32_t n, uint32_t chunkMin, uint32_t wideLevel)
+{
+	if (chunkMin == 0 || n < chunkMin || n <= kChunkRefs) return false;
+	return wideLevel + chunkLevels(n) <= kMaxWideLevels;
+}
+
+RTX_CHUNK_FN uint32_t slotWideLevel(uint32_t depth) { return depth == 0 ? 1u : (depth - 1) / (uint32_t)rtxd::kWideLevels + 1; }
+
+RTX_CHUNK_FN uint32_t chunkNodes(const rtxd::Node& leaf, uint32_t base, rtxd::WideNode* wide, uint32_t* slotRange)
+{
+	const uint64_t first = (uint32_t)leaf.first, n = (uint32_t)~leaf.link;
+	const uint32_t levels = chunkLevels((uint32_t)n);
+	if (levels == 0) return 0;
+	const uint64_t chunks = (n + kChunkRefs - 1) / kChunkRefs;
+	struct Frame { uint64_t c0, c1, group; uint32_t index, next; };
+	Frame stack[12];
+	uint64_t group = 1;
+	for (uint32_t l = 1; l < levels; l++) group *= rtxd::kWideSlots;
+	uint32_t count = 0, sp = 0;
+	auto open = [&](uint64_t c0, uint64_t c1, uint64_t g) {
+		const uint32_t index = base + count++;
+		if (wide) {
+			rtxd::Node none;
+			for (int c = 0; c < 6; c++) none.b[c] = 0.0f;
+			none.link = 0; none.first = 0;
+			for (int k = 0; k < rtxd::kWideSlots; k++) wide[index].slot[k] = none;
+		}
+		if (slotRange)
+			for (int k = 0; k < 2 * rtxd::kWideSlots; k++) slotRange[(size_t)index * 2 * rtxd::kWideSlots + k] = 0;
+		stack[sp].c0 = c0; stack[sp].c1 = c1; stack[sp].group = g; stack[sp].index = index; stack[sp].next = 0;
+		sp++;
+	};
+	open(0, chunks, group);
+	while (sp) {
+		Frame& f = stack[sp - 1];
+		const uint64_t lo = f.c0 + (uint64_t)f.next * f.group;
+		if (f.next == (uint32_t)rtxd::kWideSlots || lo >= f.c1) { sp--; continue; }
+		const uint64_t hi = lo + f.group < f.c1 ? lo + f.group : f.c1;
+		const uint32_t k = f.next++, index = f.index;
+		const uint64_t rb = first + lo * kChunkRefs, re = first + (hi * kChunkRefs < n ? hi * kChunkRefs : n);
+		rtxd::Node sl = leaf;
+		if (hi - lo == 1) { sl.link = (int32_t)~(uint32_t)(re - rb); sl.first = (int32_t)rb; }
+		else {
+			sl.link = (int32_t)(base + count) + 1; sl.first = 0;
+			open(lo, hi, f.group / rtxd::kWideSlots);
+		}
+		if (wide) wide[index].slot[k] = sl;
+		if (slotRange) { slotRange[((size_t)index * rtxd::kWideSlots + k) * 2] = (uint32_t)rb; slotRange[((size_t)index * rtxd::kWideSlots + k) * 2 + 1] = (uint32_t)re; }
+	}
+	return count;
+}
+
+}
diff --git a/rendering_amd/csrc/rtx_flatten.hip b/rendering_amd/csrc/rtx_flatten.hip
--- a/rendering_amd/csrc/rtx_flatten.hip
+++ b/rendering_amd/csrc/rtx_flatten.hip
@@ -102,7 +102,36 @@
 	if (i == 0) wideOf[0] = 0;
 }
 
-__global__ void __launch_bounds__(256) wideKernel(const Node* nodes, uint32_t n, const uint32_t* isRoot, const uint32_t* wideOf, uint32_t nWide,
+__device__ inline uint32_t chunkCountOf(const Node* nodes, const uint32_t* depth, uint32_t i, uint32_t chunkMin)
+{
+	if (!isLeaf(nodes, i) || !rtxchunk::chunkSplit((uint32_t)~nodes[i].link, chunkMin, rtxchunk::slotWideLevel(depth[i]))) return 0;
+	return rtxchunk::chunkNodes(nodes[i], 0, nullptr, nullptr);
+}
+
+__global__ void __launch_bounds__(256) chunkCountKernel(const Node* nodes, const uint32_t* depth, uint32_t n, uint32_t chunkMin, uint32_t* count)
+{
+	const uint32_t i = blockIdx.x * 256 + threadIdx.x;
+	if (i < n) count[i] = chunkCountOf(nodes, depth, i, chunkMin);
+}
+
+__global__ void chunkTotalKernel(const Node* nodes, const uint32_t* depth, uint32_t n, uint32_t chunkMin, const uint32_t* chunkAt, uint32_t* ctl)
+{
+	if (blockIdx.x != 0 || threadIdx.x != 0) return;
+	ctl[5] = chunkAt[n - 1] + chunkCountOf(nodes, depth, n - 1, chunkMin);
+}
+
+__global__ void __launch_bounds__(256) chunkKernel(const Node* nodes, const uint32_t* depth, uint32_t n, uint32_t chunkMin, const uint32_t* chunkAt,
+                                                   uint32_t nRegular, uint32_t nWide, WideNode* wide, uint32_t* slotRange)
+{
+	const uint32_t i = blockIdx.x * 256 + threadIdx.x;
+	if (i >= n) return;
+	const uint32_t count = chunkCountOf(nodes, depth, i, chunkMin);
+	if (count == 0 || nRegular + chunkAt[i] + count > nWide) return;
+	rtxchunk::chunkNodes(nodes[i], nRegular + chunkAt[i], wide, slotRange);
+}
+
+__global__ void __launch_bounds__(256) wideKernel(const Node* nodes, uint32_t n, const uint32_t* isRoot, const uint32_t* wideOf, uint32_t nRegular,
+                                                  const uint32_t* depth, uint32_t chunkMin, const uint32_t* chunkAt,
                                                   WideNode* wide, uint32_t* slotNode)
 {
 	const uint32_t i = blockIdx.x * 256 + threadIdx.x;
@@ -116,7 +145,7 @@
 		ns = gatherSlots(nodes, i, slots);
 		wi = wideOf[i];
 	}
-	if (wi >= nWide) return;
+	if (wi >= nRegular) return;
 	for (int k = 0; k < kWideSlots; k++) {
 		Node sl;
 		for (int c = 0; c < 6; c++) sl.b[c] = 0.0f;
@@ -126,6 +155,7 @@
 			sn = slots[k];
 			sl = nodes[sn];
 			if (!isLeaf(nodes, sn)) { sl.link = (int32_t)wideOf[sn] + 1; sl.first = 0; }
+			else if (chunkMin && chunkCountOf(nodes, depth, sn, chunkMin)) { sl.link = (int32_t)(nRegular + chunkAt[sn]) + 1; sl.first = 0; }
 		}
 		wide[wi].slot[k] = sl;
 		slotNode[(size_t)wi * kWideSlots + k] = sn;
@@ -138,13 +168,8 @@
 	a.ps = 0; a.wlo = INFINITY; a.whi = -INFINITY; a.planes = 1; a.rb = 0xffffffffu; a.re = 0; a.pad = 0;
 }
 
-__global__ void __launch_bounds__(256) leafAggKernel(const Node* nodes, uint32_t n, const uint32_t* refs, const float* pos, Agg* agg)
-{
-	const uint32_t i = blockIdx.x * 256 + threadIdx.x;
-	if (i >= n || !isLeaf(nodes, i)) return;
-	Agg a;
-	aggInit(a);
-	const uint32_t begin = (uint32_t)nodes[i].first, count = (uint32_t)~nodes[i].link;
+__device__ inline void aggRefs(Agg& a, const uint32_t* refs, const float* pos, uint32_t begin, uint32_t count)
+{
 	if (count) { a.rb = begin; a.re = begin + count; }
 	for (uint32_t r = begin; r < begin + count; r++) {
 		const float* p = pos + (size_t)refs[r] * 9;
@@ -166,6 +191,15 @@
 		for (int k = 0; k < 3; k++) { a.qlo[k] = dmin(a.qlo[k], mq[k]); a.qhi[k] = dmax(a.qhi[k], mq[k]); w += v0[k] * mq[k]; }
 		a.wlo = dmin(a.wlo, w); a.whi = dmax(a.whi, w);
 	}
+}
+
+__global__ void __launch_bounds__(256) leafAggKernel(const Node* nodes, uint32_t n, const uint32_t* refs, const float* pos, Agg* agg)
+{
+	const uint32_t i = blockIdx.x * 256 + threadIdx.x;
+	if (i >= n || !isLeaf(nodes, i)) return;
+	Agg a;
+	aggInit(a);
+	aggRefs(a, refs, pos, (uint32_t)nodes[i].first, (uint32_t)~nodes[i].link);
 	agg[i] = a;
 }
 
@@ -208,7 +242,8 @@
 	pr.P = pr.Pgen = (float)(a.ps * (1.0 + 0x1p-20) + 1e-37);
 }
 
-__global__ void __launch_bounds__(256) pruneKernel(const uint32_t* slotNode, uint32_t nWide, const Agg* agg, PruneBlock* prune, uint32_t* slotRange)
+__global__ void __launch_bounds__(256) pruneKernel(const uint32_t* slotNode, uint32_t nWide, uint32_t nRegular, const Agg* agg, const uint32_t* refs, const float* pos,
+                                                   PruneBlock* prune, uint32_t* slotRange)
 {
 	const uint32_t t = blockIdx.x * 256 + threadIdx.x;
 	if (t >= nWide * kWideSlots) return;
@@ -220,9 +255,16 @@
 	pr.h[0] = pr.h[1] = pr.h[2] = -1e30f;
 	pl.wlo = -INFINITY; pl.whi = INFINITY;
 	uint32_t rb = 0, re = 0;
-	const uint32_t nd = slotNode[t];
-	if (nd != kNone) {
-		const Agg& a = agg[nd];
+	const uint32_t nd = wi < nRegular ? slotNode[t] : kNone;
+	Agg own;
+	bool have = nd != kNone;
+	if (wi >= nRegular && slotRange[(size_t)t * 2] < slotRange[(size_t)t * 2 + 1]) {
+		aggInit(own);
+		aggRefs(own, refs, pos, slotRange[(size_t)t * 2], slotRange[(size_t)t * 2 + 1] - slotRange[(size_t)t * 2]);
+		have = true;
+	}
+	if (have) {
+		const Agg& a = nd != kNone ? agg[nd] : own;
 		if (a.rb < a.re) { rb = a.rb; re = a.re; }
 		makeRec(a, pr);
 		if ((a.lo[0] <= a.hi[0]) && isfinite(pr.P) && a.planes && a.wlo <= a.whi && isfinite(a.wlo) && isfinite(a.whi)) {
@@ -327,7 +369,7 @@
 	const size_t scanTmp = n / 512 + 64;
 	const size_t szCtl = kCtlWords * 4, szU = ((size_t)n * 4 + 255) & ~(size_t)255;
 	const size_t szAgg = (size_t)n * sizeof(Agg), szBox = (size_t)n * 32, szTmp = scanTmp * 4;
-	const size_t need = szCtl + 7 * szU + szAgg + szBox + szTmp;
+	const size_t need = szCtl + 8 * szU + szAgg + szBox + szTmp;
 	HIPCHK(s->flatScratch.reserve(need));
 	char* scratch = s->flatScratch;
 	uint32_t* ctl = (uint32_t*)scratch;
@@ -338,9 +380,10 @@
 	uint32_t* count = (uint32_t*)(scratch + szCtl + 4 * szU);
 	uint32_t* wideOf = (uint32_t*)(scratch + szCtl + 5 * szU);
 	uint32_t* at = (uint32_t*)(scratch + szCtl + 6 * szU);
-	Agg* agg = (Agg*)(scratch + szCtl + 7 * szU);
-	float* box8 = (float*)(scratch + szCtl + 7 * szU + szAgg);
-	uint32_t* tmp = (uint32_t*)(scratch + szCtl + 7 * szU + szAgg + szBox);
+	uint32_t* chunkAt = (uint32_t*)(scratch + szCtl + 7 * szU);
+	Agg* agg = (Agg*)(scratch + szCtl + 8 * szU);
+	float* box8 = (float*)(scratch + szCtl + 8 * szU + szAgg);
+	uint32_t* tmp = (uint32_t*)(scratch + szCtl + 8 * szU + szAgg + szBox);
 	uint32_t launches = 0;
 
 	Node* nodes = nullptr;
@@ -350,6 +393,12 @@
 	HIPCHK(hipMemsetAsync(parent, 0xff, (size_t)n * 4, st));
 	hipLaunchKernelGGL(nodesKernel, dim3(blocksFor(n)), dim3(256), 0, st, b->bounds, b->skip, b->leafBegin, b->leafCount, n, nodes, parent, ctl);
 	hipLaunchKernelGGL(depthKernel, dim3(blocksFor(n)), dim3(256), 0, st, nodes, (const uint32_t*)parent, n, depth, isRoot, ctl);
+	const uint32_t chunkMin = s->knobs.leafChunkMin;
+	if (chunkMin) {
+		hipLaunchKernelGGL(chunkCountKernel, dim3(blocksFor(n)), dim3(256), 0, st, (const Node*)nodes, (const uint32_t*)depth, n, chunkMin, chunkAt);
+		if ((rc = scanExclusive(chunkAt, n, tmp, st, launches))) return rc;
+		hipLaunchKernelGGL(chunkTotalKernel, dim3(1), dim3(64), 0, st, (const Node*)nodes, (const uint32_t*)depth, n, chunkMin, (const uint32_t*)chunkAt, ctl);
+	}
 	uint32_t c0[16];
 	HIPCHK(hipMemcpy(c0, ctl, sizeof(c0), hipMemcpyDeviceToHost));
 	const bool boxesRegular = (c0[0] & 1u) == 0, nested = (c0[0] & 2u) == 0;
@@ -357,13 +406,17 @@
 	memcpy(bounds, &c0[8], 24);
 	const bool hasWide = boxesRegular && nested && !((uint32_t)(kWideSlots - 1) * depthMax + 1 > (uint32_t)kWideStackEntries);
 	const bool rootLeaf = nRoots == 0;
-	const uint32_t nWide = hasWide ? (rootLeaf ? 1u : nRoots) : 0u;
+	const uint32_t nRegular = hasWide ? (rootLeaf ? 1u : nRoots) : 0u;
+	const uint32_t nWide = nRegular + (hasWide && chunkMin ? c0[5] : 0u);
+	const bool pruneOn = nWide && s->knobs.prune;
 
 	WideNode* wide = nullptr;
 	DevArray<uint32_t> slotNode;
+	DevArray<uint32_t> slotRange;
 	if (nWide) {
 		HIPCHK(owned.alloc(&wide, (size_t)nWide * sizeof(WideNode)));
-		HIPCHK(slotNode.reserve((size_t)nWide * kWideSlots));
+		HIPCHK(slotNode.reserve((size_t)nRegular * kWideSlots));
+		if (pruneOn) HIPCHK(slotRange.reserve((size_t)nWide * kWideSlots * 2));
 	}
 	if (nWide && !rootLeaf) {
 		HIPCHK(hipMemcpyAsync(rank, isRoot, (size_t)n * 4, hipMemcpyDeviceToDevice, st));
@@ -372,7 +425,10 @@
 		if ((rc = scanExclusive(count, nRoots, tmp, st, launches))) return rc;
 		hipLaunchKernelGGL(childIndexKernel, dim3(blocksFor(n)), dim3(256), 0, st, nodes, n, (const uint32_t*)isRoot, (const uint32_t*)rank, (const uint32_t*)count, wideOf);
 	}
-	if (nWide) hipLaunchKernelGGL(wideKernel, dim3(blocksFor(n)), dim3(256), 0, st, nodes, n, (const uint32_t*)isRoot, (const uint32_t*)wideOf, nWide, wide, slotNode.get());
+	if (nWide) hipLaunchKernelGGL(wideKernel, dim3(blocksFor(n)), dim3(256), 0, st, nodes, n, (const uint32_t*)isRoot, (const uint32_t*)wideOf, nRegular,
+	                              (const uint32_t*)depth, nWide > nRegular ? chunkMin : 0u, (const uint32_t*)chunkAt, wide, slotNode.get());
+	if (nWide > nRegular) hipLaunchKernelGGL(chunkKernel, dim3(blocksFor(n)), dim3(256), 0, st, (const Node*)nodes, (const uint32_t*)depth, n, chunkMin, (const uint32_t*)chunkAt,
+	                                         nRegular, nWide, wide, pruneOn ? slotRange.get() : (uint32_t*)nullptr);
 	dm.wide = wide; dm.nWide = nWide;
 
 	RefA* ra = nullptr; RefB* rb = nullptr; RefC* rcr = nullptr;
@@ -386,7 +442,6 @@
 	HIPCHK(hipMemcpyAsync(at, flag, (size_t)n * 4, hipMemcpyDeviceToDevice, st));
 	if ((rc = scanExclusive(at, n, tmp, st, launches))) return rc;
 
-	const bool pruneOn = nWide && s->knobs.prune;
 	if (pruneOn) {
 		hipLaunchKernelGGL(leafAggKernel, dim3(blocksFor(n)), dim3(256), 0, st, nodes, n, (const uint32_t*)b->refs, pos_dev, agg);
 		for (uint32_t d = maxDepth + 1; d-- > 0;)
@@ -415,13 +470,12 @@
 
 	sm = rtx_scene::SrcMesh();
 	dm.prune = nullptr;
-	DevArray<uint32_t> slotRange;
 	if (pruneOn) {
 		const uint32_t nCopies = s->knobs.sources ? 2u + std::min<uint32_t>(nLights, kMaxSrcLights) : 1u;
 		PruneBlock* pb = nullptr;
 		HIPCHK(owned.alloc(&pb, (size_t)nCopies * nWide * sizeof(PruneBlock)));
-		HIPCHK(slotRange.reserve((size_t)nWide * kWideSlots * 2));
-		hipLaunchKernelGGL(pruneKernel, dim3(blocksFor((size_t)nWide * kWideSlots)), dim3(256), 0, st, (const uint32_t*)slotNode, nWide, (const Agg*)agg, pb, slotRange.get());
+		hipLaunchKernelGGL(pruneKernel, dim3(blocksFor((size_t)nWide * kWideSlots)), dim3(256), 0, st, (const uint32_t*)slotNode, nWide, nRegular, (const Agg*)agg,
+		                   (const uint32_t*)b->refs, pos_dev, pb, slotRange.get());
 		for (uint32_t c = 1; c < nCopies; c++) HIPCHK(hipMemcpyAsync(pb + (size_t)c * nWide, pb, (size_t)nWide * sizeof(PruneBlock), hipMemcpyDeviceToDevice, st));
 		dm.prune = pb;
 		sm.pruneAlloc = pb; sm.pruneWide = nWide;
```

Result: no change. 18300 (median of 6 runs) (+0.7%).
